# riveSunder/therldaisyworld

Hardware: AMD Instinct MI355X
Metric: cell-updates/sec (grid x batch), fused stencil+growth step (higher is better)
Workload: dtype f32

## Files before the change

therldaisyworld_amd/csrc/dw_api.hip:

```cpp
#include <hip/hip_runtime.h>

#include <cmath>
#include <cstdarg>
#include <cstdio>
#include <cstdlib>
#include <cstring>
#include <memory>
#include <new>
#include <optional>
#include <type_traits>
#include <vector>

#include "../../include/daisyworld_hip.h"
#include "dw_kernels.hpp"
#include "dw_host_util.hpp"
#include "dw_plan.hpp"
#include "dw_series.hpp"
#include "dw_episode_staging.hpp"

using namespace dw;

static thread_local char g_err[512] = "";

static int fail(int code, const char* fmt, ...) {
    va_list ap;
    va_start(ap, fmt);
    vsnprintf(g_err, sizeof(g_err), fmt, ap);
    va_end(ap);
    return code;
}

#define HIPCHK(expr)                                                                           \
    do {                                                                                       \
        hipError_t e_ = (expr);                                                                \
        if (e_ != hipSuccess)                                                                  \
            return fail(e_ == hipErrorOutOfMemory ? DW_ENOMEM : DW_EHIP, "%s failed: %s (%s:%d)", \
                        #expr, hipGetErrorString(e_), __FILE__, __LINE__);                      \
    } while (0)

#define NEED(cond, code, ...)                      \
    do {                                           \
        if (!(cond)) return fail(code, __VA_ARGS__); \
    } while (0)

enum UnqKind { UNQ_F64 = 1, UNQ_F32 = 2 };
enum UnqOwner { OWN_NONE = 0, OWN_CUR = 1, OWN_PREV = 2 };

static thread_local int t_fail_in = 0;
struct DeviceMem {
    static int alloc(void** p, size_t n) {
        if (t_fail_in > 0 && --t_fail_in == 0) return hipErrorOutOfMemory;
        return hipMalloc(p, n);
    }
    static int release(void* p) { return hipFree(p); }
};
struct PinnedMem {
    static int alloc(void** p, size_t n) { return hipHostMalloc(p, n, hipHostMallocDefault); }
    static int release(void* p) { return hipHostFree(p); }
};
template <class T> using DevBuf = Buf<T, DeviceMem>;
template <class T> using PinnedBuf = Buf<T, PinnedMem>;

struct dw_handle {
    dw_params prm;
    hipStream_t stream = nullptr;
    bool own_stream = false;
    size_t cells = 0;
    DevBuf<plane_t> L16[2];
    DevBuf<plane_t> D16[2];
    int cur = 0;
    DevBuf<double> L64;
    DevBuf<double> D64;
    DevBuf<float> U32L;
    DevBuf<float> U32D;
    UnqKind unq_kind = UNQ_F64;
    UnqOwner unq = OWN_NONE;
    bool have_state = false;
    bool stepped = false;
    double L_last = 0.0;
    bool L_per_world = false;
    bool P_per_world = false;
    DevBuf<int> idx;
    DevBuf<double> st;
    DevBuf<int> action;
    DevBuf<int> action_tmp;
    bool have_agents = false;
    DevBuf<StatsDev> stats2[2];
    size_t stats_bytes = 0;
    int sp = 0;
    DevBuf<uint4> fixq;
    unsigned int qcap = 0;
    DevBuf<int> redo_tiles;
    Switches sw{};
    StepPlan plan{};
    DevBuf<int> done_at;
    DevBuf<int> agents_done_at;
    DevBuf<int> n_alive;
    DevBuf<double> scratch;
    DevBuf<unsigned char> ep_buf;
    DevBuf<double> mlp_w;
    int mlp_members = 0;
    PinnedBuf<unsigned char> ep_pinned;
    DevBuf<double> reward_d;
    DevBuf<unsigned char> done_d;
    hipEvent_t ev0 = nullptr, ev1 = nullptr;
    hipEvent_t evf0 = nullptr, evf1 = nullptr;
    int fused_launches = 0;
    DevBuf<StatsDev> side_stats;
    DevBuf<StatsDev> trace_d;
    DevBuf<TempStatsDev> temp_d;
    DevBuf<TempPartial> temp_part;
    DevBuf<unsigned char> pw_tab;
    PinnedBuf<unsigned char> pw_pinned;
    PinnedBuf<unsigned char> pinned;
    struct Snapshot {
        DevBuf<plane_t> L, D;
        DevBuf<plane_t> PL, PD;
        bool stepped = false;
        double L_last = 0.0;
        bool L_per_world = false, P_per_world = false;
        UnqOwner unq = OWN_NONE;
        DevBuf<int> idx;
        DevBuf<double> st;
        DevBuf<unsigned char> stats;
        bool valid = false, agents = false;
    } snap[DW_SNAPSHOT_SLOTS];
    std::vector<std::pair<const void*, size_t>> lds_limit;
    bool created = false;
};

static inline bool cur_quantised(const dw_handle* h) { return h->unq != OWN_CUR; }

static inline bool lacks_shared_L(const dw_handle* h) { return h->stepped && h->L_per_world; }
#define NEED_SHARED_L(h, what)                                                                                          \
    NEED(!lacks_shared_L(h), DW_ESTATE,                                                                                 \
         "%s derives its temperature channels from the last step's luminosity, and the last step "                      \
         "(dw_step_n_trace_per_world) took a per-world luminosity: take a shared-L step or upload a state first", what)
static inline bool lacks_shared_constants(const dw_handle* h) { return lacks_shared_L(h) && h->P_per_world; }
#define NEED_SHARED_CONSTANTS(h, what)                                                                                  \
    NEED(!lacks_shared_constants(h), DW_ESTATE,                                                                         \
         "%s evaluates the last step's input state with one set of constants, and the last step "                       \
         "(dw_step_n_trace_ensemble) took per-world constants: take a shared-L step or upload a state first", what)

template <int V> using int_c = std::integral_constant<int, V>;

template <int V, int... Vs, class F>
static decltype(auto) with_int(int v, F&& f) {
    if constexpr (sizeof...(Vs) == 0) return f(int_c<V>{});
    else return v == V ? f(int_c<V>{}) : with_int<Vs...>(v, f);
}

template <class F>
static decltype(auto) with_bool(bool b, F&& f) { return b ? f(std::true_type{}) : f(std::false_type{}); }

template <class P> using elem_t = std::remove_cv_t<std::remove_pointer_t<P>>;

template <class F>
static decltype(auto) with_unq_planes(const dw_handle* h, F&& f) {
    return h->unq_kind == UNQ_F64 ? f(h->L64.get(), h->D64.get()) : f(h->U32L.get(), h->U32D.get());
}

template <class F>
static decltype(auto) with_planes(const dw_handle* h, bool unq, int buf, F&& f) {
    return unq ? with_unq_planes(h, f) : f(h->L16[buf].get(), h->D16[buf].get());
}

template <class F>
static auto with_derived_from(const dw_handle* h, F&& f) {
    const bool post = h->stepped;
    return with_planes(h, h->unq == (post ? OWN_PREV : OWN_CUR), post ? 1 - h->cur : h->cur, [&](auto* L, auto* D) {
        return with_bool(post, [&](auto POST) { return f(L, D, POST); });
    });
}

struct SyncOnExit {
    hipStream_t stream;
    bool armed = true;
    explicit SyncOnExit(hipStream_t s) : stream(s) {}
    ~SyncOnExit() { if (armed) (void)hipStreamSynchronize(stream); }
    void disarm() { armed = false; }
};

static int alloc_failed(int rc, const char* what, size_t bytes) {
    (void)hipGetLastError();
    const hipError_t e = static_cast<hipError_t>(rc);
    return fail(e == hipErrorOutOfMemory ? DW_ENOMEM : DW_EHIP, "allocating %s (%zu bytes) failed: %s", what, bytes,
                hipGetErrorString(e));
}
template <class B>
static int reserve(B& buf, const char* what, size_t need, size_t first_size = 0) {
    const int rc = buf.reserve(need, first_size);
    return rc ? alloc_failed(rc, what, need) : DW_OK;
}

static int alloc_group(dw_handle* h, const char* what, std::initializer_list<GroupItem<DeviceMem>> group) {
    static int fail_left = -1;
    if (h->created && fail_left < 0)
        if (const char* e = test_hook("DW_TEST_FAIL_GROUP_ALLOC")) fail_left = std::atoi(e);
    const bool armed = h->created && fail_left > 0;
    if (armed) t_fail_in = (int)group.size();
    const int rc = dw::alloc_group(group);
    if (armed && t_fail_in == 0) --fail_left;
    t_fail_in = 0;
    size_t bytes = 0;
    for (const auto& g : group) bytes += g.bytes;
    return rc ? alloc_failed(rc, what, bytes) : DW_OK;
}

static void release_unquantised(dw_handle* h) {
    if (h->unq != OWN_NONE || !h->U32L.get()) return;
    for (const auto& sn : h->snap)
        if (sn.valid && sn.unq == OWN_PREV) return;
    if (h->cells * 2 * sizeof(float) < ((size_t)1 << 30)) return;
    (void)hipStreamSynchronize(h->stream);
    h->U32L.reset();
    h->U32D.reset();
}

static void drop_unquantised_previous(dw_handle* h) {
    if (h->unq == OWN_PREV) { h->unq = OWN_NONE; h->stepped = false; }
    release_unquantised(h);
}

static int ensure_u32(dw_handle* h) {
    const size_t n = sizeof(float) * h->cells;
    return alloc_group(h, "two float32 planes", {{h->U32L, n}, {h->U32D, n}});
}

static int ensure_f64(dw_handle* h) {
    const size_t n = sizeof(double) * h->cells;
    return alloc_group(h, "two float64 planes", {{h->L64, n}, {h->D64, n}});
}
// ... 87 lines not shown
static void fill_episode_io(IO& io, const dw_handle* h, const EpisodeStaging& S) {
    const int cur = h->cur, prev = 1 - h->cur;
    io.L = h->L16[cur].get(); io.D = h->D16[cur].get(); io.prevL = h->L16[prev].get(); io.prevD = h->D16[prev].get();
    io.idx = h->idx.get(); io.st = h->st.get();
    io.P32 = S.at<const PhysF32>(h->ep_buf.get(), EpisodeStaging::P32);
    io.Ls = S.at<const double>(h->ep_buf.get(), EpisodeStaging::LS);
    io.stats = h->stats2[h->sp].get();
    io.fixups = &io.stats[h->prm.batch].sum_l;
}

template <class Kernel>
static int set_lds_limit(dw_handle* h, Kernel kern, size_t bytes) {
    const void* k = reinterpret_cast<const void*>(kern);
    size_t* set = nullptr;
    for (auto& e : h->lds_limit)
        if (e.first == k) set = &e.second;
    if (set && *set >= bytes) return DW_OK;
    HIPCHK(hipFuncSetAttribute(k, hipFuncAttributeMaxDynamicSharedMemorySize, (int)bytes));
    if (set) *set = bytes;
    else h->lds_limit.emplace_back(k, bytes);
    return DW_OK;
}

static int ensure_fixq(dw_handle* h, const StepPlan& plan) {
    if (!plan.need_fixq) return DW_OK;
    const dw_params& p = h->prm;
    size_t per_q = (h->cells / 64 + kNumQueues - 1) / kNumQueues;
    if (per_q < 2048) per_q = 2048;
    per_q = (per_q + 255) / 256 * 256;
    const size_t max_tiles = (size_t)p.batch * ((p.height + 7) / 8) * ((p.width / 4 + 15) / 16);
    if (int rc = alloc_group(h, "the near-tie queues", {{h->fixq, sizeof(uint4) * 3 * per_q * kNumQueues},
                                                         {h->redo_tiles, sizeof(int) * max_tiles}}))
        return rc;
    h->qcap = (unsigned int)per_q;
    return DW_OK;
}

struct StepOut {
    plane_t* L; plane_t* D;
    PhysF32 P;
    PhysF64 P64;
    StatsDev* stats;
    unsigned long long* fixups;
    unsigned long long* zero_me;
    int zero_n;
};
static StepOut step_out(const dw_handle* h) {
    const int out = 1 - h->cur;
    StatsDev* stats = h->stats2[1 - h->sp].get();
    return StepOut{h->L16[out].get(), h->D16[out].get(), PhysF32{}, PhysF64{}, stats, &stats[h->prm.batch].sum_l,
                   reinterpret_cast<unsigned long long*>(h->stats2[h->sp].get()),
                   (int)(h->stats_bytes / sizeof(unsigned long long))};
}

template <int TCQ, int RPT, bool EXACT>
static int launch_tiled(dw_handle* h, const plane_t* iL, const plane_t* iD, const StepOut& o, const FixQ& fq) {
    auto kern = step_tiled<TCQ, RPT, EXACT>;
    if constexpr (TileCfg<TCQ, RPT>::LDS_BYTES > 64 * 1024)
        if (int rc = set_lds_limit(h, kern, TileCfg<TCQ, RPT>::LDS_BYTES)) return rc;
    const Geom& g = h->plan.geom;
    constexpr size_t lds_bytes = TileCfg<TCQ, RPT>::LDS_BYTES;
    hipLaunchKernelGGL(kern, dim3((unsigned)g.chunk * 8u), dim3(256), lds_bytes, h->stream, iL, iD, o.L, o.D, g, o.P, o.stats,
                       o.fixups, o.zero_me, o.zero_n, fq);
    HIPCHK(hipGetLastError());
    if (EXACT) {
        const dim3 qg((fq.qcap + 255) / 256, kNumQueues);
        hipLaunchKernelGGL(fixup_cells, qg, dim3(256), 0, h->stream, o.L, o.D, h->prm.height, h->prm.width, o.P64, o.stats, fq);
        hipLaunchKernelGGL(redo_tiles_f64, dim3(256), dim3(256), 0, h->stream, iL, iD, o.L, o.D, g, TileCfg<TCQ, RPT>::TR, TCQ,
                           o.P64, o.stats, fq);
        HIPCHK(hipGetLastError());
    }
    return DW_OK;
}

static dim3 generic_grid(const dw_params& p, int* cpt) {
    *cpt = generic_cells_per_thread(p.batch, (long long)p.height * p.width);
    return dim3((unsigned)(((long long)p.height * p.width + 256LL * *cpt - 1) / (256LL * *cpt)), (unsigned)p.batch);
}

template <class T, int PREC>
static auto launch_generic(dw_handle* h, const T* iL, const T* iD, const StepOut& o, const FirstStepBound& fb = {}) {
    const dw_params& p = h->prm;
    int cpt;
    const dim3 grid = generic_grid(p, &cpt);
    hipLaunchKernelGGL((step_generic<T, PREC>), grid, dim3(256), 0, h->stream, iL, iD, o.L, o.D, p.height, p.width, o.P, o.P64,
                       o.stats, o.fixups, o.zero_me, o.zero_n, cpt, fb);
}

static int launch_first_step(dw_handle* h, double L, const StepOut& o) {
    const StepPlan& pl = h->plan;
    const FirstStepBound fb = pl.first_prec == 3 ? derive_first_bound(h->prm, L, o.P, h->unq_kind == UNQ_F64, h->sw.first_slack)
                                                 : FirstStepBound{};
    if (pl.first_stream) {
        const dim3 grid((unsigned)((pl.first_geom.nstrips + 3) / 4));
        with_unq_planes(h, [&](auto* iL, auto* iD) {
            with_int<1, 3>(pl.first_prec, [&](auto PR) {
                with_int<0, 1, 2, 3>(pl.halo, [&](auto HL) {
                    hipLaunchKernelGGL((step_first_stream<elem_t<decltype(iL)>, PR, HL>), grid, dim3(256), 0, h->stream, iL, iD,
                                       o.L, o.D, pl.first_geom, o.P, o.P64, o.stats, o.fixups, o.zero_me, o.zero_n, fb);
                });
            });
        });
    } else {
        with_unq_planes(h, [&](auto* iL, auto* iD) {
            with_int<1, 3, 2>(pl.first_prec, [&](auto PR) { launch_generic<elem_t<decltype(iL)>, PR>(h, iL, iD, o, fb); });
        });
    }
    HIPCHK(hipGetLastError());
    return DW_OK;
}

static int launch_step(dw_handle* h, const StepOut& o) {
    const dw_params& p = h->prm;
    const StepPlan& pl = h->plan;
    const plane_t* iL = h->L16[h->cur].get();
    const plane_t* iD = h->D16[h->cur].get();
    const bool ex = p.precision == DW_PRECISION_EXACT;
    if (pl.kind == STEP_GENERIC) {
        const int prec = p.precision == DW_PRECISION_F64 ? 2 : (ex ? 0 : 1);
        with_int<2, 0, 1>(prec, [&](auto PR) { launch_generic<plane_t, PR>(h, iL, iD, o); });
    } else if (pl.kind == STEP_STREAM && ex) {
        const StreamExactArgs A{iL, iD, o.L, o.D, pl.sgeom, o.P, o.stats, o.fixups, o.zero_me, o.zero_n, o.P64};
        with_int<0, 1, 2, 3>(pl.halo, [&](auto HL) {
            with_bool(pl.sym_albedo, [&](auto SYM) {
                hipLaunchKernelGGL((step_stream_exact<HL, SYM>), dim3((unsigned)pl.sgeom.chunk * 8u), dim3(256), 0, h->stream, A);
            });
        });
    } else if (pl.kind == STEP_STREAM) {
        with_int<0, 1, 2, 3>(pl.halo, [&](auto HL) {
            hipLaunchKernelGGL((step_stream_fast<HL>), dim3((unsigned)pl.sgeom.chunk * 8u), dim3(256), 0, h->stream, iL, iD, o.L,
                               o.D, pl.sgeom, o.P, o.P64, o.stats, o.fixups, o.zero_me, o.zero_n);
        });
    } else {
        FixQ fq;
        fq.entries = h->fixq.get();
        fq.counts = reinterpret_cast<unsigned int*>(o.stats + p.batch + 1);
        fq.qcap = h->qcap;
        fq.redo_tiles = h->redo_tiles.get();
        auto tiled = [&](auto TCQ, auto RPT) {
            return with_bool(ex, [&](auto EX) { return launch_tiled<TCQ, RPT, EX>(h, iL, iD, o, fq); });
        };
        if (pl.tcq == 64) return with_int<8, 4, 2>(pl.rpt, [&](auto RPT) { return tiled(int_c<64>{}, RPT); });
        return pl.tcq == 32 ? tiled(int_c<32>{}, int_c<4>{}) : tiled(int_c<16>{}, int_c<2>{});
    }
    HIPCHK(hipGetLastError());
    return DW_OK;
}

static void step_done(dw_handle* h, double L, bool stepped, bool per_world = false, bool per_world_constants = false) {
    h->cur = 1 - h->cur;
    h->sp = 1 - h->sp;
    h->unq = h->unq == OWN_CUR ? OWN_PREV : OWN_NONE;
    h->stepped = stepped;
    h->L_last = L;
    h->L_per_world = per_world;
    h->P_per_world = per_world && per_world_constants;
    release_unquantised(h);
}

static void episode_done(dw_handle* h, double L_last, bool per_world) {
    h->unq = OWN_NONE;
    h->stepped = true;
    h->L_last = per_world ? 0.0 : L_last;
    h->L_per_world = per_world;
    h->P_per_world = per_world;
}

static int launch_forward(dw_handle* h, double L) {
    const dw_params& p = h->prm;
    NEED(h->have_state, DW_ESTATE, "no state uploaded (call dw_upload_state_* or dw_init_random)");
    StepOut o = step_out(h);
    o.P = derive_f32(p, L);
    o.P64 = make_f64(p, L);
#ifdef DW_TUNING
    if (const char* e = std::getenv("DW_ABLATE")) {
        if (std::strcmp(e, "copy") == 0) {
            const int in = h->cur;
            const size_t n4 = h->cells * sizeof(plane_t) / 16;
            hipLaunchKernelGGL(copy_planes, dim3((unsigned)((n4 + 255) / 256)), dim3(256), 0, h->stream,
                               reinterpret_cast<const float4*>(h->L16[in].get()), reinterpret_cast<const float4*>(h->D16[in].get()),
                               reinterpret_cast<float4*>(o.L), reinterpret_cast<float4*>(o.D), n4);
            HIPCHK(hipGetLastError());
            step_done(h, L, true);
            return DW_OK;
        }
        const int v = std::strcmp(e, "nomath") == 0 ? 1 : 0;
        HIPCHK(hipMemcpyToSymbolAsync(HIP_SYMBOL(g_ablate), &v, sizeof(int), 0, hipMemcpyHostToDevice, h->stream));
    }
#endif
    if (int rc = h->unq == OWN_CUR ? launch_first_step(h, L, o) : launch_step(h, o)) return rc;
    step_done(h, L, true);
    return DW_OK;
}

static int launch_forward_pw(dw_handle* h, const PhysF32* row32, const PhysF64* row64, const FirstStepBound* rowfb, bool sym,
                             bool constants) {
    const dw_params& p = h->prm;
    const StepPlan& pl = h->plan;
    const StepOut o = step_out(h);
    const bool ex = p.precision == DW_PRECISION_EXACT;
    auto generic = [&](auto* iL, auto* iD, auto PR) {
        int cpt;
        const dim3 grid = generic_grid(p, &cpt);
        hipLaunchKernelGGL((step_generic_pw<elem_t<decltype(iL)>, PR>), grid, dim3(256), 0, h->stream, iL, iD, o.L, o.D,
                           p.height, p.width, row32, row64, rowfb, o.stats, o.fixups, o.zero_me, o.zero_n, cpt);
    };
    const plane_t* iL = h->L16[h->cur].get();
    const plane_t* iD = h->D16[h->cur].get();
    if (h->unq == OWN_CUR) {
        with_unq_planes(h, [&](auto* uL, auto* uD) {
            with_int<1, 3, 2>(pl.first_prec, [&](auto PR) { generic(uL, uD, PR); });
        });
    } else if (pl.pw_stream && ex) {
        const StreamExactPwArgs A{iL, iD, o.L, o.D, pl.sgeom, row32, row64, o.stats, o.fixups, o.zero_me, o.zero_n};
        with_int<0, 1, 2>(pl.halo, [&](auto HL) {
            with_bool(sym, [&](auto SYM) {
                hipLaunchKernelGGL((step_stream_exact_pw<HL, SYM>), dim3((unsigned)pl.sgeom.chunk * 8u), dim3(256), 0, h->stream, A);
            });
        });
    } else if (pl.pw_stream) {
        with_int<0, 1, 2>(pl.halo, [&](auto HL) {
            hipLaunchKernelGGL((step_stream_fast_pw<HL>), dim3((unsigned)pl.sgeom.chunk * 8u), dim3(256), 0, h->stream, iL, iD, o.L,
                               o.D, pl.sgeom, row32, row64, o.stats, o.fixups, o.zero_me, o.zero_n);
        });
    } else {
        const int prec = p.precision == DW_PRECISION_F64 ? 2 : (ex ? 0 : 1);
        with_int<2, 0, 1>(prec, [&](auto PR) { generic(iL, iD, PR); });
    }
    HIPCHK(hipGetLastError());
    step_done(h, 0.0, true, true, constants);
    return DW_OK;
}

static int launch_forward_fused2_pw(dw_handle* h, const PairPw* row, StatsDev* trace) {
    const StepPlan& pl = h->plan;
    const StepOut o = step_out(h);
    const FusedGeom& g = pl.fgeom;
    const dim3 grid((unsigned)g.chunk * 8u);
    const plane_t *inL = h->L16[h->cur].get(), *inD = h->D16[h->cur].get();
    with_int<kFusedRot, kFusedOvl>(pl.fused_mode, [&](auto MODE) {
        hipLaunchKernelGGL((trace_pair_fast_pw<MODE>), grid, dim3(256), 0, h->stream, inL, inD, o.L, o.D, g, row, o.zero_me,
                           o.zero_n, trace);
    });
    HIPCHK(hipGetLastError());
    step_done(h, 0.0, false, true, true);
    return DW_OK;
}

static int temp_chunks(const dw_handle* h) {
    return (int)(((long long)h->prm.height * h->prm.width + kTempChunk - 1) / kTempChunk);
}
static size_t temp_part_bytes(const dw_handle* h) { return sizeof(TempPartial) * (size_t)h->prm.batch * temp_chunks(h); }

static int launch_temp_moments(dw_handle* h, bool current, double L, const PhysF64* row64, TempStatsDev* out) {
    const dw_params& p = h->prm;
    const int chunks = temp_chunks(h);
    const PhysF64 P = row64 ? PhysF64{} : make_f64(p, L);
    TempPartial* part = h->temp_part.get();
    auto reduce = [&](auto* iL, auto* iD) {
        with_bool(row64 != nullptr, [&](auto TABLE) {
            hipLaunchKernelGGL((temp_moments_pw<elem_t<decltype(iL)>, TABLE>), dim3((unsigned)chunks, (unsigned)p.batch), dim3(256),
                               0, h->stream, iL, iD, p.height, p.width, P, row64, part);
        });
    };
    if (current) with_planes(h, h->unq == OWN_CUR, h->cur, reduce);
    else with_derived_from(h, [&](auto* iL, auto* iD, auto) { reduce(iL, iD); });
    HIPCHK(hipGetLastError());
    hipLaunchKernelGGL(temp_moments_finish_pw, dim3((unsigned)((p.batch + 63) / 64)), dim3(64), 0, h->stream, part, p.batch, chunks,
                       (double)p.height * (double)p.width, out);
    HIPCHK(hipGetLastError());
    return DW_OK;
}

template <class F>
static auto with_fused_layout(const StepPlan& pl, F&& f) {
    if (pl.packed) return f(int_c<kFusedRot>{}, std::true_type{});
    return with_int<kFusedRot, kFusedRing, kFusedOvl>(pl.fused_mode, [&](auto MODE) { return f(MODE, std::false_type{}); });
}

static int launch_forward_fused2(dw_handle* h, double L1, double L2, unsigned int* pstats = nullptr,
                                 float thr_hi = 0.f, StatsDev* trace = nullptr) {
    const dw_params& p = h->prm;
    const StepPlan& pl = h->plan;
    const bool exact = p.precision == DW_PRECISION_EXACT;
    PhysF32 P1, P2;
    if (exact) derive_f32_pair(p, L1, L2, &P1, &P2);
    else { P1 = derive_f32(p, L1); P2 = derive_f32(p, L2); }
    const StepOut o = step_out(h);
    const FusedGeom& g = pl.fgeom;
    const dim3 grid((unsigned)g.chunk * 8u);
    const plane_t *inL = h->L16[h->cur].get(), *inD = h->D16[h->cur].get();
    auto exact_args = [&] {
        return FusedExactArgs{inL, inD, o.L, o.D, g, P1, lum_part(P2), o.zero_me, o.zero_n, pstats, thr_hi, make_f64(p, L1), L1, L2};
    };
    if (trace && exact) {
        const TraceExactArgs A{exact_args(), trace, h->sw.force_rescan ? 1 : 0};
        with_int<kFusedRot, kFusedOvl>(pl.fused_mode, [&](auto MODE) {
            with_bool(pl.sym_albedo, [&](auto SYM) {
                hipLaunchKernelGGL((trace_pair_exact<MODE, SYM>), grid, dim3(256), 0, h->stream, A);
            });
        });
    } else if (trace) {
        with_int<kFusedRot, kFusedOvl>(pl.fused_mode, [&](auto MODE) {
            hipLaunchKernelGGL((trace_pair_fast<MODE>), grid, dim3(256), 0, h->stream, inL, inD, o.L, o.D, g, P1, P2, o.zero_me,
                               o.zero_n, trace);
        });
    } else if (pl.seam_strips && !pstats && !exact) {
        const FusedGeom &gs = pl.seam_geom, &gl = pl.left_geom;
        hipLaunchKernelGGL(step_stream_fused2_seam_pw, dim3((unsigned)gs.chunk * 8u), dim3(256), 0, h->stream, inL, inD, o.L, o.D,
                           gs, P1, P2, o.zero_me, o.zero_n);
        if (gl.nstrips)
            hipLaunchKernelGGL(step_stream_fused2_left_pw, dim3((unsigned)gl.chunk * 8u), dim3(256), 0, h->stream, inL, inD, o.L,
                               o.D, gl, P1, P2, o.zero_me, 0);
    } else if (pl.fmt_planes && !pstats && !exact) {
        hipLaunchKernelGGL((step_stream_fused2_fmt_pw<kFusedOvl>), grid, dim3(256), 0, h->stream, inL, inD, o.L, o.D, g, P1, P2,
                           o.zero_me, o.zero_n);
    } else if (exact) {
        const FusedExactArgs A = exact_args();
        with_bool(pstats != nullptr, [&](auto STATS) {
            with_fused_layout(pl, [&](auto MODE, auto PACK) {
                with_bool(pl.sym_albedo, [&](auto SYM) {
                    hipLaunchKernelGGL((step_stream_fused2_exact<MODE, PACK, STATS, SYM>), grid, dim3(256), 0, h->stream, A);
                });
            });
        });
    } else {
        with_bool(pstats != nullptr, [&](auto STATS) {
            with_fused_layout(pl, [&](auto MODE, auto PACK) {
                hipLaunchKernelGGL((step_stream_fused2<MODE, PACK, STATS>), grid, dim3(256), 0, h->stream, inL, inD, o.L, o.D, g,
                                   P1, P2, o.zero_me, o.zero_n, pstats, thr_hi);
            });
        });
    }
    HIPCHK(hipGetLastError());
    step_done(h, L2, false);
    return DW_OK;
}

static int launch_agents(dw_handle* h, const int* d_action, int act_b, int act_n, bool standalone = false,
                         double* d_reward = nullptr, unsigned char* d_done = nullptr, unsigned char* d_ok = nullptr) {
    const dw_params& p = h->prm;
    if (p.n_agents == 0) return DW_OK;
    NEED(h->have_state, DW_ESTATE, "no state uploaded");
    NEED(h->have_agents, DW_ESTATE, "no agents uploaded (call dw_upload_agents or dw_init_random)");
    NEED(p.collision_mode == 0 || standalone, DW_EINVAL,
         "collision_mode=1: call dw_update_agents, apply the collision pass (it consumes the caller's RNG) to the "
         "downloaded agent states, upload them, then dw_step without actions");
    const int blocks = (p.batch + 63) / 64;
    with_planes(h, h->unq == OWN_CUR, h->cur, [&](auto* L, auto* D) {
        using T = elem_t<decltype(L)>;
        hipLaunchKernelGGL(agents_update<T>, dim3(blocks), dim3(64), 0, h->stream, L, D, h->idx.get(), h->st.get(), d_action,
                           act_b, act_n, p.batch, p.n_agents, p.height, p.width, p.agent_gamma,
                           p.collision_mode == 0 ? 1 : 0, d_reward, d_done, d_ok);
    });
    HIPCHK(hipGetLastError());
    return DW_OK;
}

static int stage_host_actions(dw_handle* h, const int32_t* action, int b, int n) {
    const dw_params& p = h->prm;
    NEED(b >= 0 && n >= 0 && b <= p.batch && n <= p.n_agents, DW_EINVAL,
         "action block %dx%d exceeds (B,N)=(%d,%d)", b, n, p.batch, p.n_agents);
    if ((size_t)b * n)
        HIPCHK(hipMemcpyAsync(h->action_tmp.get(), action, sizeof(int) * (size_t)b * n, hipMemcpyHostToDevice,
                              h->stream));
    return DW_OK;
}

static int clear_stats(dw_handle* h) {
    for (int i = 0; i < 2; ++i) HIPCHK(hipMemsetAsync(h->stats2[i].get(), 0, h->stats_bytes, h->stream));
    return DW_OK;
}

static void state_arrived(dw_handle* h, UnqOwner unq, UnqKind kind = UNQ_F64) {
    if (unq == OWN_CUR) h->unq_kind = kind;
    h->unq = unq;
    h->have_state = true;
    h->stepped = false;
    for (auto& sn : h->snap) sn.valid = false;
}

template <class T>
static auto init_random_into(dw_handle* h, uint64_t seed, T* L, T* D) {
    const dw_params& p = h->prm;
    if (int crc = clear_stats(h)) return crc;
    const int ncell = p.height * p.width;
    const dim3 g((unsigned)((ncell + kInitChunk - 1) / kInitChunk), (unsigned)p.batch);
    hipLaunchKernelGGL((init_random_cells<T>), g, dim3(256), 0, h->stream, L, D, ncell,
                       (long long)p.world_offset, (unsigned long long)seed, (float)p.light_proportion,
                       (float)p.dark_proportion, (float)p.initial_al, (float)p.initial_ad, h->stats2[h->sp].get());
    HIPCHK(hipGetLastError());
    if (p.n_agents) {
        const int bn = p.batch * p.n_agents;
        hipLaunchKernelGGL(init_random_agents, dim3((bn + 255) / 256), dim3(256), 0, h->stream, h->idx.get(), h->st.get(),
                           p.batch, p.n_agents, p.height, p.width, (long long)p.world_offset,
                           (unsigned long long)seed);
        HIPCHK(hipGetLastError());
    }
    h->have_agents = true;
    return (int)DW_OK;
}

extern "C" {

const char* dw_last_error(void) { return g_err; }
int dw_abi_version(void) { return DW_ABI_VERSION; }

int dw_pinned_alloc(size_t bytes, void** out) {
    NEED(out && bytes > 0, DW_EINVAL, "null argument");
    int ndev = 0;
    NEED(hipGetDeviceCount(&ndev) == hipSuccess && ndev > 0, DW_ENODEVICE, "no HIP device");
    HIPCHK(hipHostMalloc(out, bytes, hipHostMallocDefault));
    return DW_OK;
}
int dw_pinned_free(void* p) {
    if (p) HIPCHK(hipHostFree(p));
    return DW_OK;
}

#ifndef DW_BUILD_ID
#define DW_BUILD_ID "unknown"
#endif
static const char kBuildId[] = "DW_BUILD_ID=" DW_BUILD_ID;
const char* dw_build_id(void) { return kBuildId + 12; }

int dw_default_params(dw_params* p, int32_t batch, int32_t height, int32_t width, int32_t n_agents) {
    NEED(p, DW_EINVAL, "null params");
    std::memset(p, 0, sizeof(*p));
    p->abi_version = DW_ABI_VERSION;
    p->batch = batch; p->height = height; p->width = width; p->n_agents = n_agents;
    p->device = 0; p->precision = DW_PRECISION_EXACT; p->obs_mask = 0x0BA; p->collision_mode = 0;
    p->world_offset = 0;
    p->p = 1.0; p->g = 0.003265; p->S = 1000.0; p->sigma = 5.67e-8; p->gamma = 0.25;
    p->q = 0.2 * p->S / p->sigma; p->q2 = p->q / 8.0; p->dt = 1.0;
    p->albedo_bare = 0.5; p->albedo_light = 0.75; p->albedo_dark = 0.25; p->temp_optimal = 295.5;
    p->agent_gamma = 0.05; p->food_chain_penalty = 0.5;
    p->initial_al = 0.2; p->initial_ad = 0.2; p->light_proportion = 0.33; p->dark_proportion = 0.33;
    return DW_OK;
}

static int check_params(const dw_params* p) {
    NEED(p, DW_EINVAL, "null params");
    NEED(p->abi_version == DW_ABI_VERSION, DW_EINVAL, "ABI version %d != %d", p->abi_version, DW_ABI_VERSION);
    NEED(p->batch >= 1 && p->height >= 3 && p->width >= 3, DW_EINVAL,
         "need batch>=1 and grid >= 3x3 (got B=%d H=%d W=%d)", p->batch, p->height, p->width);
    NEED(p->height <= 65535 && p->width <= 65532, DW_EINVAL, "grid dimension too large");
    NEED((long long)p->height * p->width <= 0x7fffffffLL, DW_EINVAL,
         "a world of %dx%d cells exceeds the 2^31-1 cells per world the kernels index", p->height, p->width);
    NEED(p->n_agents >= 0, DW_EINVAL, "n_agents < 0");
    NEED(p->precision >= 0 && p->precision <= 2, DW_EINVAL, "bad precision %d", p->precision);
    NEED(p->precision == DW_PRECISION_F64 || p->g >= 0.0, DW_EINVAL,
         "g < 0 (a growth curve opening upwards) is evaluated by DW_PRECISION_F64 only");
    NEED((double)p->batch * p->height * p->width < 9.0e18, DW_EINVAL, "too many cells");
    return DW_OK;
}

int dw_create(const dw_params* p, dw_handle** out) {
    NEED(out, DW_EINVAL, "null out");
    *out = nullptr;
    int rc = check_params(p);
    if (rc) return rc;
    int ndev = 0;
    if (hipGetDeviceCount(&ndev) != hipSuccess || ndev <= 0)
        return fail(DW_ENODEVICE, "no HIP device available (this library has no CPU fallback)");
    NEED(p->device >= 0 && p->device < ndev, DW_ENODEVICE, "device %d out of range (%d devices)", p->device, ndev);
    HIPCHK(hipSetDevice(p->device));
    hipDeviceProp_t prop;
    HIPCHK(hipGetDeviceProperties(&prop, p->device));
    if (std::strncmp(prop.gcnArchName, "gfx950", 6) != 0)
        return fail(DW_ENODEVICE, "device %d is %s; this library is built for gfx950 only", p->device,
                    prop.gcnArchName);
    std::unique_ptr<dw_handle, int (*)(dw_handle*)> h(new (std::nothrow) dw_handle(), dw_destroy);
    NEED(h, DW_ENOMEM, "host allocation failed");
    h->prm = *p;
    h->cells = (size_t)p->batch * p->height * p->width;
    HIPCHK(hipStreamCreateWithFlags(&h->stream, hipStreamNonBlocking));
    h->own_stream = true;
    const size_t bn = (size_t)p->batch * (p->n_agents > 0 ? p->n_agents : 1);
    const size_t pb = sizeof(plane_t) * h->cells;
    h->stats_bytes = sizeof(StatsDev) * (p->batch + 1) + sizeof(unsigned int) * (kNumQueues + 1) * 16;
    if (int rc = alloc_group(h.get(), "the handle's state",
                             {{h->L16[0], pb}, {h->D16[0], pb}, {h->L16[1], pb}, {h->D16[1], pb},
                              {h->idx, sizeof(int) * bn * 2}, {h->st, sizeof(double) * bn}, {h->action, sizeof(int) * bn},
                              {h->action_tmp, sizeof(int) * bn}, {h->reward_d, sizeof(double) * bn}, {h->done_d, bn},
                              {h->agents_done_at, sizeof(int) * bn}, {h->done_at, sizeof(int) * p->batch},
                              {h->n_alive, sizeof(int)}, {h->stats2[0], h->stats_bytes}, {h->stats2[1], h->stats_bytes},
                              {h->side_stats, sizeof(StatsDev) * (p->batch + 1)}}))
        return rc;
    for (int i = 0; i < 2; ++i) HIPCHK(hipMemsetAsync(h->stats2[i].get(), 0, h->stats_bytes, h->stream));
    h->sw = read_switches();
    h->plan = plan_steps(*p, h->sw);
    if (int rc = ensure_fixq(h.get(), h->plan)) return rc;
    HIPCHK(hipMemsetAsync(h->action.get(), 0, sizeof(int) * bn, h->stream));
    HIPCHK(hipMemsetAsync(h->done_at.get(), 0, sizeof(int) * p->batch, h->stream));
    HIPCHK(hipMemsetAsync(h->agents_done_at.get(), 0, sizeof(int) * bn, h->stream));
    HIPCHK(hipMemsetAsync(h->n_alive.get(), 0, sizeof(int), h->stream));
    HIPCHK(hipEventCreate(&h->ev0));
    HIPCHK(hipEventCreate(&h->ev1));
    HIPCHK(hipEventCreate(&h->evf0));
    HIPCHK(hipEventCreate(&h->evf1));
    h->created = true;
    *out = h.release();
    return DW_OK;
}

int dw_destroy(dw_handle* h) {
    if (!h) return DW_OK;
    (void)hipSetDevice(h->prm.device);
    if (h->stream) (void)hipStreamSynchronize(h->stream);
    if (h->ev0) (void)hipEventDestroy(h->ev0);
    if (h->ev1) (void)hipEventDestroy(h->ev1);
    if (h->evf0) (void)hipEventDestroy(h->evf0);
    if (h->evf1) (void)hipEventDestroy(h->evf1);
    if (h->own_stream && h->stream) (void)hipStreamDestroy(h->stream);
    delete h;
    return DW_OK;
}

int dw_set_params(dw_handle* h, const dw_params* p) {
    NEED(h, DW_EINVAL, "null handle");
    int rc = check_params(p);
    if (rc) return rc;
    const dw_params& o = h->prm;
    NEED(p->batch == o.batch && p->height == o.height && p->width == o.width && p->n_agents == o.n_agents &&
             p->device == o.device,
         DW_EINVAL, "dw_set_params cannot change shape or device; create a new handle");
    HIPCHK(hipSetDevice(p->device));
    const StepPlan plan = plan_steps(*p, h->sw);
    if ((rc = ensure_fixq(h, plan))) return rc;
    h->prm = *p;
    h->plan = plan;
    return DW_OK;
}

int dw_get_params(const dw_handle* h, dw_params* out) {
    NEED(h && out, DW_EINVAL, "null argument");
    *out = h->prm;
    return DW_OK;
}


static int refresh_stats(dw_handle* h) {
    const dw_params& p = h->prm;
    if (int rc = clear_stats(h)) return rc;
    const int n = p.height * p.width;
    const dim3 g((unsigned)((n + kInitChunk - 1) / kInitChunk), (unsigned)p.batch);
    auto reduce = [&](auto* L, auto* D) {
        hipLaunchKernelGGL((stats_only<elem_t<decltype(L)>>), g, dim3(256), 0, h->stream, L, D, n, h->stats2[h->sp].get());
    };
    if (cur_quantised(h)) reduce(h->L16[h->cur].get(), h->D16[h->cur].get());
    else with_unq_planes(h, reduce);
    HIPCHK(hipGetLastError());
    return DW_OK;
}

int dw_upload_state_f64(dw_handle* h, const double* light, const double* dark) {
    NEED(h && light && dark, DW_EINVAL, "null argument");
    HIPCHK(hipSetDevice(h->prm.device));
    if (int arc = ensure_f64(h)) return arc;
    HIPCHK(hipMemcpyAsync(h->L64.get(), light, sizeof(double) * h->cells, hipMemcpyHostToDevice, h->stream));
    HIPCHK(hipMemcpyAsync(h->D64.get(), dark, sizeof(double) * h->cells, hipMemcpyHostToDevice, h->stream));
    state_arrived(h, OWN_CUR, UNQ_F64);
    int rc = refresh_stats(h);
    if (rc) return rc;
    HIPCHK(hipStreamSynchronize(h->stream));
    return DW_OK;
}

int dw_upload_state_f32(dw_handle* h, const float* light, const float* dark, int quantised) {
    NEED(h && light && dark, DW_EINVAL, "null argument");
    HIPCHK(hipSetDevice(h->prm.device));
    const unsigned blocks = (unsigned)((h->cells + 255) / 256);
    if (quantised) {
        int rc = ensure_scratch(h, sizeof(float) * 2 * h->cells);
        if (rc) return rc;
        float* sL = reinterpret_cast<float*>(h->scratch.get());
        float* sD = sL + h->cells;
        HIPCHK(hipMemcpyAsync(sL, light, sizeof(float) * h->cells, hipMemcpyHostToDevice, h->stream));
        HIPCHK(hipMemcpyAsync(sD, dark, sizeof(float) * h->cells, hipMemcpyHostToDevice, h->stream));
        hipLaunchKernelGGL(f32nat_to_plane, dim3(blocks), dim3(256), 0, h->stream, sL, h->L16[h->cur].get(), h->cells);
        hipLaunchKernelGGL(f32nat_to_plane, dim3(blocks), dim3(256), 0, h->stream, sD, h->D16[h->cur].get(), h->cells);
        HIPCHK(hipGetLastError());
        state_arrived(h, OWN_NONE);
    } else {
        int rc = ensure_u32(h);
        if (rc) return rc;
        HIPCHK(hipMemcpyAsync(h->U32L.get(), light, sizeof(float) * h->cells, hipMemcpyHostToDevice, h->stream));
        HIPCHK(hipMemcpyAsync(h->U32D.get(), dark, sizeof(float) * h->cells, hipMemcpyHostToDevice, h->stream));
        hipLaunchKernelGGL(f32nat_to_permille, dim3(blocks), dim3(256), 0, h->stream, h->U32L.get(), h->U32L.get(), h->cells);
        hipLaunchKernelGGL(f32nat_to_permille, dim3(blocks), dim3(256), 0, h->stream, h->U32D.get(), h->U32D.get(), h->cells);
        HIPCHK(hipGetLastError());
        state_arrived(h, OWN_CUR, UNQ_F32);
    }
    int rc = refresh_stats(h);
    if (rc) return rc;
    HIPCHK(hipStreamSynchronize(h->stream));
    return DW_OK;
}

int dw_upload_agents(dw_handle* h, const int32_t* indices, const double* states) {
    NEED(h, DW_EINVAL, "null handle");
    const dw_params& p = h->prm;
    HIPCHK(hipSetDevice(p.device));
    const size_t bn = (size_t)p.batch * p.n_agents;
    if (bn) {
        NEED(indices && states, DW_EINVAL, "null argument");
        for (size_t i = 0; i < bn; ++i) {
            NEED(indices[2 * i] >= 0 && indices[2 * i] < p.height && indices[2 * i + 1] >= 0 &&
                     indices[2 * i + 1] < p.width,
                 DW_EINVAL, "agent %zu position (%d,%d) outside the %dx%d grid", i, indices[2 * i],
                 indices[2 * i + 1], p.height, p.width);
        }
        HIPCHK(hipMemcpyAsync(h->idx.get(), indices, sizeof(int) * bn * 2, hipMemcpyHostToDevice, h->stream));
        HIPCHK(hipMemcpyAsync(h->st.get(), states, sizeof(double) * bn, hipMemcpyHostToDevice, h->stream));
        HIPCHK(hipStreamSynchronize(h->stream));
    }
    h->have_agents = true;
    return DW_OK;
}

int dw_download_agents(dw_handle* h, int32_t* indices, double* states) {
    NEED(h, DW_EINVAL, "null handle");
    const dw_params& p = h->prm;
    HIPCHK(hipSetDevice(p.device));
    const size_t bn = (size_t)p.batch * p.n_agents;
    if (bn) {
        NEED(h->have_agents, DW_ESTATE, "no agents");
        if (indices) HIPCHK(hipMemcpyAsync(indices, h->idx.get(), sizeof(int) * bn * 2, hipMemcpyDeviceToHost, h->stream));
        if (states) HIPCHK(hipMemcpyAsync(states, h->st.get(), sizeof(double) * bn, hipMemcpyDeviceToHost, h->stream));
    }
    HIPCHK(hipStreamSynchronize(h->stream));
    return DW_OK;
}

int dw_init_random(dw_handle* h, uint64_t seed) {
    NEED(h, DW_EINVAL, "null handle");
    HIPCHK(hipSetDevice(h->prm.device));
    if (int rc = ensure_u32(h)) return rc;
    if (int rc = init_random_into(h, seed, h->U32L.get(), h->U32D.get())) return rc;
    state_arrived(h, OWN_CUR, UNQ_F32);
    return DW_OK;
}

int dw_init_random_quantised(dw_handle* h, uint64_t seed) {
    NEED(h, DW_EINVAL, "null handle");
    HIPCHK(hipSetDevice(h->prm.device));
    if (int rc = init_random_into(h, seed, h->L16[h->cur].get(), h->D16[h->cur].get())) return rc;
    state_arrived(h, OWN_NONE);
    release_unquantised(h);
    return DW_OK;
}

int dw_download_planes(dw_handle* h, int which, double* light, double* dark) {
    NEED(h, DW_EINVAL, "null handle");
    NEED(h->have_state, DW_ESTATE, "no state");
    HIPCHK(hipSetDevice(h->prm.device));
    NEED(which == DW_STATE_CURRENT || which == DW_STATE_PREVIOUS, DW_EINVAL, "bad state selector");
    NEED(which == DW_STATE_CURRENT || h->stepped, DW_ESTATE, "no previous state before the first step");
    const int buf = which == DW_STATE_CURRENT ? h->cur : 1 - h->cur;
    const bool unq = (which == DW_STATE_CURRENT && h->unq == OWN_CUR) || (which == DW_STATE_PREVIOUS && h->unq == OWN_PREV);
    const size_t bytes = sizeof(double) * h->cells;
    if (unq && h->unq_kind == UNQ_F64) {
        if (light) HIPCHK(hipMemcpyAsync(light, h->L64.get(), bytes, hipMemcpyDeviceToHost, h->stream));
        if (dark) HIPCHK(hipMemcpyAsync(dark, h->D64.get(), bytes, hipMemcpyDeviceToHost, h->stream));
    } else {
        int rc = ensure_scratch(h, bytes);
        if (rc) return rc;
        const unsigned blocks = (unsigned)((h->cells + 255) / 256);
        for (int pl = 0; pl < 2; ++pl) {
            double* dst = pl == 0 ? light : dark;
            if (!dst) continue;
            if (unq)
                hipLaunchKernelGGL((plane_to_f64<float>), dim3(blocks), dim3(256), 0, h->stream,
                                   pl == 0 ? h->U32L.get() : h->U32D.get(), h->scratch.get(), h->cells);
            else
                hipLaunchKernelGGL((plane_to_f64<plane_t>), dim3(blocks), dim3(256), 0, h->stream,
                                   pl == 0 ? h->L16[buf].get() : h->D16[buf].get(), h->scratch.get(), h->cells);
            HIPCHK(hipGetLastError());
            HIPCHK(hipMemcpyAsync(dst, h->scratch.get(), bytes, hipMemcpyDeviceToHost, h->stream));
        }
    }
    HIPCHK(hipStreamSynchronize(h->stream));
    return DW_OK;
}

static int run_materialise(dw_handle* h, double L, double* d_grid7, double* d_temps, double* d_betas,
                           double* d_growth, double* d_teff) {
    const dw_params& p = h->prm;
    const dim3 g((unsigned)((p.height * p.width + 255) / 256), (unsigned)p.batch);
    const PhysF64 P = make_f64(p, h->stepped && !h->L_per_world ? h->L_last : L);
    const plane_t* cL = h->L16[h->cur].get();
    const plane_t* cD = h->D16[h->cur].get();
    with_derived_from(h, [&](auto* pL, auto* pD, auto POST) {
        hipLaunchKernelGGL((materialise<elem_t<decltype(pL)>, POST>), g, dim3(256), 0, h->stream, pL, pD, cL, cD, p.height,
                           p.width, P, d_grid7, d_temps, d_betas, d_growth, d_teff);
    });
    HIPCHK(hipGetLastError());
    if (h->stepped && d_grid7 && p.n_agents && h->have_agents) {
        hipLaunchKernelGGL(agents_stamp, dim3((p.batch + 63) / 64), dim3(64), 0, h->stream, d_grid7, h->idx.get(),
                           h->st.get(), p.batch, p.n_agents, p.height, p.width);
        HIPCHK(hipGetLastError());
    }
    return DW_OK;
}

int dw_download_grid(dw_handle* h, double L_init, double* grid7) {
    NEED(h && grid7, DW_EINVAL, "null argument");
    NEED(h->have_state, DW_ESTATE, "no state");
    NEED_SHARED_L(h, "dw_download_grid");
    HIPCHK(hipSetDevice(h->prm.device));
    const size_t bytes = sizeof(double) * 7 * h->cells;
    int rc = ensure_scratch(h, bytes);
    if (rc) return rc;
    rc = run_materialise(h, L_init, h->scratch.get(), nullptr, nullptr, nullptr, nullptr);
    if (rc) return rc;
    HIPCHK(hipMemcpyAsync(grid7, h->scratch.get(), bytes, hipMemcpyDeviceToHost, h->stream));
    HIPCHK(hipStreamSynchronize(h->stream));
    return DW_OK;
}

int dw_download_caches(dw_handle* h, double L, double* temps, double* betas, double* growth,
                       double* temp_effective) {
    NEED(h, DW_EINVAL, "null handle");
    NEED(h->have_state, DW_ESTATE, "no state");
    NEED_SHARED_CONSTANTS(h, "dw_download_caches");
    HIPCHK(hipSetDevice(h->prm.device));
    const size_t n = h->cells;
    int rc = ensure_scratch(h, sizeof(double) * 9 * n);
    if (rc) return rc;
    double* d_t = h->scratch.get();
    double* d_b = d_t + 3 * n;
    double* d_g = d_b + 3 * n;
    double* d_e = d_g + 2 * n;
    rc = run_materialise(h, L, nullptr, temps ? d_t : nullptr, betas ? d_b : nullptr, growth ? d_g : nullptr,
                         temp_effective ? d_e : nullptr);
    if (rc) return rc;
    if (temps) HIPCHK(hipMemcpyAsync(temps, d_t, sizeof(double) * 3 * n, hipMemcpyDeviceToHost, h->stream));
    if (betas) HIPCHK(hipMemcpyAsync(betas, d_b, sizeof(double) * 3 * n, hipMemcpyDeviceToHost, h->stream));
    if (growth) HIPCHK(hipMemcpyAsync(growth, d_g, sizeof(double) * 2 * n, hipMemcpyDeviceToHost, h->stream));
    if (temp_effective) HIPCHK(hipMemcpyAsync(temp_effective, d_e, sizeof(double) * n, hipMemcpyDeviceToHost, h->stream));
    HIPCHK(hipStreamSynchronize(h->stream));
    return DW_OK;
}

int dw_reduce_temperature(dw_handle* h, double L, dw_temp_stats* per_world) {
    NEED(h && per_world, DW_EINVAL, "null argument");
    NEED(h->have_state, DW_ESTATE, "no state");
    NEED_SHARED_CONSTANTS(h, "dw_reduce_temperature");
    static_assert(sizeof(dw_temp_stats) == sizeof(TempStatsDev), "temperature record layout");
    HIPCHK(hipSetDevice(h->prm.device));
    const size_t bytes = sizeof(TempStatsDev) * (size_t)h->prm.batch;
    if (int rc = alloc_group(h, "the temperature reduction", {{h->temp_part, temp_part_bytes(h)}, {h->temp_d, bytes}})) return rc;
    if (int rc = launch_temp_moments(h, false, h->stepped && !h->L_per_world ? h->L_last : L, nullptr, h->temp_d.get())) return rc;
    HIPCHK(hipMemcpyAsync(per_world, h->temp_d.get(), bytes, hipMemcpyDeviceToHost, h->stream));
    HIPCHK(hipStreamSynchronize(h->stream));
    return DW_OK;
}


int dw_update_agents(dw_handle* h, const int32_t* action, int32_t action_b, int32_t action_n) {
    NEED(h && action, DW_EINVAL, "null argument");
    HIPCHK(hipSetDevice(h->prm.device));
    int rc = stage_host_actions(h, action, action_b, action_n);
    if (rc) return rc;
    return launch_agents(h, h->action_tmp.get(), action_b, action_n, true);
}

int dw_step(dw_handle* h, const int32_t* action, int32_t action_b, int32_t action_n, double L) {
    NEED(h, DW_EINVAL, "null handle");
    HIPCHK(hipSetDevice(h->prm.device));
    if (action) {
        int rc = stage_host_actions(h, action, action_b, action_n);
        if (rc) return rc;
        rc = launch_agents(h, h->action_tmp.get(), action_b, action_n);
        if (rc) return rc;
    }
    return launch_forward(h, L);
}

int dw_step_device_actions(dw_handle* h, double L) {
    NEED(h, DW_EINVAL, "null handle");
    HIPCHK(hipSetDevice(h->prm.device));
    int rc = launch_agents(h, h->action.get(), h->prm.batch, h->prm.n_agents);
    if (rc) return rc;
    return launch_forward(h, L);
}

int dw_upload_actions(dw_handle* h, const int32_t* action) {
    NEED(h && action, DW_EINVAL, "null argument");
    HIPCHK(hipSetDevice(h->prm.device));
    const size_t bn = (size_t)h->prm.batch * h->prm.n_agents;
    if (bn) {
        HIPCHK(hipMemcpyAsync(h->action.get(), action, sizeof(int) * bn, hipMemcpyHostToDevice, h->stream));
        HIPCHK(hipStreamSynchronize(h->stream));
    }
    return DW_OK;
}

int dw_download_actions(dw_handle* h, int32_t* action) {
    NEED(h && action, DW_EINVAL, "null argument");
    HIPCHK(hipSetDevice(h->prm.device));
    const size_t bn = (size_t)h->prm.batch * h->prm.n_agents;
    if (bn) HIPCHK(hipMemcpyAsync(action, h->action.get(), sizeof(int) * bn, hipMemcpyDeviceToHost, h->stream));
    HIPCHK(hipStreamSynchronize(h->stream));
    return DW_OK;
}

int dw_step_n(dw_handle* h, int32_t nsteps, double* L_io, double dL, double min_L, double max_L,
              int use_device_actions) {
    NEED(h && L_io, DW_EINVAL, "null argument");
    NEED(nsteps >= 0, DW_EINVAL, "nsteps < 0");
    HIPCHK(hipSetDevice(h->prm.device));
    double L = *L_io;
    auto advance = [&]() { L += dL; L = L > max_L ? max_L : L; L = L < min_L ? min_L : L; };
    int s0 = 0;
    h->fused_launches = 0;
    if (!use_device_actions && nsteps >= 1 && h->have_state && !cur_quantised(h)) {
        int rc = launch_forward(h, L);
        if (rc) return rc;
        advance();
        s0 = 1;
    }
    const bool big_packed = h->plan.allow_fuse && h->plan.packed && h->cells >= ((size_t)1 << 23);
    if (!use_device_actions && nsteps - s0 > 1 && h->have_state && h->prm.height * h->prm.width <= 4096 && !big_packed &&
        episode_kernel_applies(h)) {
        std::vector<double> Ls;
        while (s0 < nsteps) {
            const int k = nsteps - s0 < 4096 ? nsteps - s0 : 4096;
            Ls.resize(k);
            for (int i = 0; i < k; ++i) { Ls[i] = L; advance(); }
            int rc = run_episode_impl(h, k, Ls.data(), kPolicySkipAgents, nullptr, nullptr, 5, nullptr, nullptr);
            if (rc) return rc;
            s0 += k;
        }
        *L_io = L;
        return DW_OK;
    }
    if (!use_device_actions && h->plan.allow_fuse && h->have_state && nsteps - s0 >= 3) {
        drop_unquantised_previous(h);
        HIPCHK(hipEventRecord(h->evf0, h->stream));
        int launched = 0;
        while (nsteps - s0 >= 3) {
            const double L1 = L;
            advance();
            const double L2 = L;
            advance();
            int rc = launch_forward_fused2(h, L1, L2);
            if (rc) return rc;
            s0 += 2;
            launched += 1;
        }
        HIPCHK(hipEventRecord(h->evf1, h->stream));
        h->fused_launches = launched;
    }
    for (int s = s0; s < nsteps; ++s) {
        int rc;
        if (use_device_actions) {
            rc = launch_agents(h, h->action.get(), h->prm.batch, h->prm.n_agents);
            if (rc) return rc;
        }
        rc = launch_forward(h, L);
        if (rc) return rc;
        advance();
    }
    *L_io = L;
    return DW_OK;
}

static bool ensemble_pairs(const dw_handle* h) { return h->plan.trace_pairs && h->prm.precision == DW_PRECISION_FAST; }

static int check_per_world(const WorldRows& rows, const dw_world_params* worlds, const double* L_schedule, size_t nsteps, size_t B) {
    for (size_t i = 0; i < nsteps * B; ++i)
        NEED(std::isfinite(L_schedule[i]) && L_schedule[i] >= 0.0, DW_EINVAL,
             "L_schedule[step %zu][world %zu] = %g: a luminosity is finite and not negative", i / B, i % B, L_schedule[i]);
    for (size_t b = 0; worlds && b < B; ++b) {
        if (check_params(&rows.params(b)) != DW_OK) {
            char why[sizeof(g_err)];
            snprintf(why, sizeof(why), "%s", g_err);
            return fail(DW_EINVAL, "worlds[%zu].g = %g: %s", b, worlds[b].g, why);
        }
    }
    return DW_OK;
}

struct PwTable {
    dw_handle* h;
    const PwLayout lay;
    hipEvent_t uploaded = nullptr;
    bool in_flight = false;
    PwTable(dw_handle* h_, const PwLayout& lay_) : h(h_), lay(lay_) {}
    PwTable(const PwTable&) = delete;
    ~PwTable() { if (uploaded) (void)hipEventDestroy(uploaded); }
    unsigned char* img() const { return h->pw_pinned.get(); }
    unsigned char* dev() const { return h->pw_tab.get(); }
    GroupItem<DeviceMem> item() const { return {h->pw_tab, lay.bytes}; }
    int alloc(const char* what, std::initializer_list<GroupItem<DeviceMem>> group) {
        if (int rc = alloc_group(h, what, group)) return rc;
        if (int rc = reserve(h->pw_pinned, "the page-locked image of the per-world constants", lay.bytes)) {
            h->pw_tab.reset();
            return rc;
        }
        HIPCHK(hipEventCreateWithFlags(&uploaded, hipEventDisableTiming));
        return DW_OK;
    }
    int next_chunk(const SeriesSchedule& q, size_t c, const double* Ls, WorldRows& worlds, bool first_bound = false) {
        if (in_flight) HIPCHK(hipEventSynchronize(uploaded));
        fill_chunk(q, c, Ls, worlds, lay, img());
        if (first_bound) worlds.first_bound(Ls, lay.p32(img(), 0), h->unq_kind == UNQ_F64, h->sw.first_slack, lay.fb(img()));
        auto part = [&](size_t off, size_t bytes) { return hipMemcpyAsync(dev() + off, img() + off, bytes, hipMemcpyHostToDevice, h->stream); };
        const size_t singles = q.chunks[c].singles, pairs = q.chunks[c].pairs;
        if (singles) {
            HIPCHK(part(0, sizeof(PhysF32) * singles * lay.B));
            HIPCHK(part(lay.o64, sizeof(PhysF64) * singles * lay.B));
        }
        if (first_bound) HIPCHK(part(lay.ofb, sizeof(FirstStepBound) * lay.B));
        if (pairs) HIPCHK(part(lay.opair, sizeof(PairPw) * pairs * lay.B));
        HIPCHK(hipEventRecord(uploaded, h->stream));
        in_flight = true;
        return DW_OK;
    }
};

struct SeriesRun {
    dw_handle* h;
    const SeriesSchedule& q;
    const double* Ls;
    dw_world_stats* trace;
    dw_temp_stats* temps;
    PwTable* table;
    bool sym, constants;
    size_t B, row_bytes, trow_bytes;
    bool first_pair = true;
    bool keep_rows() const { return trace || q.even; }

    int alloc() {
        const GroupItem<DeviceMem> tr{h->trace_d, keep_rows() ? q.rows * row_bytes : 0}, part{h->temp_part, temp_part_bytes(h)},
            td{h->temp_d, q.rows * trow_bytes};
        if (!table) return temps ? alloc_group(h, "the trace buffer and the temperature reduction", {tr, part, td})
                                 : alloc_group(h, "the trace buffer", {tr});
        if (temps) return table->alloc("the per-world constants, the trace buffer and the temperature reduction", {table->item(), tr, part, td});
        return keep_rows() ? table->alloc("the per-world constants and the trace buffer", {table->item(), tr})
                           : table->alloc("the per-world constants", {table->item()});
    }
    int step(int t) {
        const size_t sr = (size_t)t % q.rows, tr = table ? q.row_of[(size_t)t] : 0;
        StatsDev* row = keep_rows() ? h->trace_d.get() + sr * B : nullptr;
        unsigned char* tab = table ? table->dev() : nullptr;
        if (q.is_pair[(size_t)t]) {
            if (first_pair) drop_unquantised_previous(h);
            first_pair = false;
            return table ? launch_forward_fused2_pw(h, table->lay.pair(tab, tr), row)
                         : launch_forward_fused2(h, Ls[t], Ls[t + 1], nullptr, 0.f, row);
        }
        const PhysF64* r64 = table ? table->lay.p64(tab, tr) : nullptr;
        if (temps)
            if (int rc = launch_temp_moments(h, true, table ? 0.0 : Ls[t], r64, h->temp_d.get() + sr * B)) return rc;
        if (int rc = table ? launch_forward_pw(h, table->lay.p32(tab, tr), r64, table->lay.fb(tab), sym, constants)
                           : launch_forward(h, Ls[t])) return rc;
        if (row) HIPCHK(hipMemcpyAsync(row, h->stats2[h->sp].get(), row_bytes, hipMemcpyDeviceToDevice, h->stream));
        return DW_OK;
    }
    int run(WorldRows* worlds) {
        const int nsteps = (int)q.is_pair.size();
        const bool first_bound = h->unq == OWN_CUR && h->plan.first_prec == 3;
        size_t c = 0;
        for (int t = 0; t < nsteps; t += q.took(t)) {
            const size_t sr = (size_t)t % q.rows, left = (size_t)(nsteps - t), filled = sr + (size_t)q.took(t);
            if (table && t == (c ? q.chunks[c - 1].end : 0)) {
                if (int rc = table->next_chunk(q, c, Ls, *worlds, c == 0 && first_bound)) return rc;
                ++c;
            }
            if (q.even && sr == 0)
                HIPCHK(hipMemsetAsync(h->trace_d.get(), 0, (left < q.rows ? left : q.rows) * row_bytes, h->stream));
            if (int rc = step(t)) return rc;
            if (filled != q.rows && t + q.took(t) != nsteps) continue;
            const size_t r0 = ((size_t)t - sr) * B;
            if (temps) HIPCHK(hipMemcpyAsync(temps + r0, h->temp_d.get(), filled * trow_bytes, hipMemcpyDeviceToHost, h->stream));
            if (trace) HIPCHK(hipMemcpyAsync(trace + r0, h->trace_d.get(), filled * row_bytes, hipMemcpyDeviceToHost, h->stream));
        }
        return DW_OK;
    }
};

enum SeriesForm { SHARED_L, PER_WORLD_L, PER_WORLD_CONSTANTS };
static int run_series(dw_handle* h, int32_t nsteps, const double* L_schedule, dw_world_stats* trace, dw_temp_stats* temps,
                      bool always_even, bool may_pair, SeriesForm form = SHARED_L, const dw_world_params* worlds = nullptr) {
    const bool pw = form != SHARED_L;
    NEED(nsteps >= 0, DW_EINVAL, "nsteps < 0");
    if (nsteps == 0) return DW_OK;
    NEED(h->have_state, DW_ESTATE, "no state uploaded (call dw_upload_state_* or dw_init_random)");
    static_assert(sizeof(dw_world_stats) == sizeof(StatsDev), "stats layout");
    static_assert(sizeof(dw_temp_stats) == sizeof(TempStatsDev), "temperature record layout");
    const dw_params& p = h->prm;
    const size_t B = (size_t)p.batch;
    std::unique_ptr<WorldRows> rows(pw ? new WorldRows(p, worlds, B) : nullptr);
    if (int rc = pw ? check_per_world(*rows, worlds, L_schedule, (size_t)nsteps, B) : DW_OK) return rc;
    const bool sym = worlds ? worlds_symmetric(worlds, B) && !h->sw.no_sym : h->plan.sym_albedo;
    HIPCHK(hipSetDevice(p.device));
    const SeriesSchedule q = plan_series(SeriesSpec{nsteps, B, sizeof(StatsDev), sizeof(TempStatsDev), h->sw.trace_rows, always_even,
                                                    may_pair, cur_quantised(h), temps != nullptr, pw ? L_schedule : nullptr});
    std::unique_ptr<PwTable> table(pw ? new PwTable(h, PwLayout(B, q.trows, q.prows)) : nullptr);
    SeriesRun run{h, q, L_schedule, trace, temps, table.get(), sym, form == PER_WORLD_CONSTANTS, B, sizeof(StatsDev) * B, sizeof(TempStatsDev) * B};
    if (int rc = run.alloc()) return rc;
    SyncOnExit sync(h->stream);
    h->fused_launches = 0;
    if (int rc = run.run(rows.get())) return rc;
    HIPCHK(hipStreamSynchronize(h->stream));
    sync.disarm();
    return DW_OK;
}

int dw_step_n_trace(dw_handle* h, int32_t nsteps, const double* L_schedule, dw_world_stats* trace) {
    NEED(h && L_schedule && trace, DW_EINVAL, "null argument");
    return run_series(h, nsteps, L_schedule, trace, nullptr, true, h->plan.trace_pairs);
}

int dw_step_n_trace_per_world(dw_handle* h, int32_t nsteps, const double* L_schedule, dw_world_stats* trace) {
    NEED(h && L_schedule, DW_EINVAL, "null argument");
    return run_series(h, nsteps, L_schedule, trace, nullptr, false, false, PER_WORLD_L);
}

int dw_world_params_of(const dw_handle* h, dw_world_params* out) {
    NEED(h && out, DW_EINVAL, "null argument");
    *out = world_params_of(h->prm);
    return DW_OK;
}

int dw_step_n_trace_ensemble(dw_handle* h, int32_t nsteps, const dw_world_params* worlds, const double* L_schedule,
                             dw_world_stats* trace, dw_temp_stats* temps) {
    static_assert(sizeof(dw_world_params) == 96, "dw_world_params layout");
    NEED(h && worlds && L_schedule, DW_EINVAL, "null argument");
    return run_series(h, nsteps, L_schedule, trace, temps, false, ensemble_pairs(h), PER_WORLD_CONSTANTS, worlds);
}

int dw_step_n_trace_temperature(dw_handle* h, int32_t nsteps, const double* L_schedule, int per_world, dw_world_stats* trace,
                                dw_temp_stats* temps) {
    NEED(h && L_schedule && temps, DW_EINVAL, "null argument");
    return run_series(h, nsteps, L_schedule, trace, temps, false, false, per_world ? PER_WORLD_L : SHARED_L);
}

int dw_last_step_n_timing(dw_handle* h, float* fused_ms, int32_t* fused_launches, int32_t* plane_elem_bytes) {
    NEED(h && fused_ms && fused_launches && plane_elem_bytes, DW_EINVAL, "null argument");
    HIPCHK(hipSetDevice(h->prm.device));
    *fused_ms = 0.f;
    *fused_launches = h->fused_launches;
    *plane_elem_bytes = (int32_t)sizeof(plane_t);
    if (h->fused_launches > 0) {
        HIPCHK(hipEventSynchronize(h->evf1));
        HIPCHK(hipEventElapsedTime(fused_ms, h->evf0, h->evf1));
    }
    return DW_OK;
}

int dw_forward_f64(dw_handle* h, const double* light, const double* dark, double L, double* grid7,
                   double* temps, double* betas, double* growth, double* temp_effective) {
    NEED(h && light && dark && grid7, DW_EINVAL, "null argument");
    const dw_params& p = h->prm;
    HIPCHK(hipSetDevice(p.device));
    const size_t n = h->cells;
    int rc = ensure_scratch(h, sizeof(double) * 18 * n + sizeof(plane_t) * 2 * n + 16);
    if (rc) return rc;
    double* dL = h->scratch.get();
    double* dD = dL + n;
    double* dG = dD + n;
    double* d_t = dG + 7 * n;
    double* d_b = d_t + 3 * n;
    double* d_g = d_b + 3 * n;
    double* d_e = d_g + 2 * n;
    plane_t* nL = reinterpret_cast<plane_t*>(d_e + n);
    plane_t* nD = nL + n;
    StatsDev* tmp_stats = h->side_stats.get();
    HIPCHK(hipMemsetAsync(tmp_stats, 0, sizeof(StatsDev) * (p.batch + 1), h->stream));
    HIPCHK(hipMemcpyAsync(dL, light, sizeof(double) * n, hipMemcpyHostToDevice, h->stream));
    {
        const hipError_t e2 = hipMemcpyAsync(dD, dark, sizeof(double) * n, hipMemcpyHostToDevice, h->stream);
        if (e2 != hipSuccess) {
            (void)hipStreamSynchronize(h->stream);
            return fail(DW_EHIP, "dw_forward_f64: %s", hipGetErrorString(e2));
        }
    }
    const PhysF32 P = derive_f32(p, L);
    const PhysF64 P64 = make_f64(p, L);
    const dim3 g((unsigned)((p.height * p.width + 255) / 256), (unsigned)p.batch);
    unsigned long long* tmp_fix = &tmp_stats[p.batch].sum_l;
    hipLaunchKernelGGL((step_generic<double, 2>), g, dim3(256), 0, h->stream, dL, dD, nL, nD, p.height, p.width, P,
                       P64, tmp_stats, tmp_fix, (unsigned long long*)nullptr, 0);
    hipLaunchKernelGGL((materialise<double, true>), g, dim3(256), 0, h->stream, dL, dD, nL, nD, p.height, p.width,
                       P64, dG, temps ? d_t : (double*)nullptr, betas ? d_b : (double*)nullptr,
                       growth ? d_g : (double*)nullptr, temp_effective ? d_e : (double*)nullptr);
    hipError_t le = hipGetLastError();
    if (le == hipSuccess && p.n_agents && h->have_agents) {
        hipLaunchKernelGGL(agents_stamp, dim3((p.batch + 63) / 64), dim3(64), 0, h->stream, dG, h->idx.get(), h->st.get(),
                           p.batch, p.n_agents, p.height, p.width);
        le = hipGetLastError();
    }
    if (le == hipSuccess) le = hipMemcpyAsync(grid7, dG, sizeof(double) * 7 * n, hipMemcpyDeviceToHost, h->stream);
    if (le == hipSuccess && temps) le = hipMemcpyAsync(temps, d_t, sizeof(double) * 3 * n, hipMemcpyDeviceToHost, h->stream);
    if (le == hipSuccess && betas) le = hipMemcpyAsync(betas, d_b, sizeof(double) * 3 * n, hipMemcpyDeviceToHost, h->stream);
    if (le == hipSuccess && growth) le = hipMemcpyAsync(growth, d_g, sizeof(double) * 2 * n, hipMemcpyDeviceToHost, h->stream);
    if (le == hipSuccess && temp_effective)
        le = hipMemcpyAsync(temp_effective, d_e, sizeof(double) * n, hipMemcpyDeviceToHost, h->stream);
    const hipError_t se = hipStreamSynchronize(h->stream);
    if (le == hipSuccess) le = se;
    if (le != hipSuccess) return fail(DW_EHIP, "dw_forward_f64: %s", hipGetErrorString(le));
    return DW_OK;
}

int dw_conv3x3_f64(dw_handle* h, const double* plane, const double kernel[9], double* out) {
    NEED(h && plane && kernel && out, DW_EINVAL, "null argument");
    const dw_params& p = h->prm;
    HIPCHK(hipSetDevice(p.device));
    const size_t n = h->cells;
    int rc = ensure_scratch(h, sizeof(double) * 2 * n);
    if (rc) return rc;
    double* d_in = h->scratch.get();
    double* d_out = d_in + n;
    Kernel9 K;
    for (int i = 0; i < 9; ++i) K.k[i] = kernel[i];
    SyncOnExit guard(h->stream);
    HIPCHK(hipMemcpyAsync(d_in, plane, sizeof(double) * n, hipMemcpyHostToDevice, h->stream));
    const dim3 g((unsigned)((p.height * p.width + 255) / 256), (unsigned)p.batch);
    hipLaunchKernelGGL(conv3x3_f64, g, dim3(256), 0, h->stream, d_in, d_out, p.height, p.width, K);
    HIPCHK(hipGetLastError());
    HIPCHK(hipMemcpyAsync(out, d_out, sizeof(double) * n, hipMemcpyDeviceToHost, h->stream));
    HIPCHK(hipStreamSynchronize(h->stream));
    guard.disarm();
    return DW_OK;
}

int dw_stage_f64(dw_handle* h, int stage, const double* in, double* out, double L, const double kernel[9]) {
    NEED(h && in && out, DW_EINVAL, "null argument");
    NEED(stage >= kStageAlbedo && stage <= kStageGrowth, DW_EINVAL, "bad stage %d", stage);
    NEED(kernel || stage > kStageDensity, DW_EINVAL, "the stencil stages need their 3x3 kernel");
    const dw_params& p = h->prm;
    HIPCHK(hipSetDevice(p.device));
    const size_t n = h->cells, nin = (size_t)stage_inputs(stage), nout = (size_t)stage_outputs(stage);
    int rc = ensure_scratch(h, sizeof(double) * (nin + nout) * n);
    if (rc) return rc;
    double* d_in = h->scratch.get();
    double* d_out = d_in + nin * n;
    Kernel9 K{};
    if (kernel) for (int i = 0; i < 9; ++i) K.k[i] = kernel[i];
    const PhysF64 P = make_f64(p, L);
    SyncOnExit guard(h->stream);
    HIPCHK(hipMemcpyAsync(d_in, in, sizeof(double) * nin * n, hipMemcpyHostToDevice, h->stream));
    const dim3 g((unsigned)((p.height * p.width + 255) / 256), (unsigned)p.batch);
    with_int<kStageAlbedo, kStageDensity, kStageTemperature, kStageGrowthRate, kStageGrowth>(stage, [&](auto S) {
        hipLaunchKernelGGL((stage_f64<S>), g, dim3(256), 0, h->stream, d_in, d_out, p.batch, p.height, p.width, P, K);
    });
    HIPCHK(hipGetLastError());
    HIPCHK(hipMemcpyAsync(out, d_out, sizeof(double) * nout * n, hipMemcpyDeviceToHost, h->stream));
    HIPCHK(hipStreamSynchronize(h->stream));
    guard.disarm();
    return DW_OK;
}

int dw_get_obs(dw_handle* h, double L_init, double* obs) {
    NEED(h, DW_EINVAL, "null handle");
    const dw_params& p = h->prm;
    HIPCHK(hipSetDevice(p.device));
    const size_t bn = (size_t)p.batch * p.n_agents;
    if (bn == 0) return DW_OK;
    NEED(obs, DW_EINVAL, "null obs");
    NEED(h->have_state && h->have_agents, DW_ESTATE, "no state / agents");
    int rc = observe_into_scratch(h, L_init, 0);
    if (rc) return rc;
    HIPCHK(hipMemcpyAsync(obs, h->scratch.get(), sizeof(double) * bn * 63, hipMemcpyDeviceToHost, h->stream));
    HIPCHK(hipStreamSynchronize(h->stream));
    return DW_OK;
}

int dw_env_step(dw_handle* h, const int32_t* action, int32_t action_b, int32_t action_n, double L, double* obs,
                double* reward, uint8_t* done) {
    NEED(h, DW_EINVAL, "null handle");
    const dw_params& p = h->prm;
    HIPCHK(hipSetDevice(p.device));
    const size_t bn = (size_t)p.batch * p.n_agents;
    auto up = [](size_t v) { return (v + 255) / 256 * 256; };
    const bool big_obs = sizeof(double) * bn * 63 > ((size_t)512 << 10);
    const size_t o_act = 0, o_obs = up(sizeof(int) * bn), o_rew = o_obs + sizeof(double) * bn * 63;
    const size_t total = up(o_rew + sizeof(double) * bn + bn) + 256;
    if (int rc = reserve(h->pinned, "the page-locked step staging", total)) return rc;
    if (action) {
        NEED(action_b >= 0 && action_n >= 0 && action_b <= p.batch && action_n <= p.n_agents, DW_EINVAL,
             "action block %dx%d exceeds (B,N)=(%d,%d)", action_b, action_n, p.batch, p.n_agents);
        const size_t na = (size_t)action_b * action_n;
        if (na) {
            std::memcpy(h->pinned.get() + o_act, action, sizeof(int) * na);
            HIPCHK(hipMemcpyAsync(h->action_tmp.get(), h->pinned.get() + o_act, sizeof(int) * na, hipMemcpyHostToDevice, h->stream));
        }
        int rc = launch_agents(h, h->action_tmp.get(), action_b, action_n);
        if (rc) return rc;
    }
    int rc = launch_forward(h, L);
    if (rc) return rc;
    if (bn) {
        NEED(h->have_agents, DW_ESTATE, "no agents");
        const size_t d_rew = sizeof(double) * bn * 63, d_done = d_rew + sizeof(double) * bn, d_total = d_done + bn;
        rc = observe_into_scratch(h, L, d_total - d_rew + 64, true);
        if (rc) return rc;
        unsigned char* blk = reinterpret_cast<unsigned char*>(h->scratch.get());
        if (big_obs) {
            if (obs) HIPCHK(hipMemcpyAsync(obs, blk, d_rew, hipMemcpyDeviceToHost, h->stream));
            HIPCHK(hipMemcpyAsync(h->pinned.get() + o_rew, blk + d_rew, d_total - d_rew, hipMemcpyDeviceToHost, h->stream));
        } else {
            HIPCHK(hipMemcpyAsync(h->pinned.get() + o_obs, blk, d_total, hipMemcpyDeviceToHost, h->stream));
        }
        HIPCHK(hipStreamSynchronize(h->stream));
        const unsigned char* src = big_obs ? h->pinned.get() + o_rew - d_rew : h->pinned.get() + o_obs;
        if (obs && !big_obs) std::memcpy(obs, src, d_rew);
        if (reward) std::memcpy(reward, src + d_rew, sizeof(double) * bn);
        if (done) std::memcpy(done, src + d_done, bn);
    }
    return DW_OK;
}

int dw_get_reward_done(dw_handle* h, double* reward, uint8_t* done) {
    NEED(h, DW_EINVAL, "null handle");
    const dw_params& p = h->prm;
    HIPCHK(hipSetDevice(p.device));
    const int bn = p.batch * p.n_agents;
    if (bn == 0) return DW_OK;
    NEED(h->have_agents, DW_ESTATE, "no agents");
    hipLaunchKernelGGL(reward_done, dim3((bn + 255) / 256), dim3(256), 0, h->stream, h->st.get(), h->reward_d.get(), h->done_d.get(), bn);
    HIPCHK(hipGetLastError());
    if (reward) HIPCHK(hipMemcpyAsync(reward, h->reward_d.get(), sizeof(double) * bn, hipMemcpyDeviceToHost, h->stream));
    if (done) HIPCHK(hipMemcpyAsync(done, h->done_d.get(), (size_t)bn, hipMemcpyDeviceToHost, h->stream));
    HIPCHK(hipStreamSynchronize(h->stream));
    return DW_OK;
}

int dw_reduce(dw_handle* h, dw_world_stats* per_world) {
    NEED(h && per_world, DW_EINVAL, "null argument");
    NEED(h->have_state, DW_ESTATE, "no state");
    static_assert(sizeof(dw_world_stats) == sizeof(StatsDev), "stats layout");
    HIPCHK(hipSetDevice(h->prm.device));
    HIPCHK(hipMemcpyAsync(per_world, h->stats2[h->sp].get(), sizeof(StatsDev) * h->prm.batch, hipMemcpyDeviceToHost,
                          h->stream));
    HIPCHK(hipStreamSynchronize(h->stream));
    return DW_OK;
}

static int launch_policy_greedy(dw_handle* h, int argmin, const int* agent_mode, int codes) {
    const dw_params& p = h->prm;
    const int bn = p.batch * p.n_agents;
    const dim3 g((unsigned)((bn + 255) / 256));
    if (h->unq == OWN_CUR && h->unq_kind == UNQ_F32)
        hipLaunchKernelGGL(policy_greedy<float>, g, dim3(256), 0, h->stream, h->U32L.get(), h->U32D.get(), h->idx.get(), p.batch, p.n_agents,
                           p.height, p.width, p.obs_mask, argmin, agent_mode, h->action.get(), codes);
    else
        hipLaunchKernelGGL(policy_greedy<plane_t>, g, dim3(256), 0, h->stream, h->L16[h->cur].get(), h->D16[h->cur].get(), h->idx.get(),
                           p.batch, p.n_agents, p.height, p.width, p.obs_mask, argmin, agent_mode, h->action.get(), codes);
    HIPCHK(hipGetLastError());
    return DW_OK;
}

int dw_policy_greedy(dw_handle* h, int mode) {
    NEED(h, DW_EINVAL, "null handle");
    const dw_params& p = h->prm;
    HIPCHK(hipSetDevice(p.device));
    const int bn = p.batch * p.n_agents;
    if (bn == 0) return DW_OK;
    NEED(h->have_state && h->have_agents, DW_ESTATE, "no state / agents");
    NEED(mode == DW_POLICY_ARGMAX || mode == DW_POLICY_ARGMIN, DW_EINVAL, "bad policy mode");
    NEED(cur_quantised(h) || h->unq_kind != UNQ_F64, DW_ESTATE,
         "device policy on an exact float64 initial state is not supported; compute the action on the host");
    return launch_policy_greedy(h, mode == DW_POLICY_ARGMIN ? 1 : 0, nullptr, 0);
}

int dw_policy_per_agent(dw_handle* h, const int32_t* agent_mode) {
    NEED(h && agent_mode, DW_EINVAL, "null argument");
    const dw_params& p = h->prm;
    HIPCHK(hipSetDevice(p.device));
    const int bn = p.batch * p.n_agents;
    if (bn == 0) return DW_OK;
    NEED(h->have_state && h->have_agents, DW_ESTATE, "no state / agents");
    NEED(cur_quantised(h) || h->unq_kind != UNQ_F64, DW_ESTATE,
         "device policy on an exact float64 initial state is not supported; compute the action on the host");
    for (int n = 0; n < p.n_agents; ++n)
        NEED(agent_mode[n] == DW_POLICY_ARGMAX || agent_mode[n] == DW_POLICY_ARGMIN || agent_mode[n] == DW_POLICY_TABLE,
             DW_EINVAL, "agent %d: bad policy mode %d", n, agent_mode[n]);
    std::vector<int> m(p.n_agents);
    for (int n = 0; n < p.n_agents; ++n) m[n] = agent_mode[n] == DW_POLICY_TABLE ? 2 : agent_mode[n];
    HIPCHK(hipMemcpyAsync(h->action_tmp.get(), m.data(), sizeof(int) * p.n_agents, hipMemcpyHostToDevice, h->stream));
    const int prc = launch_policy_greedy(h, 0, h->action_tmp.get(), 0);
    HIPCHK(hipStreamSynchronize(h->stream));
    return prc;
}

static int observe_into_scratch(dw_handle* h, double L_init, size_t extra_bytes, bool reward_tail) {
    const dw_params& p = h->prm;
    const size_t bn = (size_t)p.batch * p.n_agents;
    NEED_SHARED_L(h, "an observation");
    int rc = ensure_scratch(h, sizeof(double) * bn * 63 + extra_bytes);
    if (rc) return rc;
    double* d_rew = reward_tail ? h->scratch.get() + bn * 63 : nullptr;
    unsigned char* d_done = reward_tail ? reinterpret_cast<unsigned char*>(h->scratch.get() + bn * 64) : nullptr;
    const int threads = (int)(bn * 9);
    const dim3 g((threads + 127) / 128);
    const PhysF64 P = make_f64(p, h->stepped ? h->L_last : L_init);
    const plane_t* cL = h->L16[h->cur].get();
    const plane_t* cD = h->D16[h->cur].get();
    with_derived_from(h, [&](auto* pL, auto* pD, auto POST) {
        hipLaunchKernelGGL((observe<elem_t<decltype(pL)>, POST>), g, dim3(128), 0, h->stream, pL, pD, cL, cD, h->idx.get(),
                           h->st.get(), p.batch, p.n_agents, p.height, p.width, P, p.obs_mask, h->scratch.get(), d_rew, d_done);
    });
    HIPCHK(hipGetLastError());
    return DW_OK;
}

static int policy_mlp_impl(dw_handle* h, const double* params, int32_t n_members, const int32_t* world_member,
                           int32_t agent_begin, int32_t agent_end, double L_init) {
    const dw_params& p = h->prm;
    NEED(agent_begin >= 0 && agent_begin <= agent_end && agent_end <= p.n_agents, DW_EINVAL, "bad agent range");
    NEED(h->have_state && h->have_agents, DW_ESTATE, "no state / agents");
    const size_t bn = (size_t)p.batch * p.n_agents;
    if (bn == 0 || agent_begin == agent_end) return DW_OK;
    if (world_member)
        for (int b = 0; b < p.batch; ++b)
            NEED(world_member[b] >= 0 && world_member[b] < n_members, DW_EINVAL, "world %d: member %d out of range", b,
                 world_member[b]);
    const size_t wbytes = sizeof(double) * 1808 * (size_t)n_members;
    const size_t mbytes = world_member ? sizeof(int) * (size_t)p.batch : 0;
    int rc = observe_into_scratch(h, L_init, wbytes + mbytes + 16);
    if (rc) return rc;
    double* d_w = h->scratch.get() + bn * 63;
    int* d_m = world_member ? reinterpret_cast<int*>(d_w + 1808 * (size_t)n_members) : nullptr;
    SyncOnExit guard(h->stream);
    HIPCHK(hipMemcpyAsync(d_w, params, wbytes, hipMemcpyHostToDevice, h->stream));
    if (world_member) HIPCHK(hipMemcpyAsync(d_m, world_member, mbytes, hipMemcpyHostToDevice, h->stream));
    const int n = p.batch * (agent_end - agent_begin);
    hipLaunchKernelGGL(policy_mlp, dim3((n + 3) / 4), dim3(64), 0, h->stream, h->scratch.get(), d_w, d_m, p.batch,
                       p.n_agents, agent_begin, agent_end, h->action.get());
    HIPCHK(hipGetLastError());
    HIPCHK(hipStreamSynchronize(h->stream));
    guard.disarm();
    return DW_OK;
}

int dw_policy_mlp(dw_handle* h, const double* params, int32_t n_params, int32_t agent_begin, int32_t agent_end,
                  double L_init) {
    NEED(h && params, DW_EINVAL, "null argument");
    HIPCHK(hipSetDevice(h->prm.device));
    NEED(n_params == 63 * 16 + 16 * 32 + 32 * 9, DW_EINVAL, "the MLP policy has 1808 parameters (63-16-32-9), got %d", n_params);
    return policy_mlp_impl(h, params, 1, nullptr, agent_begin, agent_end, L_init);
}

int dw_policy_mlp_population(dw_handle* h, const double* params, int32_t n_members, const int32_t* world_member,
                             int32_t agent_begin, int32_t agent_end, double L_init) {
    NEED(h && params && world_member, DW_EINVAL, "null argument");
    HIPCHK(hipSetDevice(h->prm.device));
    NEED(n_members >= 1, DW_EINVAL, "n_members < 1");
    return policy_mlp_impl(h, params, n_members, world_member, agent_begin, agent_end, L_init);
}

int dw_run_episode_mlp(dw_handle* h, int32_t nsteps, const double* L_schedule, const double* params, int32_t n_members,
                       const int32_t* member_a, const int32_t* member_b, int32_t split, double L_init, double* reward,
                       uint8_t* done) {
    NEED(h && L_schedule, DW_EINVAL, "null argument");
    const dw_params& p = h->prm;
    HIPCHK(hipSetDevice(p.device));
    NEED(nsteps >= 1 && nsteps <= 4096, DW_EINVAL, "nsteps must be in 1..4096");
    NEED(n_members >= 1, DW_EINVAL, "n_members < 1");
    NEED(params || (h->mlp_w.get() && h->mlp_members == n_members), DW_ESTATE,
         "params == NULL but no parameter sets of %d members are on the device", n_members);
    NEED(p.collision_mode == 0, DW_EINVAL, "collision_mode=1 is not implemented on the device");
    NEED(split >= 0 && split <= p.n_agents, DW_EINVAL, "split outside 0..n_agents");
    NEED(h->have_state && h->have_agents, DW_ESTATE, "no state / agents");
    const int B = p.batch, N = p.n_agents;
    const size_t K = (size_t)nsteps, bn = (size_t)B * N;
    NEED(bn > 0, DW_EINVAL, "no agents");
    for (int b = 0; b < B; ++b) {
        NEED(!member_a || (member_a[b] >= 0 && member_a[b] < n_members), DW_EINVAL, "world %d: member out of range", b);
        NEED(!member_b || (member_b[b] >= 0 && member_b[b] < n_members), DW_EINVAL, "world %d: member out of range", b);
    }
    NEED(n_members == 1 || (member_a && member_b), DW_EINVAL, "several parameter sets need both member maps");
    const size_t wbytes = sizeof(double) * 1808 * (size_t)n_members;
    EpisodeRegions regions;
    regions.rows = K; regions.mlp = true;
    const EpisodeStaging S(K, (size_t)B, (size_t)N, regions);
    using R = EpisodeStaging;
    const size_t o_ma = S.off[R::MEMBER_A], o_mb = S.off[R::MEMBER_B], o_p32 = S.off[R::P32], o_ls = S.off[R::LS];
    if (int erc = ensure_ep_buf(h, S.total)) return erc;
    if (params) {
        if (h->mlp_members != n_members) {
            h->mlp_w.reset();
            h->mlp_members = 0;
            if (int rc = reserve(h->mlp_w, "the parameter sets", wbytes)) return rc;
            h->mlp_members = n_members;
        }
    }
    const double* d_w = h->mlp_w.get();
    const int* d_ma = member_a ? reinterpret_cast<const int*>(h->ep_buf.get() + o_ma) : nullptr;
    const int* d_mb = member_b ? reinterpret_cast<const int*>(h->ep_buf.get() + o_mb) : nullptr;
    double* d_r = S.at<double>(h->ep_buf.get(), R::REWARD);
    unsigned char* d_d = S.at<unsigned char>(h->ep_buf.get(), R::DONE);
    SyncOnExit guard(h->stream);
    if (params) HIPCHK(hipMemcpyAsync(h->mlp_w.get(), params, wbytes, hipMemcpyHostToDevice, h->stream));
    if (member_a) HIPCHK(hipMemcpyAsync(h->ep_buf.get() + o_ma, member_a, sizeof(int) * B, hipMemcpyHostToDevice, h->stream));
    if (member_b) HIPCHK(hipMemcpyAsync(h->ep_buf.get() + o_mb, member_b, sizeof(int) * B, hipMemcpyHostToDevice, h->stream));
    const int Cc = p.height * p.width;
    const int wpb = worlds_per_block(Cc);
    size_t lds = 0;
    const EpisodeForm form = episode_mlp_form(h, &lds);
    const bool wave_kernel = form == EPISODE_WAVE, small = form != EPISODE_STEPWISE;
    std::vector<PhysF32> p32;
    SyncOnExit guard2(h->stream);
    size_t t = 0;
    while (t < K) {
        if (small && cur_quantised(h) && h->stepped && h->unq == OWN_NONE) {
            NEED_SHARED_L(h, "the episode's first observation");
            const size_t Kr = K - t;
            p32.resize(Kr);
            for (size_t i = 0; i < Kr; ++i) p32[i] = derive_f32(p, L_schedule[t + i]);
            HIPCHK(hipMemcpyAsync(h->ep_buf.get() + o_p32, p32.data(), sizeof(PhysF32) * Kr, hipMemcpyHostToDevice, h->stream));
            HIPCHK(hipMemcpyAsync(h->ep_buf.get() + o_ls, L_schedule + t, sizeof(double) * Kr, hipMemcpyHostToDevice, h->stream));
            StatsDev* stats = h->stats2[h->sp].get();
            if (!wave_kernel) HIPCHK(hipMemsetAsync(stats, 0, sizeof(StatsDev) * (B + 1), h->stream));
            EpisodeMlpIO io;
            fill_episode_io(io, h, S);
            io.weights = d_w; io.member_a = d_ma; io.member_b = d_mb;
            io.reward = d_r + t * bn; io.done = d_d + t * bn;
            io.action = h->action.get();
            const bool ex = p.precision == DW_PRECISION_EXACT;
            if (wave_kernel) {
                auto kern = ex ? episode_mlp_wave<true> : episode_mlp_wave<false>;
                if (int rc = set_lds_limit(h, kern, lds)) return rc;
                const EpisodeMlpWaveArgs A{io, B, N, p.height, p.width, (int)Kr, p.obs_mask, (int)split, p.agent_gamma,
                                           h->L_last, make_f64(p, L_schedule[t])};
                hipLaunchKernelGGL(kern, dim3((unsigned)((B + 3) / 4)), dim3(256), lds, h->stream, A);
            } else {
                auto kern = ex ? episode_mlp<true> : episode_mlp<false>;
                if (int rc = set_lds_limit(h, kern, lds)) return rc;
                hipLaunchKernelGGL(kern, dim3((unsigned)((B + wpb - 1) / wpb)), dim3(256), lds, h->stream, io, B, N, p.height,
                                   p.width, wpb, (int)Kr, p.obs_mask, p.agent_gamma, make_f64(p, L_schedule[t]), h->L_last,
                                   (int)split);
            }
            HIPCHK(hipGetLastError());
            h->stepped = true;
            h->L_last = L_schedule[K - 1];
            h->L_per_world = false;
            t = K;
            break;
        }
        int rc = observe_into_scratch(h, L_init, 0);
        if (rc) return rc;
        hipLaunchKernelGGL(policy_mlp, dim3((unsigned)((bn + 3) / 4)), dim3(64), 0, h->stream, h->scratch.get(), d_w, d_ma, B, N,
                           0, N, h->action.get(), d_mb, split);
        HIPCHK(hipGetLastError());
        rc = launch_agents(h, h->action.get(), B, N, false, d_r + t * bn, d_d + t * bn);
        if (rc) return rc;
        rc = launch_forward(h, L_schedule[t]);
        if (rc) return rc;
        ++t;
    }
    if (reward) HIPCHK(hipMemcpyAsync(reward, d_r, sizeof(double) * K * bn, hipMemcpyDeviceToHost, h->stream));
    if (done) HIPCHK(hipMemcpyAsync(done, d_d, K * bn, hipMemcpyDeviceToHost, h->stream));
    HIPCHK(hipStreamSynchronize(h->stream));
    guard2.disarm();
    guard.disarm();
    return DW_OK;
}

int dw_lifespan_reset(dw_handle* h) {
    NEED(h, DW_EINVAL, "null handle");
    const dw_params& p = h->prm;
    HIPCHK(hipSetDevice(p.device));
    const size_t bn = (size_t)p.batch * (p.n_agents > 0 ? p.n_agents : 1);
    HIPCHK(hipMemsetAsync(h->done_at.get(), 0, sizeof(int) * p.batch, h->stream));
    HIPCHK(hipMemsetAsync(h->agents_done_at.get(), 0, sizeof(int) * bn, h->stream));
    HIPCHK(hipMemsetAsync(h->n_alive.get(), 0, sizeof(int), h->stream));
    return DW_OK;
}

int dw_lifespan_accumulate(dw_handle* h, uint32_t threshold_k) {
    NEED(h, DW_EINVAL, "null handle");
    const dw_params& p = h->prm;
    HIPCHK(hipSetDevice(p.device));
    HIPCHK(hipMemsetAsync(h->n_alive.get(), 0, sizeof(int), h->stream));
    const int n = p.batch * (p.n_agents > 0 ? p.n_agents : 1);
    hipLaunchKernelGGL(lifespan_accumulate, dim3((n + 255) / 256), dim3(256), 0, h->stream, h->stats2[h->sp].get(), h->st.get(), p.batch,
                       p.n_agents, threshold_k, h->done_at.get(), h->agents_done_at.get(), h->n_alive.get());
    HIPCHK(hipGetLastError());
    return DW_OK;
}

int dw_lifespan_download(dw_handle* h, int32_t* done_at, int32_t* agents_done_at, int32_t* n_worlds_alive) {
    NEED(h, DW_EINVAL, "null handle");
    const dw_params& p = h->prm;
    HIPCHK(hipSetDevice(p.device));
    if (done_at) HIPCHK(hipMemcpyAsync(done_at, h->done_at.get(), sizeof(int) * p.batch, hipMemcpyDeviceToHost, h->stream));
    if (agents_done_at && p.n_agents)
        HIPCHK(hipMemcpyAsync(agents_done_at, h->agents_done_at.get(), sizeof(int) * (size_t)p.batch * p.n_agents,
                              hipMemcpyDeviceToHost, h->stream));
    if (n_worlds_alive) HIPCHK(hipMemcpyAsync(n_worlds_alive, h->n_alive.get(), sizeof(int), hipMemcpyDeviceToHost, h->stream));
    HIPCHK(hipStreamSynchronize(h->stream));
    return DW_OK;
}

int dw_run_episode(dw_handle* h, int32_t nsteps, const double* L_schedule, int policy_mode,
                   const uint8_t* use_table, const int8_t* table, uint32_t threshold_k, uint8_t* world_alive,
                   uint8_t* agent_ok) {
    NEED(h && L_schedule, DW_EINVAL, "null argument");
    NEED(policy_mode >= 0 && policy_mode <= 3, DW_EINVAL, "bad policy mode");
    return run_episode_impl(h, nsteps, L_schedule, policy_mode, use_table, table, threshold_k, world_alive, agent_ok);
}

static EpisodeForm episode_form(const dw_handle* h) {
    const dw_params& p = h->prm;
    const int C = p.height * p.width, N = p.n_agents;
    if (C > 4096 || p.precision == DW_PRECISION_F64 || p.collision_mode != 0 || h->sw.no_episode_kernel)
        return EPISODE_STEPWISE;
    return C <= kEwMaxCells && N <= 64 && !h->sw.no_episode_wave ? EPISODE_WAVE : EPISODE_WORKGROUP;
}

static EpisodeForm episode_mlp_form(const dw_handle* h, size_t* lds_bytes) {
    const dw_params& p = h->prm;
    const int Cc = p.height * p.width, N = p.n_agents;
    const int wpb = worlds_per_block(Cc);
    const bool wave_kernel = Cc <= kEwMaxCells && 16 * N <= 64 && !h->sw.no_episode_wave;
    const size_t lds = wave_kernel ? episode_wave_shared_bytes() + episode_mlp_wave_world_bytes(Cc, N) * 4
                                   : episode_mlp_world_bytes(Cc, N) * wpb;
    if (lds_bytes) *lds_bytes = lds;
    const bool small = Cc <= 4096 && lds <= 160 * 1024 && p.precision != DW_PRECISION_F64 && p.collision_mode == 0 &&
                       !h->sw.no_episode_kernel;
    return !small ? EPISODE_STEPWISE : (wave_kernel ? EPISODE_WAVE : EPISODE_WORKGROUP);
}

static bool episode_kernel_applies(const dw_handle* h) { return episode_form(h) != EPISODE_STEPWISE && cur_quantised(h); }

static int launch_policy(dw_handle* h, int policy_mode, bool from_table, const unsigned char* codes, unsigned char* d_ok = nullptr) {
    const size_t bn = (size_t)h->prm.batch * h->prm.n_agents;
    if (policy_mode == DW_POLICY_TABLE || from_table) {
        hipLaunchKernelGGL(actions_from_table, dim3((unsigned)((bn + 255) / 256)), dim3(256), 0, h->stream,
                           reinterpret_cast<const signed char*>(codes), (int)bn, h->action.get());
        if (int rc = launch_policy_greedy(h, 0, nullptr, 1)) return rc;
    } else if (policy_mode == DW_POLICY_ZEROS) {
        HIPCHK(hipMemsetAsync(h->action.get(), 0, sizeof(int) * bn, h->stream));
    } else if (int rc = launch_policy_greedy(h, policy_mode == DW_POLICY_ARGMIN ? 1 : 0, nullptr, 0)) {
        return rc;
    }
    HIPCHK(hipGetLastError());
    return launch_agents(h, h->action.get(), h->prm.batch, h->prm.n_agents, false, nullptr, nullptr, d_ok);
}

static EpisodeIO episode_io(const dw_handle* h, int policy_mode, const EpisodeStaging& S, size_t t0, bool wave, bool have_use_table,
                            bool have_table) {
    using R = EpisodeStaging;
    unsigned char* dev = h->ep_buf.get();
    EpisodeIO io{};
    fill_episode_io(io, h, S);
    io.use_table = wave && !have_use_table ? nullptr : dev + S.off[R::USE_TABLE] + t0;
    io.table = wave && !have_table ? nullptr : reinterpret_cast<const signed char*>(dev + S.off[R::TABLE] + t0 * S.bn);
    io.world_alive = dev + S.off[R::WORLD_ALIVE] + t0 * S.B;
    io.agent_ok = dev + S.off[R::AGENT_OK] + t0 * S.bn;
    io.action = (h->prm.n_agents > 0 && policy_mode != kPolicySkipAgents) ? h->action.get() : nullptr;
    return io;
}

static int run_episode_stepwise(dw_handle* h, int32_t nsteps, const double* L_schedule, int policy_mode,
                                const uint8_t* use_table, const int8_t* table, uint32_t threshold_k, uint8_t* world_alive,
                                uint8_t* agent_ok, dw_world_stats* trace, WorldRows* worlds = nullptr, bool sym = false) {
    using R = EpisodeStaging;
    const dw_params& p = h->prm;
    const int N = p.n_agents, B = p.batch;
    const size_t K = (size_t)nsteps, Bz = (size_t)B, bn = Bz * N;
    const bool plain = !trace && !worlds;
    EpisodeRegions regions;
    regions.trace = trace != nullptr; regions.pairs = plain; regions.slack = 256;
    EpisodeBuffers E(h, EpisodeStaging(K, Bz, (size_t)N, regions));
    SeriesSchedule q;
    std::optional<PwTable> tab;
    if (worlds) {
        q = plan_series(SeriesSpec{nsteps, Bz, sizeof(StatsDev), 0, 0, false, false, true, false, L_schedule});
        tab.emplace(h, PwLayout(Bz, q.trows));
    }
    if (int rc = E.alloc(false)) return rc;
    if (tab)
        if (int rc = tab->alloc("the per-world constants", {tab->item()})) return rc;
    SyncOnExit guard(h->stream);
    if (int rc = E.upload(nullptr, 0, true, nullptr, table)) return rc;
    unsigned char* const d_tab = E.dev(R::TABLE);
    unsigned char* const d_wa = E.dev(R::WORLD_ALIVE);
    unsigned char* const d_ok = E.dev(R::AGENT_OK);
    unsigned char* const d_code = E.dev(R::CODE);
    StatsDev* const rows = E.dev<StatsDev>(R::TRACE);
    const int nflag = B > (int)bn ? B : (int)bn;
    const bool table_steps = use_table && !(worlds && policy_mode == DW_POLICY_ZEROS);
    auto from_table = [&](size_t t) { return policy_mode == DW_POLICY_TABLE || (table_steps && use_table[t]); };
    const bool may_pair = plain && h->plan.allow_fuse && bn && N <= kLookaheadMaxAgents && policy_mode != kPolicySkipAgents &&
                          !h->sw.no_agent_fuse;
    unsigned int* pstats = (plain && world_alive) ? E.dev<unsigned int>(R::PAIR_STATS) : nullptr;
    if (pstats && may_pair) HIPCHK(hipMemsetAsync(pstats, 0, sizeof(unsigned int) * 2 * B, h->stream));
    const int uniform_code = policy_mode == DW_POLICY_ZEROS ? 0 : (policy_mode == DW_POLICY_ARGMIN ? 0xFE : 0xFF);
    if (may_pair && policy_mode != DW_POLICY_TABLE) HIPCHK(hipMemsetAsync(d_code, uniform_code, bn, h->stream));
    const bool no_preapply = h->sw.no_agent_preapply;
    bool pre_applied = false;
    size_t c = 0;
    for (size_t t = 0; t < K; ++t) {
        if (tab && (int)t == (c ? q.chunks[c - 1].end : 0)) {
            if (int rc = tab->next_chunk(q, c, L_schedule, *worlds)) return rc;
            ++c;
        }
        const bool pair = may_pair && cur_quantised(h) && K - t >= 3;
        if (pre_applied) {
            pre_applied = false;
        } else if (bn && policy_mode != kPolicySkipAgents) {
            if (int rc = launch_policy(h, policy_mode, from_table(t), d_tab + t * bn, pair ? d_ok + t * bn : nullptr)) return rc;
        }
        if (pair) {
            const double L1 = L_schedule[t], L2 = L_schedule[t + 1];
            int rc = launch_forward_fused2(h, L1, L2, pstats, (float)threshold_k);
            if (rc) return rc;
            LookaheadArgs A;
            A.inL = h->L16[1 - h->cur].get(); A.inD = h->D16[1 - h->cur].get();
            A.outL = h->L16[h->cur].get(); A.outD = h->D16[h->cur].get();
            A.idx = h->idx.get(); A.st = h->st.get();
            A.code = reinterpret_cast<const signed char*>(from_table(t + 1) ? d_tab + (t + 1) * bn : d_code);
            A.agent_ok = d_ok + (t + 1) * bn;
            A.code_next = nullptr;
            A.agent_ok_next = nullptr;
            A.action_out = h->action.get();
            if (t + 2 < K && !no_preapply) {
                A.code_next = reinterpret_cast<const signed char*>(from_table(t + 2) ? d_tab + (t + 2) * bn : d_code);
                A.agent_ok_next = d_ok + (t + 2) * bn;
                pre_applied = true;
            }
            A.alive_t = pstats ? d_wa + t * Bz : nullptr;
            A.alive_t1 = pstats ? d_wa + (t + 1) * Bz : nullptr;
            A.pstats = pstats; A.thr = threshold_k;
            A.B = B; A.N = N; A.H = p.height; A.W = p.width; A.mask = p.obs_mask;
            A.agent_gamma = p.agent_gamma;
            A.P1 = derive_f32(p, L1); A.P2 = derive_f32(p, L2);
            A.P64 = make_f64(p, L1); A.La = L1; A.Lb = L2;
            if (p.precision == DW_PRECISION_EXACT)
                hipLaunchKernelGGL((agents_lookahead_patch<true>), dim3((unsigned)B), dim3(64), 0, h->stream, A);
            else
                hipLaunchKernelGGL((agents_lookahead_patch<false>), dim3((unsigned)B), dim3(64), 0, h->stream, A);
            HIPCHK(hipGetLastError());
            ++t;
            continue;
        }
        if (tab) {
            const size_t tr = q.row_of[t];
            if (int rc = launch_forward_pw(h, tab->lay.p32(tab->dev(), tr), tab->lay.p64(tab->dev(), tr), tab->lay.fb(tab->dev()), sym, true)) return rc;
        } else if (int rc = launch_forward(h, L_schedule[t])) {
            return rc;
        }
        hipLaunchKernelGGL(episode_flags, dim3((unsigned)((nflag + 255) / 256)), dim3(256), 0, h->stream,
                           h->stats2[h->sp].get(), h->st.get(), B, N, threshold_k, d_wa + t * Bz, d_ok + t * bn);
        if (trace)
            hipLaunchKernelGGL(episode_stats_row_pw, dim3((unsigned)((B + 255) / 256)), dim3(256), 0, h->stream,
                               h->stats2[h->sp].get(), B, rows + t * Bz);
        HIPCHK(hipGetLastError());
    }
    if (int rc = E.finish(world_alive, agent_ok, trace)) return rc;
    guard.disarm();
    return DW_OK;
}

static int check_episode_call(const dw_handle* h, int32_t nsteps, int policy_mode, const uint8_t* use_table, const int8_t* table) {
    const dw_params& p = h->prm;
    NEED(nsteps >= 1 && nsteps <= 4096, DW_EINVAL, "nsteps must be in 1..4096");
    NEED(p.precision != DW_PRECISION_F64, DW_EINVAL, "dw_run_episode supports exact and fast precision");
    NEED(p.collision_mode == 0, DW_EINVAL, "collision_mode=1 is not implemented on the device");
    NEED(h->have_state, DW_ESTATE, "no state uploaded");
    NEED(p.n_agents == 0 || h->have_agents, DW_ESTATE, "no agents uploaded");
    NEED(cur_quantised(h), DW_ESTATE, "the current state is not quantised yet; take the first step with dw_step");
    NEED(policy_mode != DW_POLICY_TABLE || table, DW_EINVAL, "DW_POLICY_TABLE needs a table");
    if (use_table && !table)
        for (int t = 0; t < nsteps; ++t) NEED(!use_table[t], DW_EINVAL, "use_table set but no table given");
    return DW_OK;
}

static int run_episode_impl(dw_handle* h, int32_t nsteps, const double* L_schedule, int policy_mode,
                            const uint8_t* use_table, const int8_t* table, uint32_t threshold_k,
                            uint8_t* world_alive, uint8_t* agent_ok, dw_world_stats* trace) {
    const dw_params& p = h->prm;
    HIPCHK(hipSetDevice(p.device));
    if (int rc = check_episode_call(h, nsteps, policy_mode, use_table, table)) return rc;
    const int C = p.height * p.width, N = p.n_agents, B = p.batch;
    const EpisodeForm form = episode_form(h);
    if (form == EPISODE_STEPWISE || (trace && form != EPISODE_WAVE))
        return run_episode_stepwise(h, nsteps, L_schedule, policy_mode, use_table, table, threshold_k, world_alive, agent_ok, trace);
    const bool wave_kernel = form == EPISODE_WAVE;
    const int wpb = worlds_per_block(C);
    const size_t world_bytes = wave_kernel ? episode_wave_world_bytes(C, N) : episode_world_bytes(C, N);
    const size_t lds = trace ? episode_wave_stats_lds_bytes(C, N)
                             : world_bytes * wpb + (wave_kernel ? episode_wave_shared_bytes() : 0);
    NEED(lds <= 160 * 1024, DW_EINVAL, "too many agents for the LDS-resident episode kernel");
    const size_t K = (size_t)nsteps;
    EpisodeRegions regions;
    regions.rows = K; regions.use_table = true; regions.trace = trace != nullptr;
    EpisodeBuffers E(h, EpisodeStaging(K, (size_t)B, (size_t)N, regions));
    if (int rc = E.alloc(E.S.fits_image())) return rc;
    PhysF32* p32 = E.p32();
    for (size_t t = 0; t < K; ++t) p32[t] = derive_f32(p, L_schedule[t]);
    SyncOnExit guard(h->stream);
    if (int rc = E.upload(L_schedule, K, true, use_table, table)) return rc;
    StatsDev* stats = h->stats2[h->sp].get();
    if (!wave_kernel) HIPCHK(hipMemsetAsync(stats, 0, sizeof(StatsDev) * (B + 1), h->stream));
    const EpisodeIO io = episode_io(h, policy_mode, E.S, 0, wave_kernel, use_table != nullptr, table && E.S.bn);
    const PhysF64 P64 = make_f64(p, L_schedule[0]);
    const dim3 grid((unsigned)((B + wpb - 1) / wpb));
    const bool ex = p.precision == DW_PRECISION_EXACT;
    if (trace) {
        auto kern = ex ? episode_wave_stats_pw<true> : episode_wave_stats_pw<false>;
        const EpisodeWaveStatsArgs A{io, E.dev<StatsDev>(EpisodeStaging::TRACE), B, N, p.height, p.width, nsteps,
                                     policy_mode, p.obs_mask, threshold_k, p.agent_gamma, P64};
        hipLaunchKernelGGL(kern, grid, dim3(256), lds, h->stream, A);
    } else if (wave_kernel) {
        auto kern = ex ? episode_wave<true> : episode_wave<false>;
        if (int rc = set_lds_limit(h, kern, lds)) return rc;
        const EpisodeWaveArgs A{io, B, N, p.height, p.width, nsteps, policy_mode, p.obs_mask, threshold_k, p.agent_gamma, P64};
        hipLaunchKernelGGL(kern, grid, dim3(256), lds, h->stream, A);
    } else {
        auto kern = ex ? episode_small<true> : episode_small<false>;
        if (int rc = set_lds_limit(h, kern, lds)) return rc;
        hipLaunchKernelGGL(kern, grid, dim3(256), lds, h->stream, io, B, N, p.height, p.width, wpb, nsteps, policy_mode,
                           p.obs_mask, p.agent_gamma, threshold_k, P64);
    }
    HIPCHK(hipGetLastError());
    episode_done(h, L_schedule[K - 1], false);
    release_unquantised(h);
    if (int rc = E.finish(world_alive, agent_ok, trace)) return rc;
    guard.disarm();
    return DW_OK;
}

int dw_run_episode_trace(dw_handle* h, int32_t nsteps, const double* L_schedule, int policy_mode,
                         const uint8_t* use_table, const int8_t* table, uint32_t threshold_k, uint8_t* world_alive,
                         uint8_t* agent_ok, dw_world_stats* trace) {
    NEED(h && L_schedule, DW_EINVAL, "null argument");
    NEED(trace, DW_EINVAL, "dw_run_episode_trace needs a trace array");
    NEED(policy_mode >= 0 && policy_mode <= 3, DW_EINVAL, "bad policy mode");
    return run_episode_impl(h, nsteps, L_schedule, policy_mode, use_table, table, threshold_k, world_alive, agent_ok, trace);
}

int dw_run_episode_ensemble(dw_handle* h, int32_t nsteps, const dw_world_params* worlds, const double* L_schedule, int policy_mode,
                            const uint8_t* use_table, const int8_t* table, uint32_t threshold_k, uint8_t* world_alive,
                            uint8_t* agent_ok) {
    NEED(h && worlds && L_schedule, DW_EINVAL, "null argument");
    NEED(policy_mode >= 0 && policy_mode <= 3, DW_EINVAL, "bad policy mode");
    const dw_params& p = h->prm;
    HIPCHK(hipSetDevice(p.device));
    if (int rc = check_episode_call(h, nsteps, policy_mode, use_table, table)) return rc;
    const int C = p.height * p.width, N = p.n_agents, B = p.batch;
    const size_t K = (size_t)nsteps, Bz = (size_t)B;
    const bool wave = episode_form(h) == EPISODE_WAVE;
    WorldRows rows_of(p, worlds, Bz, !wave);
    if (int rc = check_per_world(rows_of, worlds, L_schedule, K, Bz)) return rc;
    if (!wave)
        return run_episode_stepwise(h, nsteps, L_schedule, policy_mode, use_table, table, threshold_k, world_alive, agent_ok, nullptr,
                                    &rows_of, worlds_symmetric(worlds, Bz) && !h->sw.no_sym);
    const size_t lds = episode_wave_pw_shared_bytes() + episode_wave_pw_world_bytes(C, N) * 4;
    NEED(lds <= 160 * 1024, DW_EINVAL, "too many agents for the LDS-resident episode kernel");
    const size_t row_bytes = (sizeof(PhysF32) + sizeof(double)) * Bz;
    size_t rows = ((size_t)32 << 20) / row_bytes / kEwSeg * kEwSeg;
    rows = rows < (size_t)kEwSeg ? (size_t)kEwSeg : rows;
    rows = rows > K ? K : rows;
    EpisodeRegions regions;
    regions.rows = rows; regions.per_world = true; regions.use_table = true;
    EpisodeBuffers E(h, EpisodeStaging(K, Bz, (size_t)N, regions));
    if (int rc = E.alloc(true)) return rc;
    SyncOnExit guard(h->stream);
    PhysF64* p64 = E.S.at<PhysF64>(E.img, EpisodeStaging::P64);
    for (size_t b = 0; b < Bz; ++b) p64[b] = make_f64(rows_of.params(b), 0.0);
    const bool ex = p.precision == DW_PRECISION_EXACT;
    auto kern = ex ? episode_wave_pw<true> : episode_wave_pw<false>;
    if (int rc = set_lds_limit(h, kern, lds)) return rc;
    PhysF32* r32 = E.p32();
    for (size_t t0 = 0; t0 < K; t0 += rows) {
        const size_t kk = K - t0 < rows ? K - t0 : rows;
        if (t0) HIPCHK(hipStreamSynchronize(h->stream));
        for (size_t t = 0; t < kk; ++t) rows_of.single(L_schedule + (t0 + t) * Bz, r32 + t * Bz, nullptr);
        if (int rc = E.upload(L_schedule + t0 * Bz, kk * Bz, t0 == 0, use_table, table)) return rc;
        const EpisodeWavePwArgs A{episode_io(h, policy_mode, E.S, t0, true, use_table != nullptr, table && E.S.bn),
                                  E.dev<const PhysF64>(EpisodeStaging::P64), B, N, p.height, p.width, (int)kk, policy_mode,
                                  p.obs_mask, threshold_k, p.agent_gamma};
        hipLaunchKernelGGL(kern, dim3((unsigned)((B + 3) / 4)), dim3(256), lds, h->stream, A);
        HIPCHK(hipGetLastError());
        episode_done(h, 0.0, true);
    }
    release_unquantised(h);
    if (int rc = E.finish(world_alive, agent_ok, nullptr)) return rc;
    guard.disarm();
    return DW_OK;
}

struct CopyJobs {
    const void* src[8];
    void* dst[8];
    unsigned long long bytes[8];
    int n;
};
__global__ __launch_bounds__(256) void copy_regions(CopyJobs J) {
    const size_t stride = (size_t)gridDim.x * blockDim.x, t0 = (size_t)blockIdx.x * blockDim.x + threadIdx.x;
    for (int j = 0; j < J.n; ++j) {
        const size_t nb = J.bytes[j];
        const uint4* s16 = static_cast<const uint4*>(J.src[j]);
        uint4* d16 = static_cast<uint4*>(J.dst[j]);
        for (size_t i = t0; i < nb / 16; i += stride) d16[i] = s16[i];
        const unsigned char* s1 = static_cast<const unsigned char*>(J.src[j]);
        unsigned char* d1 = static_cast<unsigned char*>(J.dst[j]);
        for (size_t i = (nb & ~(size_t)15) + t0; i < nb; i += stride) d1[i] = s1[i];
    }
}
static int launch_copy_regions(dw_handle* h, const CopyJobs& J) {
    size_t most = 0;
    for (int j = 0; j < J.n; ++j) {
        NEED(J.src[j] && J.dst[j], DW_EINVAL, "snapshot region not allocated");
        NEED(((reinterpret_cast<uintptr_t>(J.src[j]) | reinterpret_cast<uintptr_t>(J.dst[j])) & 15) == 0, DW_EINVAL,
             "snapshot region not 16-byte aligned");
        most = J.bytes[j] > most ? J.bytes[j] : most;
    }
    if (J.n == 0 || most == 0) return DW_OK;
    size_t blocks = (most / 16 + 255) / 256;
    blocks = blocks < 1 ? 1 : (blocks > 8192 ? 8192 : blocks);
    hipLaunchKernelGGL(copy_regions, dim3((unsigned)blocks), dim3(256), 0, h->stream, J);
    HIPCHK(hipGetLastError());
    return DW_OK;
}

int dw_snapshot_save_slot(dw_handle* h, int32_t slot) {
    NEED(h, DW_EINVAL, "null handle");
    NEED(slot >= 0 && slot < DW_SNAPSHOT_SLOTS, DW_EINVAL, "snapshot slot out of range");
    const dw_params& p = h->prm;
    HIPCHK(hipSetDevice(p.device));
    NEED(h->have_state, DW_ESTATE, "no state uploaded");
    NEED(cur_quantised(h), DW_ESTATE, "the current state is an un-quantised upload; take a step first");
    dw_handle::Snapshot& sn = h->snap[slot];
    sn.valid = false;
    const size_t bn = (size_t)p.batch * p.n_agents;
    const size_t pb = sizeof(plane_t) * h->cells;
    const int rc = bn ? alloc_group(h, "a snapshot", {{sn.L, pb}, {sn.D, pb}, {sn.stats, h->stats_bytes},
                                                      {sn.idx, sizeof(int) * 2 * bn}, {sn.st, sizeof(double) * bn}})
                      : alloc_group(h, "a snapshot", {{sn.L, pb}, {sn.D, pb}, {sn.stats, h->stats_bytes}});
    if (rc) return rc;
    const bool keep_prev = h->stepped && h->unq != OWN_PREV;
    if (keep_prev)
        if (int prc = alloc_group(h, "a snapshot's previous state", {{sn.PL, pb}, {sn.PD, pb}})) return prc;
    CopyJobs J;
    J.n = 0;
    auto job = [&J](void* dst, const void* src, size_t bytes) { J.dst[J.n] = dst; J.src[J.n] = src; J.bytes[J.n] = bytes; ++J.n; };
    job(sn.L.get(), h->L16[h->cur].get(), pb);
    job(sn.D.get(), h->D16[h->cur].get(), pb);
    job(sn.stats.get(), h->stats2[h->sp].get(), h->stats_bytes);
    if (keep_prev) {
        job(sn.PL.get(), h->L16[1 - h->cur].get(), pb);
        job(sn.PD.get(), h->D16[1 - h->cur].get(), pb);
    }
    sn.stepped = h->stepped;
    sn.L_last = h->L_last;
    sn.L_per_world = h->L_per_world;
    sn.P_per_world = h->P_per_world;
    sn.unq = h->unq;
    sn.agents = bn && h->have_agents;
    if (sn.agents) {
        job(sn.idx.get(), h->idx.get(), sizeof(int) * 2 * bn);
        job(sn.st.get(), h->st.get(), sizeof(double) * bn);
    }
    if (int crc = launch_copy_regions(h, J)) return crc;
    sn.valid = true;
    return DW_OK;
}

int dw_snapshot_restore_slot(dw_handle* h, int32_t slot) {
    NEED(h, DW_EINVAL, "null handle");
    NEED(slot >= 0 && slot < DW_SNAPSHOT_SLOTS, DW_EINVAL, "snapshot slot out of range");
    const dw_params& p = h->prm;
    HIPCHK(hipSetDevice(p.device));
    const dw_handle::Snapshot& sn = h->snap[slot];
    NEED(sn.valid, DW_ESTATE, "no snapshot saved in this slot (or a later upload / dw_init_random invalidated it)");
    const size_t bn = (size_t)p.batch * p.n_agents;
    const size_t pb = sizeof(plane_t) * h->cells;
    CopyJobs J;
    J.n = 0;
    auto job = [&J](void* dst, const void* src, size_t bytes) { J.dst[J.n] = dst; J.src[J.n] = src; J.bytes[J.n] = bytes; ++J.n; };
    job(h->L16[h->cur].get(), sn.L.get(), pb);
    job(h->D16[h->cur].get(), sn.D.get(), pb);
    job(h->stats2[h->sp].get(), sn.stats.get(), h->stats_bytes);
    if (sn.agents) {
        job(h->idx.get(), sn.idx.get(), sizeof(int) * 2 * bn);
        job(h->st.get(), sn.st.get(), sizeof(double) * bn);
    }
    if (sn.stepped && sn.unq != OWN_PREV) {
        job(h->L16[1 - h->cur].get(), sn.PL.get(), pb);
        job(h->D16[1 - h->cur].get(), sn.PD.get(), pb);
    }
    if (int rc = launch_copy_regions(h, J)) return rc;
    HIPCHK(hipMemsetAsync(h->stats2[1 - h->sp].get(), 0, h->stats_bytes, h->stream));
    h->unq = sn.unq;
    h->stepped = sn.stepped;
    h->L_last = sn.L_last;
    h->L_per_world = sn.L_per_world;
    h->P_per_world = sn.P_per_world;
    return DW_OK;
}

int dw_snapshot_save(dw_handle* h) { return dw_snapshot_save_slot(h, 0); }
int dw_snapshot_restore(dw_handle* h) { return dw_snapshot_restore_slot(h, 0); }


int dw_set_stream(dw_handle* h, void* hip_stream) {
    NEED(h, DW_EINVAL, "null handle");
    HIPCHK(hipSetDevice(h->prm.device));
    HIPCHK(hipStreamSynchronize(h->stream));
    if (h->own_stream) HIPCHK(hipStreamDestroy(h->stream));
    h->stream = reinterpret_cast<hipStream_t>(hip_stream);
    h->own_stream = false;
    return DW_OK;
}

int dw_sync(dw_handle* h) {
    NEED(h, DW_EINVAL, "null handle");
    HIPCHK(hipSetDevice(h->prm.device));
    HIPCHK(hipStreamSynchronize(h->stream));
    return DW_OK;
}

int dw_timer_start(dw_handle* h) {
    NEED(h, DW_EINVAL, "null handle");
    HIPCHK(hipSetDevice(h->prm.device));
    HIPCHK(hipEventRecord(h->ev0, h->stream));
    return DW_OK;
}

int dw_timer_stop(dw_handle* h, float* elapsed_ms) {
    NEED(h && elapsed_ms, DW_EINVAL, "null argument");
    HIPCHK(hipSetDevice(h->prm.device));
    HIPCHK(hipEventRecord(h->ev1, h->stream));
    HIPCHK(hipEventSynchronize(h->ev1));
    HIPCHK(hipEventElapsedTime(elapsed_ms, h->ev0, h->ev1));
    return DW_OK;
}

int dw_device_planes(dw_handle* h, int which, void** light, void** dark) {
    NEED(h && light && dark, DW_EINVAL, "null argument");
    NEED(which == DW_STATE_CURRENT || which == DW_STATE_PREVIOUS, DW_EINVAL, "bad state selector");
    const int buf = which == DW_STATE_CURRENT ? h->cur : 1 - h->cur;
    NEED(which != DW_STATE_CURRENT || cur_quantised(h), DW_ESTATE,
         "the current state is an un-quantised upload: it has no binary16 planes before the first step");
    *light = h->L16[buf].get();
    *dark = h->D16[buf].get();
    return DW_OK;
}

int dw_kernel_info(dw_handle* h, char* buf, size_t buflen) {
    NEED(h && buf && buflen, DW_EINVAL, "null argument");
    const dw_params& p = h->prm;
    const StepPlan& pl = h->plan;
    const char* prec = p.precision == DW_PRECISION_EXACT ? "exact" : (p.precision == DW_PRECISION_FAST ? "fast" : "f64");
    static const char* const halo_name[] = {"rotate", "dpp-old", "general", "packed"};
    if (pl.kind == STEP_STREAM) {
        const StripGeom& g = pl.sgeom;
        snprintf(buf, buflen,
                 "step_stream_%s<halo=%s> wave-strip=%dx256 cells, register window + DPP neighbours, %d-row blocks in "
                 "flight%s, %d strips, grid=%d x 256 threads (4 strips each), XCD-chunked",
                 prec, halo_name[pl.halo], g.SR,
                 p.precision == DW_PRECISION_EXACT ? DW_STREAM_RB_EXACT : DW_STREAM_RB_FAST,
                 p.precision == DW_PRECISION_EXACT ? ", in-wave float64 fix-up from an LDS queue" : "", g.nstrips,
                 g.chunk * 8);
        if (pl.allow_fuse) {
            const size_t n = std::strlen(buf);
            snprintf(buf + n, buflen - n, "; dw_step_n fuses step pairs (step_stream_fused2%s%s",
                     p.precision == DW_PRECISION_EXACT ? "_exact" : "",
                     pl.seam_strips ? "_seam_pw, format buffer accesses" : (pl.fmt_planes ? "_fmt_pw, format buffer accesses" : ""));
            if (pl.seam_strips) {
                const size_t m = std::strlen(buf);
                snprintf(buf + m, buflen - m, ", seam strips: %d x %d columns + %d columns of %d row bands per wave", pl.seam_geom.ncs,
                         kSeamCols, pl.left_geom.cols_per_strip, pl.left_geom.wpr);
            }
            const size_t m = std::strlen(buf);
            snprintf(buf + m, buflen - m, ")");
        }
    } else if (pl.kind == STEP_TILED) {
        const int TR = (256 / pl.tcq) * pl.rpt;
        snprintf(buf, buflen,
                 "step_tiled<TCQ=%d,RPT=%d,%s> tile=%dx%d cells, %zu B LDS/workgroup, %d tiles, grid=%d x 256 threads, "
                 "XCD-chunked",
                 pl.tcq, pl.rpt, prec, TR, pl.tcq * 4, pl.tile_lds, pl.geom.ntiles, pl.geom.chunk * 8);
    } else {
        snprintf(buf, buflen, "step_generic<%s> one thread per cell, grid=(%d,%d) x 256 threads", prec,
                 (p.height * p.width + 255) / 256, p.batch);
    }
    {
        const size_t n = std::strlen(buf);
        snprintf(buf + n, buflen - n, pl.trace_pairs ? "; trace: step pairs" : "; trace: single steps");
    }
    {
        const size_t n = std::strlen(buf);
        snprintf(buf + n, buflen - n, pl.pw_stream ? "; per-world L: wave strips" : "; per-world L: generic");
    }
    {
        static const char* const form_name[] = {"launches per step", "workgroup (LDS)", "one wave per world"};
        const size_t n = std::strlen(buf);
        snprintf(buf + n, buflen - n, "; episode: %s; mlp episode: %s", form_name[episode_form(h)], form_name[episode_mlp_form(h)]);
    }
    {
        const size_t n = std::strlen(buf);
        snprintf(buf + n, buflen - n, "; ensemble episode: %s", episode_form(h) == EPISODE_WAVE ? "one wave per world" : "launches per step");
    }
    {
        const size_t n = std::strlen(buf);
        snprintf(buf + n, buflen - n, "; episode trace: %s", episode_form(h) == EPISODE_WAVE ? "one wave per world" : "launches per step");
    }
    if (pl.first_stream) {
        const size_t n = std::strlen(buf);
        snprintf(buf + n, buflen - n, "; first step: wave-strip=%dx256", pl.first_geom.SR);
    }
    if (h->sw.text[0]) {
        const size_t n = std::strlen(buf);
        snprintf(buf + n, buflen - n, "; switches[%s]", h->sw.text);
    }
    {
        const size_t n = std::strlen(buf);
        snprintf(buf + n, buflen - n, "; per-world constants: %s",
                 ensemble_pairs(h) ? "step pairs" : (pl.pw_stream ? "wave strips" : "generic"));
    }
    return DW_OK;
}

int dw_audit_tie_bound(dw_handle* h, double L, double out[4]) {
    NEED(h && out, DW_EINVAL, "null argument");
    const dw_params& p = h->prm;
    HIPCHK(hipSetDevice(p.device));
    NEED(h->have_state && cur_quantised(h), DW_ESTATE, "the audit needs a quantised current state");
    const StepPlan& pl = h->plan;
    int rc = ensure_scratch(h, 4 * sizeof(unsigned long long));
    if (rc) return rc;
    unsigned long long* d = reinterpret_cast<unsigned long long*>(h->scratch.get());
    HIPCHK(hipMemsetAsync(d, 0, 4 * sizeof(unsigned long long), h->stream));
    const dim3 g((unsigned)((p.height * p.width + 255) / 256), (unsigned)p.batch);
    hipLaunchKernelGGL(tie_audit, g, dim3(256), 0, h->stream, h->L16[h->cur].get(), h->D16[h->cur].get(), p.height, p.width,
                       derive_f32(p, L), make_f64(p, L), d, pl.sym_albedo && pl.kind == STEP_STREAM ? 1 : 0);
    HIPCHK(hipGetLastError());
    unsigned long long r[4];
    HIPCHK(hipMemcpyAsync(r, d, sizeof(r), hipMemcpyDeviceToHost, h->stream));
    HIPCHK(hipStreamSynchronize(h->stream));
    std::memcpy(&out[0], &r[0], sizeof(double));
    std::memcpy(&out[1], &r[1], sizeof(double));
    out[2] = (double)r[2];
    out[3] = (double)r[3];
    return DW_OK;
}

int dw_last_fixup_count(dw_handle* h, uint64_t* count) {
    NEED(h && count, DW_EINVAL, "null argument");
    HIPCHK(hipSetDevice(h->prm.device));
    std::vector<StatsDev> st((size_t)h->prm.batch + 1);
    HIPCHK(hipMemcpyAsync(st.data(), h->stats2[h->sp].get(), sizeof(StatsDev) * st.size(), hipMemcpyDeviceToHost, h->stream));
    HIPCHK(hipStreamSynchronize(h->stream));
    unsigned long long v = st[h->prm.batch].sum_l;
    for (int b = 0; b < h->prm.batch; ++b) v += st[b].reserved;
    *count = v;
    return DW_OK;
}

}
```

therldaisyworld_amd/csrc/dw_common.hpp:

```cpp
#pragma once
#include <type_traits>

#include "dw_physics.hpp"
#include "dw_types.hpp"

namespace dw {

__device__ __forceinline__ float wave_sum(float v) {
#pragma unroll
    for (int o = 32; o > 0; o >>= 1) v += __shfl_xor(v, o, 64);
    return v;
}
__device__ __forceinline__ float wave_max(float v) {
#pragma unroll
    for (int o = 32; o > 0; o >>= 1) v = fmaxf(v, __shfl_xor(v, o, 64));
    return v;
}

__device__ __forceinline__ double to_natural(double x) { return x; }
__device__ __forceinline__ double to_natural(float k) { return (double)k / 1000.0; }
__device__ __forceinline__ double to_natural(plane_t k) { return dw_permille_to_natural((double)(float)k); }
__device__ __forceinline__ float to_permille(double x) { return (float)(x * 1000.0); }
__device__ __forceinline__ float to_permille(float k) { return k; }
__device__ __forceinline__ float to_permille(plane_t k) { return (float)k; }

typedef _Float16 dw_f16x4 __attribute__((ext_vector_type(4)));
typedef unsigned int dw_u32x2 __attribute__((ext_vector_type(2)));
__device__ __forceinline__ dw_f16x4 stream_load4_raw(const plane_t* p) { return *reinterpret_cast<const dw_f16x4*>(p); }
__device__ __forceinline__ float4 widen4(const dw_f16x4& v) { return make_float4((float)v.x, (float)v.y, (float)v.z, (float)v.w); }
__device__ __forceinline__ float4 stream_load4(const plane_t* p) { return widen4(stream_load4_raw(p)); }
__device__ __forceinline__ void stream_store4(plane_t* p, const float4& v) {
    dw_u32x2 t;
    t.x = __builtin_bit_cast(unsigned int, __builtin_amdgcn_cvt_pkrtz(v.x, v.y));
    t.y = __builtin_bit_cast(unsigned int, __builtin_amdgcn_cvt_pkrtz(v.z, v.w));
    __builtin_nontemporal_store(t, reinterpret_cast<dw_u32x2*>(p));
}

typedef float dw_fmt_f32x4 __attribute__((ext_vector_type(4)));
typedef int dw_i32x4 __attribute__((ext_vector_type(4)));
__device__ dw_fmt_f32x4 dw_buf_load_fmt4(dw_i32x4 rsrc, int voff, int soff, int aux) __asm("llvm.amdgcn.raw.buffer.load.format.v4f32");
__device__ dw_f32x2 dw_buf_load_fmt2(dw_i32x4 rsrc, int voff, int soff, int aux) __asm("llvm.amdgcn.raw.buffer.load.format.v2f32");
__device__ void dw_buf_store_fmt4(dw_fmt_f32x4 v, dw_i32x4 rsrc, int voff, int soff, int aux) __asm("llvm.amdgcn.raw.buffer.store.format.v4f32");
constexpr int kBufAuxNonTemporal = 2;
constexpr int kFmtRsrcQuads = 0x00067FAC, kFmtRsrcPairs = 0x0002FFAC;
__device__ __forceinline__ dw_i32x4 fmt_plane_rsrc(const plane_t* plane, int world, unsigned int world_bytes,
                                                   int word3 = kFmtRsrcQuads) {
    const unsigned long long base = (unsigned long long)plane + (unsigned long long)world * world_bytes;
    dw_i32x4 r;
    r.x = __builtin_amdgcn_readfirstlane((int)(unsigned int)base);
    r.y = __builtin_amdgcn_readfirstlane((int)(unsigned int)(base >> 32)) & 0xffff;
    r.z = __builtin_amdgcn_readfirstlane((int)world_bytes);
    r.w = word3;
    return r;
}
__device__ __forceinline__ float4 fmt_load4(const dw_i32x4& rsrc, int voff, int soff) {
    const dw_fmt_f32x4 v = dw_buf_load_fmt4(rsrc, voff, soff, 0);
    return make_float4(v.x, v.y, v.z, v.w);
}
__device__ __forceinline__ float4 fmt_load2x2(const dw_i32x4& rsrc, int voff_a, int voff_b, int soff) {
    const dw_f32x2 a = dw_buf_load_fmt2(rsrc, voff_a, soff, 0), c = dw_buf_load_fmt2(rsrc, voff_b, soff, 0);
    return make_float4(a.x, a.y, c.x, c.y);
}
__device__ __forceinline__ void fmt_store4(const dw_i32x4& rsrc, int voff, int soff, const float4& v) {
    dw_buf_store_fmt4(dw_fmt_f32x4{v.x, v.y, v.z, v.w}, rsrc, voff, soff, kBufAuxNonTemporal);
}
__device__ __forceinline__ float4 widen4(const float4& v) {
    typedef float f2 __attribute__((ext_vector_type(2)));
    unsigned long long lo, hi;
    asm("v_pk_mov_b32 %0, %1, %1 op_sel:[0,1]" : "=v"(lo) : "v"(f2{v.x, v.y}));
    asm("v_pk_mov_b32 %0, %1, %1 op_sel:[0,1]" : "=v"(hi) : "v"(f2{v.z, v.w}));
    return make_float4(__uint_as_float((unsigned int)lo), __uint_as_float((unsigned int)(lo >> 32)),
                       __uint_as_float((unsigned int)hi), __uint_as_float((unsigned int)(hi >> 32)));
}

__device__ __forceinline__ int wrap_near(int v, int n) { return v < 0 ? v + n : (v >= n ? v - n : v); }
__device__ __forceinline__ int wrap_near2(int v, int n) { return wrap_near(wrap_near(v, n), n); }

template <typename T>
__device__ __forceinline__ void gather9(const T* __restrict__ plane, int H, int W, int r, int c,
                                        double out[9]) {
    const int ru = r == 0 ? H - 1 : r - 1, rd = r == H - 1 ? 0 : r + 1;
    const int cl = c == 0 ? W - 1 : c - 1, cr = c == W - 1 ? 0 : c + 1;
    const int rows[3] = {ru, r, rd}, cols[3] = {cl, c, cr};
#pragma unroll
    for (int a = 0; a < 3; ++a)
#pragma unroll
        for (int b = 0; b < 3; ++b) out[a * 3 + b] = to_natural(plane[(size_t)rows[a] * W + cols[b]]);
}

struct Row4 {
    float x[4];
    float h2[4];
};

__device__ __forceinline__ Row4 load_row(const float* __restrict__ lds_row_group) {
    const float4 a = *reinterpret_cast<const float4*>(lds_row_group);
    const float4 m = *reinterpret_cast<const float4*>(lds_row_group + 4);
    const float4 c = *reinterpret_cast<const float4*>(lds_row_group + 8);
    Row4 r;
    r.x[0] = m.x; r.x[1] = m.y; r.x[2] = m.z; r.x[3] = m.w;
    r.h2[0] = a.w + m.y;
    r.h2[1] = m.x + m.z;
    r.h2[2] = m.y + m.w;
    r.h2[3] = m.z + c.x;
    return r;
}

template <bool EXACT, bool SYM = false, typename F = bool>
__device__ __forceinline__ void cells4(const PhysF32& P, const Row4& upL, const Row4& miL, const Row4& dnL,
                                       const Row4& upD, const Row4& miD, const Row4& dnD, float* ol, float* od,
                                       F* tie) {
#pragma clang fp contract(off)
    using T = dw_f32x2;
    constexpr int N = Lanes<T>::N;
#pragma unroll
    for (int i = 0; i < 4; i += N) {
        auto pr = [&](const float* a) -> T { return Lanes<T>::load(a, i); };
        const T li = pr(miL.x), di = pr(miD.x);
        const T El = pr(miL.h2) + (pr(upL.x) + pr(dnL.x));
        const T Cl = pr(upL.h2) + pr(dnL.h2);
        const T Ed = pr(miD.h2) + (pr(upD.x) + pr(dnD.x));
        const T Cd = pr(upD.h2) + pr(dnD.h2);
        const GrowthT<T> g = growth_t<EXACT || kFastSplit, T, EXACT && SYM>(P, li, di, El, Cl, Ed, Cd);
        T vl, vd;
        if (EXACT) {
            F tl[N], td[N];
            if constexpr (DW_TIE_FROM_BETA || sizeof(F) == 8) {
                vl = finish_exact_beta_t<T, F>(P, li, g.gql, g.dKl, g.bl, tl);
                vd = finish_exact_beta_t<T, F>(P, di, g.gqd, g.dKd, g.bd, td);
            } else {
                vl = finish_exact_t<T>(P, li, g.gql, g.dKl, g.oml, tl);
                vd = finish_exact_t<T>(P, di, g.gqd, g.dKd, g.omd, td);
            }
#pragma unroll
            for (int e = 0; e < N; ++e) tie[i + e] = tl[e] | td[e];
        } else {
            vl = finish_fast_t<T>(li, g.dKl, g.fl);
            vd = finish_fast_t<T>(di, g.dKd, g.fd);
        }
#pragma unroll
        for (int e = 0; e < N; ++e) {
            ol[i + e] = Lanes<T>::get(vl, e);
            od[i + e] = Lanes<T>::get(vd, e);
        }
    }
}

}
```

therldaisyworld_amd/csrc/dw_plan.hpp:

```cpp
#pragma once
#include <climits>
#include <cmath>
#include <cstddef>
#include <cstdio>
#include <cstdlib>
#include <cstring>

#include "../../include/daisyworld_hip.h"
#include "dw_types.hpp"

namespace dw {

struct Switches {
    bool no_sym = false, no_pack = false, no_fuse = false, no_ring = false, no_fmt_planes = false, no_seam_strips = false,
         no_episode_kernel = false,
         no_episode_wave = false, no_agent_fuse = false, no_agent_preapply = false, first_f64 = false,
         first_generic = false, force_rescan = false, test_hooks = false;
    int pack_min_strips = -1, strip_rows = 0, tile_rpt = 0, queue_cap = -1, mismatch_cap = -1, trace_rows = 0;
    double first_slack = -1.0;
    char kernel[16] = {0};
    char text[256] = {0};
};
inline const char* test_hook(const char* name) {
    return std::getenv("DW_TEST_HOOKS") ? std::getenv(name) : nullptr;
}
inline Switches read_switches() {
    Switches w;
    auto note = [&](const char* name, const char* val) {
        const size_t n = std::strlen(w.text);
        snprintf(w.text + n, sizeof(w.text) - n, "%s%s%s%s", n ? " " : "", name, val ? "=" : "", val ? val : "");
    };
    auto flag = [&](const char* name, bool& dst) { if (std::getenv(name)) { dst = true; note(name, nullptr); } };
    auto num = [&](const char* name, int& dst, bool test) {
        if (const char* e = test ? test_hook(name) : std::getenv(name)) { dst = std::atoi(e); note(name, e); }
    };
    w.test_hooks = std::getenv("DW_TEST_HOOKS") != nullptr;
    flag("DW_NO_SYM", w.no_sym); flag("DW_NO_PACK", w.no_pack); flag("DW_NO_FUSE", w.no_fuse); flag("DW_NO_RING", w.no_ring);
    flag("DW_NO_FMT_PLANES", w.no_fmt_planes); flag("DW_NO_SEAM_STRIPS", w.no_seam_strips);
    flag("DW_NO_EPISODE_KERNEL", w.no_episode_kernel); flag("DW_NO_EPISODE_WAVE", w.no_episode_wave);
    flag("DW_NO_AGENT_FUSE", w.no_agent_fuse); flag("DW_NO_AGENT_PREAPPLY", w.no_agent_preapply);
    flag("DW_FIRST_STEP_F64", w.first_f64); flag("DW_FIRST_GENERIC", w.first_generic);
    num("DW_PACK_MIN_STRIPS", w.pack_min_strips, false); num("DW_STRIP_ROWS", w.strip_rows, false);
    num("DW_TILE_RPT", w.tile_rpt, false);
    num("DW_TEST_QUEUE_CAP", w.queue_cap, true); num("DW_TEST_MISMATCH_CAP", w.mismatch_cap, true);
    num("DW_TEST_TRACE_ROWS", w.trace_rows, true);
    if (test_hook("DW_TEST_FORCE_RESCAN")) { w.force_rescan = true; note("DW_TEST_FORCE_RESCAN", nullptr); }
    if (const char* e = test_hook("DW_TEST_FIRST_SLACK")) { w.first_slack = std::atof(e); note("DW_TEST_FIRST_SLACK", e); }
    if (const char* e = std::getenv("DW_KERNEL")) { snprintf(w.kernel, sizeof(w.kernel), "%s", e); note("DW_KERNEL", e); }
    return w;
}

inline dw_params with_world_params(dw_params p, const dw_world_params& w) {
    p.p = w.p; p.g = w.g; p.S = w.S; p.sigma = w.sigma; p.gamma = w.gamma; p.q = w.q; p.q2 = w.q2; p.dt = w.dt;
    p.albedo_bare = w.albedo_bare; p.albedo_light = w.albedo_light; p.albedo_dark = w.albedo_dark;
    p.temp_optimal = w.temp_optimal;
    return p;
}
inline dw_world_params world_params_of(const dw_params& p) {
    return dw_world_params{p.p, p.g, p.S, p.sigma, p.gamma, p.q, p.q2, p.dt, p.albedo_bare, p.albedo_light, p.albedo_dark,
                           p.temp_optimal};
}
inline bool albedo_symmetric(double bare, double light, double dark) { return (dark - bare) == -(light - bare); }
inline bool worlds_symmetric(const dw_world_params* worlds, size_t B) {
    for (size_t b = 0; b < B; ++b)
        if (!albedo_symmetric(worlds[b].albedo_bare, worlds[b].albedo_light, worlds[b].albedo_dark)) return false;
    return true;
}

inline PhysF64 make_f64(const dw_params& p, double L) {
    PhysF64 P;
    P.p = p.p; P.g = p.g; P.S = p.S; P.sigma = p.sigma; P.gamma = p.gamma; P.q = p.q; P.q2 = p.q2;
    P.dt = p.dt; P.ab = p.albedo_bare; P.al = p.albedo_light; P.ad = p.albedo_dark;
    P.To = p.temp_optimal; P.L = L;
    const double e1 = std::exp(-1.0), e2 = std::exp(-2.0);
    const double s = 1.0 + 4.0 * e1 + 4.0 * e2;
    P.w0 = 1.0 / s; P.w1 = e1 / s; P.w2 = e2 / s;
    return P;
}

inline double cbeta_host(const dw_params& p) {
    const double cbeta = p.g * p.temp_optimal * p.temp_optimal;
    return cbeta > 1e-30 ? 1.0 / std::sqrt(cbeta) : 0x1p60;
}

inline void split_hi_lo(double v, double scale, float* hi, float* lo) {
    const double h = std::nearbyint(v * scale) / scale;
    *hi = (float)h;
    *lo = (float)(v - h);
}

inline float round_up(double v) {
    const float f = (float)v;
    return (double)f < v ? std::nextafterf(f, INFINITY) : f;
}

struct EConst { double c0l, c0d; };
inline EConst e_const(const dw_params& p, double L) {
    const double To4 = std::pow(p.temp_optimal, 4), K = p.S * L / p.sigma;
    const double e0 = K * (1.0 - p.albedo_bare * p.p) / To4 - 1.0;
    return EConst{e0 + p.q2 * (p.albedo_bare * p.p - p.albedo_light) / To4,
                  e0 + p.q2 * (p.albedo_bare * p.p - p.albedo_dark) / To4};
}

struct TieChain {
    double emin, emax, vlo;
    bool admissible;
    double ew;
    double kbmax;
    double pu, safety;
};
inline TieChain tie_chain(const dw_params& p, const EConst& c, double a1, double a2, double a3, double a4, double de) {
    const double u = std::ldexp(1.0, -24), kmax = 1000.0;
    TieChain t;
    const double pos = (std::fmax(a1, 0.0) + std::fmax(a2, 0.0)) * 8 * kmax + (std::fmax(a3, 0.0) + std::fmax(a4, 0.0)) * kmax;
    const double neg = (std::fmin(a1, 0.0) + std::fmin(a2, 0.0)) * 8 * kmax + (std::fmin(a3, 0.0) + std::fmin(a4, 0.0)) * kmax;
    t.emax = std::fmax(c.c0l, c.c0d) + pos;
    t.emin = std::fmin(c.c0l, c.c0d) + neg;
    const double vmin = 1.0 + t.emin, vmax = 1.0 + t.emax;
    t.admissible = vmin > 0.02;
    t.vlo = std::fmax(vmin, 0.02);
    const double smax = std::sqrt(std::fmax(vmax, t.vlo));
    const double ymax = std::sqrt(smax);
    const double sg = smax / (smax + 1.0), et = ymax / (ymax + 1.0);
    const double re = std::fmax(std::fabs(t.emin) / t.vlo, std::fabs(t.emax) / std::fmax(vmax, t.vlo));
    const double ev = u * (1.0 + re) + de / t.vlo;
    const double eD = 3.0 * u + (0.5 * ev + 2.0 * u) * sg + (0.25 * ev + 3.0 * u) * et;
    t.ew = 4.0 * u + eD;
    t.kbmax = std::fmax(std::fabs(p.p), std::fabs(p.p - 2.0));
    t.pu = (double)(float)p.p == p.p ? 0.0 : std::fabs(p.p);
    t.safety = 1.0 + 0x1p-7;
    return t;
}

inline PhysF32 derive_f32(const dw_params& p, double L, int hb_cap = 40) {
    const double To4 = std::pow(p.temp_optimal, 4);
    const double K = p.S * L / p.sigma;
    const double dal = p.albedo_light - p.albedo_bare, dad = p.albedo_dark - p.albedo_bare;
    const double a1 = (p.q - K) * dal / (8000.0 * To4);
    const double a2 = (p.q - K) * dad / (8000.0 * To4);
    const double a3 = (-p.q + p.q2) * dal / (1000.0 * To4);
    const double a4 = (-p.q + p.q2) * dad / (1000.0 * To4);
    const EConst c0 = e_const(p, L);
    const double c0l = c0.c0l, c0d = c0.c0d;
    const double kmax = 1000.0;
    const double maxsum = std::fabs(a1) * 8 * kmax + std::fabs(a2) * 8 * kmax + std::fabs(a3) * kmax +
                          std::fabs(a4) * kmax + std::fmax(std::fabs(c0l), std::fabs(c0d));
    int hb = 23 - (int)std::ceil(std::log2(std::fmax(maxsum, 1e-30)));
    if (hb > hb_cap) hb = hb_cap;
    if (hb < 0) hb = 0;
    const double scale = std::ldexp(1.0, hb);
    PhysF32 P;
    P.hi_bits = hb;
    split_hi_lo(a1, scale, &P.a1h, &P.a1l);
    split_hi_lo(a2, scale, &P.a2h, &P.a2l);
    split_hi_lo(a3, scale, &P.a3h, &P.a3l);
    split_hi_lo(a4, scale, &P.a4h, &P.a4l);
    split_hi_lo(c0l, scale, &P.c0lh, &P.c0ll);
    float c0dl;
    split_hi_lo(c0d, scale, &P.c0dh, &c0dl);
    P.dc0l = c0dl - P.c0ll;
    P.a1 = (float)((double)P.a1h + P.a1l); P.a2 = (float)((double)P.a2h + P.a2l);
    P.a3 = (float)((double)P.a3h + P.a3l); P.a4 = (float)((double)P.a4h + P.a4l);
    P.c0ls = (float)((double)P.c0lh + P.c0ll); P.c0ds = (float)((double)P.c0dh + c0dl);
    const double kbe = cbeta_host(p);
    P.kbeta = (float)kbe;
    const PhysF64 P64 = make_f64(p, L);
    P.dw0 = (float)(p.dt * P64.w0); P.dw1 = (float)(p.dt * P64.w1); P.dw2 = (float)(p.dt * P64.w2);
    P.p = (float)p.p; P.ck = p.dt != 0.0 ? (float)(0.001 / p.dt) : 0.f;
    P.ngamma = (float)(-p.gamma);
    const double u = std::ldexp(1.0, -24);
    const double lo_mag = std::ldexp(1.0, -(hb + 1)) * 18.0 * kmax + std::ldexp(1.0, -(hb + 1));
    const double de_abs = 6.0 * u * lo_mag + 1e-9;
    const TieChain t = tie_chain(p, c0, a1, a2, a3, a4, de_abs);
    auto e_over_D2 = [&](double e) {
        const double v = std::fmax(1.0 + e, t.vlo), sv = std::sqrt(v), yv = std::sqrt(sv);
        const double D = kbe * (yv + 1.0) * (sv + 1.0);
        return std::fabs(e) / (D * D);
    };
    const double Ae = 2.0 * de_abs * std::fmax(e_over_D2(t.emin), e_over_D2(t.emax));
    double A0 = t.safety * (kmax * std::fabs(p.dt) * t.kbmax * Ae + 2e-6);
    if (!t.admissible) A0 = 1.0;
    const double eA = t.safety * 13.0 * u;
    const double eK0d = t.safety * (6.0 * std::fabs(p.p) + t.pu + t.kbmax + 8.0 * std::fabs(p.gamma)) * u;
    const double eK1d = t.safety * ((6.0 * std::fabs(p.p) + t.pu) * u + t.kbmax * (u + 2.0 * t.ew));
    P.tie_lo = (float)(0.5 - A0);
    if ((double)P.tie_lo > 0.5 - A0) P.tie_lo = std::nextafterf(P.tie_lo, -INFINITY);
    P.eA = round_up(eA);
    const float eK0 = round_up(eK0d), eK1 = round_up(eK1d);
    P.eK0s = p.dt < 0.0 ? eK0 : -eK0;
    P.eK1s = p.dt < 0.0 ? eK1 : -eK1;
    P.neK1s = -P.eK1s;
// ... 195 lines not shown
```

therldaisyworld_amd/csrc/dw_step_fused.hpp:

```cpp
#pragma once
#include <type_traits>
#include "dw_step_stream.hpp"
#include "dw_types.hpp"

namespace dw {


template <typename TI>
__device__ inline unsigned int exact1_word(const TI* __restrict__ pL, const TI* __restrict__ pD, int H, int W,
                                           int r, int c, const PhysF64& Pa) {
    const int rr = wrap_near2(r, H), cc = wrap_near2(c, W);
    const int ru = rr == 0 ? H - 1 : rr - 1, rd = rr == H - 1 ? 0 : rr + 1;
    const int cl = cc == 0 ? W - 1 : cc - 1, cr = cc == W - 1 ? 0 : cc + 1;
    const int rows[3] = {ru, rr, rd}, cols[3] = {cl, cc, cr};
    unsigned int w1[9];
#pragma unroll
    for (int x = 0; x < 3; ++x)
#pragma unroll
        for (int y = 0; y < 3; ++y) {
            const size_t o = (size_t)rows[x] * W + cols[y];
            w1[x * 3 + y] = (unsigned)(float)pL[o] | ((unsigned)(float)pD[o] << 16);
        }
    const NewCoverF64 s1 = cell_f64_lean(Pa, w1);
    return (unsigned)dw_round3_k(s1.nl) | ((unsigned)dw_round3_k(s1.nd) << 16);
}

template <typename TI>
__device__ inline void exact2_cell(const TI* __restrict__ pL, const TI* __restrict__ pD, int H, int W, int r,
                                   int c, const PhysF64& Pa, const PhysF64& Pb, float& kl, float& kd) {
    unsigned int w2[9];
#pragma unroll
    for (int a = 0; a < 3; ++a)
#pragma unroll
        for (int e = 0; e < 3; ++e) {
            int rr = r + a - 1, cc = c + e - 1;
            rr = rr < 0 ? rr + H : (rr >= H ? rr - H : rr);
            cc = cc < 0 ? cc + W : (cc >= W ? cc - W : cc);
            const int ru = rr == 0 ? H - 1 : rr - 1, rd = rr == H - 1 ? 0 : rr + 1;
            const int cl = cc == 0 ? W - 1 : cc - 1, cr = cc == W - 1 ? 0 : cc + 1;
            const int rows[3] = {ru, rr, rd}, cols[3] = {cl, cc, cr};
            unsigned int w1[9];
#pragma unroll
            for (int x = 0; x < 3; ++x)
#pragma unroll
                for (int y = 0; y < 3; ++y) {
                    const size_t o = (size_t)rows[x] * W + cols[y];
                    w1[x * 3 + y] = (unsigned)(float)pL[o] | ((unsigned)(float)pD[o] << 16);
                }
            const NewCoverF64 s1 = cell_f64_lean(Pa, w1);
            w2[a * 3 + e] = (unsigned)dw_round3_k(s1.nl) | ((unsigned)dw_round3_k(s1.nd) << 16);
        }
    const NewCoverF64 s2 = cell_f64_lean(Pb, w2);
    kl = (float)dw_round3_k(s2.nl);
    kd = (float)dw_round3_k(s2.nd);
}

template <int MODE, bool EXACT, bool PACK = false, bool STATS = false, bool SYM = false, typename TI = plane_t,
          typename TO = plane_t, bool TRACE = false, bool FMT = false, int SEAM = kSeamNone>
__device__ __forceinline__ void fused2_body(const TI* __restrict__ inL, const TI* __restrict__ inD,
                                            TO* __restrict__ outL, TO* __restrict__ outD, const FusedGeom& G,
                                            const PhysF32& P1_, const PhysF32& P2_, const PhysF64& P64,
                                            const double& La, const double& Lb,
                                            unsigned long long* __restrict__ zero_me, int zero_n,
                                            unsigned int* __restrict__ pstats = nullptr, float thr_hi = 0.f,
                                            StatsDev* __restrict__ trace = nullptr, int trace_rescan = 0) {
    constexpr bool ROT = MODE == kFusedRot, RING = MODE == kFusedRing;
    static_assert(!RING || !PACK, "the ring exchange is written for un-packed worlds");
    static_assert(!TRACE || (!PACK && !STATS && !RING), "the trace form exists for un-packed overlapped / rotating strips");
    static_assert(SEAM == kSeamNone || FMT, "the seam strips exist for the format-access kernel");
    static_assert(!FMT || (MODE == kFusedOvl && !EXACT && !PACK && !STATS && !TRACE), "the format-access form exists for the plain float32 kernel on overlapped strips");
    __shared__ float s_edge[RING ? 2 * 4 * 8 : 1];
    __shared__ uint4 s_queue[EXACT ? 4 * kWaveQueueCap * 3 : 1];
    __shared__ unsigned int s_mm[EXACT ? 4 * kMismatchCap : 1];
    const int bid = blockIdx.x;
    const int wg = (bid & 7) * G.chunk + (bid >> 3);
    if (wg >= G.nwg) return;
    const int tid = threadIdx.x, wv = tid >> 6, lane = tid & 63;
    if (wg == 0)
        for (int i = tid; i < zero_n; i += 256) zero_me[i] = 0ull;
    const int s = RING ? wg : __builtin_amdgcn_readfirstlane(wg * 4 + wv);
    if (!RING && s >= G.nstrips) return;
    uint4* q = s_queue + (EXACT ? wv * kWaveQueueCap * 3 : 0);
    unsigned int* mm = s_mm + (EXACT ? wv * kMismatchCap : 0);
    const int spw = SEAM == kSeamLeft ? (G.nrs + G.wpr - 1) / G.wpr : G.nrs * G.ncs;
    const int b = s / spw;
    const int sw = s - b * spw;
    const int rs = SEAM == kSeamLeft ? sw * G.wpr : sw / G.ncs, cs = SEAM == kSeamLeft ? G.ncs : sw - rs * G.ncs;
    const int r0 = rs * G.SR;
    const int nr = min(G.SR, G.H - r0);
    const int band_g = SEAM == kSeamLeft ? min(lane / G.lpw, G.wpr - 1) : 0;
    const int band_j = SEAM == kSeamLeft ? min(lane - band_g * G.lpw, G.lpw - 1) : 0;
    const int band_rs = SEAM == kSeamLeft ? min(rs + band_g, G.nrs - 1) : 0;
    const int band_dr = SEAM == kSeamLeft ? (band_rs - rs) * G.SR : 0;
    const int band_nr = SEAM == kSeamLeft ? min(G.SR, G.H - band_rs * G.SR) : 0;
    const int pw = PACK ? lane / G.lpw : 0, pj = PACK ? lane - pw * G.lpw : 0;
    const int lsrc = PACK ? (pj == 0 ? lane + G.lpw - 1 : lane - 1) : 0;
    const int rsrc = PACK ? (pj == G.lpw - 1 ? lane - (G.lpw - 1) : lane + 1) : 0;
    auto world_off = [&](int lc) -> size_t {
        return (size_t)(PACK ? min(b * G.wpr + min((lc >> 2) / G.lpw, G.wpr - 1), G.B - 1) : b) * G.H * G.W;
    };
    const size_t woff = world_off(4 * lane);
    const int c00 = ROT ? 0 : (RING ? 256 * __builtin_amdgcn_readfirstlane(wv)
                                    : (SEAM == kSeamStrip ? cs * kSeamCols : (SEAM == kSeamLeft ? cs * kSeamCols - 4 : cs * 248 - 4)));
    int col = PACK ? 4 * pj : c00 + 4 * (SEAM == kSeamLeft ? band_j : lane);
    col = col < 0 ? col + G.W : col;
    col = col >= G.W ? col - G.W : col;
    int col_b = col + 2;
    if (SEAM == kSeamStrip && lane == 63) col_b = c00 == 0 ? G.W - 2 : c00 - 2;
    const bool writes = SEAM == kSeamStrip ? lane < 63
                      : SEAM == kSeamLeft ? (lane < G.wpr * G.lpw && rs + band_g < G.nrs && band_j >= 1 && band_j <= G.lpw - 2)
                      : PACK ? (pw < G.wpr && b * G.wpr + pw < G.B)
                             : ((ROT || RING) ? true : (lane >= 1 && lane <= 62 && cs * 248 + 4 * (lane - 1) < G.W));
    bool need1[4] = {true, true, true, true};
    if (PACK) { need1[0] = need1[1] = need1[2] = need1[3] = writes; }
    if (EXACT && !ROT && !RING) {
        const bool wl = __builtin_amdgcn_update_dpp(0, writes ? 1 : 0, kDppWaveShr1, 0xf, 0xf, false) != 0;
        const bool wr = __builtin_amdgcn_update_dpp(0, writes ? 1 : 0, kDppWaveShl1, 0xf, 0xf, false) != 0;
        need1[0] = writes || wl;
        need1[1] = writes;
        need1[2] = writes;
        need1[3] = writes || wr;
    }
    constexpr bool LANE_BOOLS = PACK || (STATS && MODE == kFusedOvl);
    using TieT = std::conditional_t<LANE_BOOLS, bool, unsigned long long>;
    TieT need1m[4], writes_m;
    if constexpr (LANE_BOOLS) {
        for (int i = 0; i < 4; ++i) need1m[i] = need1[i];
        writes_m = writes;
    } else {
        for (int i = 0; i < 4; ++i) need1m[i] = lane_mask(need1[i]);
        writes_m = lane_mask(writes);
    }
    const TI* pL = inL + woff;
    const TI* pD = inD + woff;

    dw_i32x4 fmt_inL, fmt_inD, fmt_outL, fmt_outD;
    int fmt_col = 0, fmt_row = 0, fmt_col_b = 0;
    if constexpr (FMT) {
        const unsigned int world_bytes = (unsigned int)(G.H * G.W) * 2u;
        fmt_inL = fmt_plane_rsrc(inL, b, world_bytes, SEAM == kSeamStrip ? kFmtRsrcPairs : kFmtRsrcQuads);
        fmt_inD = fmt_plane_rsrc(inD, b, world_bytes, SEAM == kSeamStrip ? kFmtRsrcPairs : kFmtRsrcQuads);
        fmt_outL = fmt_plane_rsrc(outL, b, world_bytes);
        fmt_outD = fmt_plane_rsrc(outD, b, world_bytes);
        fmt_col = col * 2;
        fmt_col_b = col_b * 2;
        fmt_row = G.W * 2;
    }
    struct RawIn { std::conditional_t<FMT, float4, dw_f16x4> l, d; };
    auto load_raw = [&](int rr) -> RawIn {
        RawIn w;
        if constexpr (SEAM == kSeamLeft) {
            int lr = min(rr + band_dr, r0 + band_dr + band_nr + 1);
            lr = lr < 0 ? lr + G.H : lr;
            lr = lr >= G.H ? lr - G.H : lr;
            w.l = fmt_load4(fmt_inL, fmt_col + lr * fmt_row, 0);
            w.d = fmt_load4(fmt_inD, fmt_col + lr * fmt_row, 0);
            return w;
        }
        rr = min(rr, r0 + nr + 1);
        rr = rr < 0 ? rr + G.H : rr;
        rr = rr >= G.H ? rr - G.H : rr;
        if constexpr (SEAM == kSeamStrip) {
            w.l = fmt_load2x2(fmt_inL, fmt_col, fmt_col_b, rr * fmt_row);
            w.d = fmt_load2x2(fmt_inD, fmt_col, fmt_col_b, rr * fmt_row);
        } else if constexpr (FMT) {
            w.l = fmt_load4(fmt_inL, fmt_col, rr * fmt_row);
            w.d = fmt_load4(fmt_inD, fmt_col, rr * fmt_row);
        } else {
            w.l = stream_load4_raw(pL + (size_t)rr * G.W + col);
            w.d = stream_load4_raw(pD + (size_t)rr * G.W + col);
        }
        return w;
    };
    auto pin_edge_sums = [&](Row4& L, Row4& D) {
        asm volatile("" : "+v"(L.h2[0]), "+v"(L.h2[3]), "+v"(D.h2[0]), "+v"(D.h2[3]));
    };
    auto nbrs = [&](const float4& v, float& a, float& c) {
        if (PACK) { a = __shfl(v.w, lsrc, 64); c = __shfl(v.x, rsrc, 64); }
        else if (ROT || SEAM == kSeamStrip) { a = dpp_mov_nb<kDppWaveRor1>(v.w); c = dpp_mov_nb<kDppWaveRol1>(v.x); }
        else { a = dpp_mov_nb<kDppWaveShr1>(v.w); c = dpp_mov_nb<kDppWaveShl1>(v.x); }
    };
    auto to_rows4 = [&](const float4& l, const float4& d, Row4& L, Row4& D) {
        float a, c;
        nbrs(l, a, c);
        L = make_row(l, a, c);
        nbrs(d, a, c);
        D = make_row(d, a, c);
    };
    int ring_par = 0;
    auto rows_ring = [&](const float4* v, Row4* const* out, auto NC) {
        constexpr int n = decltype(NC)::value;
        float* mine = s_edge + (ring_par * 4 + wv) * 8;
        if (lane == 63) {
#pragma unroll
            for (int i = 0; i < n; ++i) mine[i] = v[i].w;
        }
        if (lane == 0) {
#pragma unroll
            for (int i = 0; i < n; ++i) mine[4 + i] = v[i].x;
        }
        __syncthreads();
        const float* lw = s_edge + (ring_par * 4 + ((wv + 3) & 3)) * 8;
        const float* rw = s_edge + (ring_par * 4 + ((wv + 1) & 3)) * 8 + 4;
#pragma unroll
        for (int i = 0; i < n; ++i) {
            const float a = dpp_mov<kDppWaveShr1>(lw[i], v[i].w);
            const float c = dpp_mov<kDppWaveShl1>(rw[i], v[i].x);
            *out[i] = make_row(v[i], a, c);
        }
        ring_par ^= 1;
    };
    unsigned int nq = 0;
#ifndef DW_PIN_CONSTS
#define DW_PIN_CONSTS -1
#endif
    PhysF32 P1 = P1_, P2 = P2_;
    constexpr int PIN = DW_PIN_CONSTS < 0 ? (MODE == kFusedOvl ? 14 : (MODE == kFusedRing ? 8 : 0)) : DW_PIN_CONSTS;
    if constexpr (EXACT && PIN != 0 && !STATS && !PACK) {
        if constexpr ((PIN & 1) != 0) asm volatile("" : "+v"(P1.c0l), "+v"(P2.c0l));
        if constexpr ((PIN & 2) != 0) { asm volatile("" : "+v"(P1.pck)); P2.pck = P1.pck; }
        if constexpr ((PIN & 4) != 0) { asm volatile("" : "+v"(P1.eKb)); P2.eKb = P1.eKb; }
        if constexpr ((PIN & 8) != 0) { asm volatile("" : "+v"(P1.gt)); P2.gt = P1.gt; }
// ... 72 lines not shown
            const unsigned long long eq = __builtin_amdgcn_fcmpf(sm, thr_hi + 1.0f, 1 ) & writes_mask;
            if (__builtin_expect(eq != 0ull, 0)) {
                float m = 0.f;
#pragma unroll
                for (int i = 0; i < 4; ++i) m = fmaxf(m, tie_lane(tie[i]) ? 0.f : fmaxf(ol[i], od[i]));
                st_x1 = fmaxf(st_x1, in_mask(eq) ? m : 0.f);
            }
        }
    };
    const TieT use2[4] = {writes_m, writes_m, writes_m, writes_m};

    unsigned int nmm = 0;
    bool redo = false;
    const int flush_at = G.qcap >> 1;
    auto world_of = [&](int lc) -> int {
        return PACK ? min(b * G.wpr + min((lc >> 2) / G.lpw, G.wpr - 1), G.B - 1) : b;
    };
    auto grid_rc = [&](int lrow, int lc, int& gr, int& gc) {
        gr = r0 - 2 + lrow;
        gr = gr < 0 ? gr + G.H : (gr >= G.H ? gr - G.H : gr);
        gc = c00 + lc;
        gc = gc < 0 ? gc + G.W : (gc >= G.W ? gc - G.W : gc);
    };
    auto locate = [&](int lrow, int lc, size_t& wo, int& gr, int& gc) -> bool {
        grid_rc(lrow, lc, gr, gc);
        wo = world_off(lc);
        if (!PACK) return true;
        const int pwc = (lc >> 2) / G.lpw;
        gc = lc - pwc * G.W;
        return pwc < G.wpr && b * G.wpr + pwc < G.B;
    };
    auto is_output = [&](int lrow, int lc) -> bool {
        if (lrow < 2 || lrow > nr + 1) return false;
        if (PACK) return (lc >> 2) / G.lpw < G.wpr && b * G.wpr + (lc >> 2) / G.lpw < G.B;
        if (ROT || RING) return true;
        const int ln = lc >> 2;
        return lc >= 4 && lc < 252 && cs * 248 + 4 * (ln - 1) < G.W;
    };
    auto sweep_queue = [&]() {
        if (nq > (unsigned)G.qcap) redo = true;
        if (!redo && nq) {
            wait_row_stores_before_patching();
            const PhysF64* p64 = &P64;
            const double* pLa = &La;
            const double* pLb = &Lb;
            asm volatile("" : "+s"(p64), "+s"(pLa), "+s"(pLb));
            PhysF64 Pe = *p64;
            const double la = *pLa, lb = *pLb;
            for (unsigned int base = 0; base < nq; base += 64) {
                const unsigned int e = base + lane;
                bool mism = false;
                unsigned int where = 0;
                if (e < nq) {
                    const uint4 e0 = q[e * 3], e1 = q[e * 3 + 1], e2 = q[e * 3 + 2];
                    const unsigned int w[9] = {unpack_ld(e0.z), unpack_ld(e0.w), unpack_ld(e1.x),
                                               unpack_ld(e1.y), unpack_ld(e1.z), unpack_ld(e1.w),
                                               unpack_ld(e2.x), unpack_ld(e2.y), unpack_ld(e2.z)};
                    Pe.L = e0.x == 1u ? la : lb;
                    const NewCoverF64 o = cell_f64_lean(Pe, w);
                    const unsigned int kl = (unsigned)dw_round3_k(o.nl), kd = (unsigned)dw_round3_k(o.nd);
                    where = e0.y;
                    if (TRACE && (e0.x != 1u || is_output((int)(where >> 16), (int)(where & 0xffffu)))) {
                        const unsigned int f32v = unpack_ld(e2.w);
                        const float pl = (float)(f32v & 0xffffu), pd = (float)(f32v >> 16);
                        if (e0.x == 1u) {
                            tr_fix_l1 += (float)kl - pl;
                            tr_fix_d1 += (float)kd - pd;
                            tr_x1 = fmaxf(tr_x1, (float)(kl > kd ? kl : kd));
                        } else {
                            tr_fix_l2 += (float)kl - pl;
                            tr_fix_d2 += (float)kd - pd;
                            trace_patch2(pl, (float)kl);
                            trace_patch2(pd, (float)kd);
                        }
                    }
                    if (e0.x == 1u) {
                        mism = (kl | (kd << 16)) != unpack_ld(e2.w);
                        if (STATS && is_output((int)(where >> 16), (int)(where & 0xffffu))) {
                            const unsigned int mx = kl > kd ? kl : kd;
                            if (PACK) atomicMax(&pstats[2 * world_of((int)(where & 0xffffu))], mx);
                            else st_x1 = fmaxf(st_x1, (float)mx);
                        }
                    } else {
                        int gr, gc;
                        size_t wo;
                        locate((int)(where >> 16), (int)(where & 0xffffu), wo, gr, gc);
                        const size_t off = wo + (size_t)gr * G.W + gc;
                        outL[off] = (TO)(float)kl;
                        outD[off] = (TO)(float)kd;
                    }
                }
                const unsigned long long mask = lane_mask(mism);
                if (mism) {
                    const unsigned int slot = nmm + __builtin_amdgcn_mbcnt_hi((unsigned)(mask >> 32),
                                                                             __builtin_amdgcn_mbcnt_lo((unsigned)mask, 0u));
                    if (slot < (unsigned)G.mcap) mm[slot] = where;
                }
                nmm += (unsigned)__popcll(mask);
            }
            __builtin_amdgcn_fence(__ATOMIC_RELEASE, "wavefront");
            __builtin_amdgcn_wave_barrier();
        }
        nq = 0;
    };

    Row4 IL[3], ID[3], SL[3], SD[3];
    {
        const RawIn p0 = load_raw(r0 - 2), p1 = load_raw(r0 - 1), p2 = load_raw(r0);
        if constexpr (RING) {
            const float4 va[4] = {widen4(p0.l), widen4(p0.d), widen4(p1.l), widen4(p1.d)};
            const float4 vb[2] = {widen4(p2.l), widen4(p2.d)};
            Row4* const oa[4] = {&IL[0], &ID[0], &IL[1], &ID[1]};
            Row4* const ob[2] = {&IL[2], &ID[2]};
            rows_ring(va, oa, std::integral_constant<int, 4>{});
            rows_ring(vb, ob, std::integral_constant<int, 2>{});
        } else {
            to_rows4(widen4(p0.l), widen4(p0.d), IL[0], ID[0]);
            to_rows4(widen4(p1.l), widen4(p1.d), IL[1], ID[1]);
            to_rows4(widen4(p2.l), widen4(p2.d), IL[2], ID[2]);
        }
    }
    using U0 = std::integral_constant<int, 0>;
    using U1 = std::integral_constant<int, 1>;
    using U2 = std::integral_constant<int, 2>;
    auto iter = [&](auto U, auto D1, auto D2, int j, auto ST, auto MINE) {
        constexpr int u = decltype(U)::value;
        constexpr bool do1 = decltype(D1)::value, do2 = decltype(D2)::value;
        constexpr bool st_on = STATS && decltype(ST)::value;
        RawIn nx;
        if (do1) nx = load_raw(r0 + j);
        __builtin_amdgcn_sched_barrier(0);
        float l1[4], d1[4], l2[4], d2[4];
        TieT tie1[4], tie2[4];
        float sm1 = 0.f, sm2 = 0.f;
        if (do2)
            row_cells(P2, SL[u], SL[(u + 1) % 3], SL[(u + 2) % 3], SD[u], SD[(u + 1) % 3], SD[(u + 2) % 3], l2, d2, tie2,
                      use2, st_on ? &sm2 : nullptr);
        if (do1)
            row_cells(P1, IL[(u + 2) % 3], IL[u], IL[(u + 1) % 3], ID[(u + 2) % 3], ID[u], ID[(u + 1) % 3], l1, d1, tie1,
                      need1m, st_on ? &sm1 : nullptr);
        if (do2) {
            row_queue(SL[u], SL[(u + 1) % 3], SL[(u + 2) % 3], SD[u], SD[(u + 1) % 3], SD[(u + 2) % 3], l2, d2, tie2, 2,
                      j - 2);
            if (st_on) stats_step2(sm2);
            if constexpr (TRACE) trace_step2(l2, d2);
            if constexpr (SEAM == kSeamLeft) {
                if (writes && j - 4 < band_nr) {
                    const int voff = fmt_col + (r0 + band_dr + j - 4) * fmt_row;
                    fmt_store4(fmt_outL, voff, 0, make_float4(l2[0], l2[1], l2[2], l2[3]));
                    fmt_store4(fmt_outD, voff, 0, make_float4(d2[0], d2[1], d2[2], d2[3]));
                }
            } else if constexpr (FMT) {
                if (writes) {
                    fmt_store4(fmt_outL, fmt_col, (r0 + j - 4) * fmt_row, make_float4(l2[0], l2[1], l2[2], l2[3]));
                    fmt_store4(fmt_outD, fmt_col, (r0 + j - 4) * fmt_row, make_float4(d2[0], d2[1], d2[2], d2[3]));
                }
            } else if (writes) {
                const size_t off = woff + (size_t)(r0 + j - 4) * G.W + col;
                stream_store4(outL + off, make_float4(l2[0], l2[1], l2[2], l2[3]));
                stream_store4(outD + off, make_float4(d2[0], d2[1], d2[2], d2[3]));
            }
        }
        if (do1) {
            row_queue(IL[(u + 2) % 3], IL[u], IL[(u + 1) % 3], ID[(u + 2) % 3], ID[u], ID[(u + 1) % 3], l1, d1, tie1, 1, j);
            if (st_on) stats_step1(sm1, l1, d1, tie1, j >= 2 && j <= nr + 1);
            if constexpr (TRACE) {
                if (decltype(MINE)::value || (j >= 2 && j <= nr + 1)) trace_step1(l1, d1, tie1);
            }
            if constexpr (RING) {
                const float4 v[4] = {make_float4(l1[0], l1[1], l1[2], l1[3]), make_float4(d1[0], d1[1], d1[2], d1[3]),
                                     widen4(nx.l), widen4(nx.d)};
                Row4* const o[4] = {&SL[u], &SD[u], &IL[(u + 2) % 3], &ID[(u + 2) % 3]};
                rows_ring(v, o, std::integral_constant<int, 4>{});
            } else {
                to_rows4(make_float4(l1[0], l1[1], l1[2], l1[3]), make_float4(d1[0], d1[1], d1[2], d1[3]), SL[u], SD[u]);
                __builtin_amdgcn_sched_barrier(0);
                to_rows4(widen4(nx.l), widen4(nx.d), IL[(u + 2) % 3], ID[(u + 2) % 3]);
                if (!PACK) pin_edge_sums(IL[(u + 2) % 3], ID[(u + 2) % 3]);
            }
        }
    };
    using Yes = std::true_type;
    using No = std::false_type;
    iter(U1{}, Yes{}, No{}, 1, Yes{}, No{});
    iter(U2{}, Yes{}, No{}, 2, Yes{}, No{});
    iter(U0{}, Yes{}, No{}, 3, Yes{}, No{});
    const int jend = nr + 2;
    const int jloop = TRACE ? jend - 1 : jend;
    int j = 4;
    for (; j + 2 <= jloop; j += 3) {
        iter(U1{}, Yes{}, Yes{}, j, Yes{}, Yes{});
        iter(U2{}, Yes{}, Yes{}, j + 1, Yes{}, Yes{});
        iter(U0{}, Yes{}, Yes{}, j + 2, Yes{}, Yes{});
        if (EXACT && !STATS && __builtin_expect(nq >= (unsigned)flush_at, 0)) sweep_queue();
        if (CHEAP && st_sure1 && st_c2w >= (unsigned int)G.sure_need) { j += 3; break; }
    }
    if constexpr (CHEAP) {
        for (; j + 2 <= jend; j += 3) {
            iter(U1{}, Yes{}, Yes{}, j, No{}, No{});
            iter(U2{}, Yes{}, Yes{}, j + 1, No{}, No{});
            iter(U0{}, Yes{}, Yes{}, j + 2, No{}, No{});
        }
    }
    if (j <= jend) { iter(U1{}, Yes{}, Yes{}, j, Yes{}, No{}); ++j; }
    if (j <= jend) { iter(U2{}, Yes{}, Yes{}, j, Yes{}, No{}); ++j; }
    if constexpr (TRACE) {
        if (j <= jend) { iter(U0{}, Yes{}, Yes{}, j, Yes{}, No{}); ++j; }
    }
    if (j % 3 == 1) iter(U1{}, No{}, Yes{}, j, Yes{}, No{});
    else if (j % 3 == 2) iter(U2{}, No{}, Yes{}, j, Yes{}, No{});
    else iter(U0{}, No{}, Yes{}, j, Yes{}, No{});

    if (EXACT) {
        PhysF64 Pa = P64, Pb = P64;
        Pa.L = La;
        Pb.L = Lb;
        if (RING) {
            wait_row_stores_before_patching();
            __syncthreads();
        }
        sweep_queue();
        if (nmm > (unsigned)G.mcap) redo = true;
        if (RING) {
            wait_row_stores_before_patching();
            __syncthreads();
        }
        if (!redo) {
            unsigned int* s1 = reinterpret_cast<unsigned int*>(q);
            for (unsigned int m0 = 0; m0 < nmm; m0 += 2) {
                if constexpr (TRACE) wait_row_stores_before_patching();
                __builtin_amdgcn_wave_barrier();
                {
                    const unsigned int mi = lane / 25u, t = lane - mi * 25u;
                    if (lane < 50 && m0 + mi < nmm) {
                        const unsigned int where = mm[m0 + mi];
                        const int lrow = (int)(where >> 16) + (int)(t / 5u) - 2;
                        const int lcm = (int)(where & 0xffffu), dx5 = (int)(t % 5u) - 2;
                        if (PACK) {
                            const size_t wo = world_off(lcm);
                            s1[lane] = exact1_word(inL + wo, inD + wo, G.H, G.W, r0 - 2 + lrow,
                                                   lcm - ((lcm >> 2) / G.lpw) * G.W + dx5, Pa);
                        } else {
                            s1[lane] = exact1_word(pL, pD, G.H, G.W, r0 - 2 + lrow, c00 + lcm + dx5, Pa);
                        }
                    }
                }
                __builtin_amdgcn_fence(__ATOMIC_RELEASE, "wavefront");
                __builtin_amdgcn_wave_barrier();
                __builtin_amdgcn_fence(__ATOMIC_ACQUIRE, "wavefront");
                {
                    const unsigned int mi = lane / 9u, t = lane - mi * 9u;
                    if (lane < 18 && m0 + mi < nmm) {
                        const unsigned int where = mm[m0 + mi];
                        const int dy = (int)(t / 3u) - 1, dx = (int)(t % 3u) - 1;
                        const int lrow = (int)(where >> 16) + dy;
                        int lc = (int)(where & 0xffffu) + dx;
                        if (PACK) {
                            const int lcm = (int)(where & 0xffffu), base = ((lcm >> 2) / G.lpw) * G.W;
                            lc = base + (lcm - base + dx + G.W) % G.W;
                        } else if (ROT) {
                            lc = (lc + 256) & 255;
                        }
                        if (is_output(lrow, lc)) {
                            unsigned int w2[9];
#pragma unroll
                            for (int a = 0; a < 3; ++a)
#pragma unroll
                                for (int e = 0; e < 3; ++e) w2[a * 3 + e] = s1[mi * 25u + (unsigned)((1 + dy + a) * 5 + (1 + dx + e))];
                            const NewCoverF64 o = cell_f64_lean(Pb, w2);
                            int gr, gc;
                            size_t wo;
                            locate(lrow, lc, wo, gr, gc);
                            const size_t off = wo + (size_t)gr * G.W + gc;
                            if constexpr (TRACE) {
                                const float ol_ = (float)__builtin_bit_cast(TO, __hip_atomic_load(reinterpret_cast<const unsigned short*>(outL + off),
                                                                                                  __ATOMIC_RELAXED, __HIP_MEMORY_SCOPE_AGENT));
                                const float od_ = (float)__builtin_bit_cast(TO, __hip_atomic_load(reinterpret_cast<const unsigned short*>(outD + off),
                                                                                                  __ATOMIC_RELAXED, __HIP_MEMORY_SCOPE_AGENT));
                                const float nl_ = (float)dw_round3_k(o.nl), nd_ = (float)dw_round3_k(o.nd);
                                bool dup = false;
                                if (mi == 1u) {
                                    const unsigned int w0 = mm[m0];
                                    const int dr = lrow - (int)(w0 >> 16);
                                    int dc = lc - (int)(w0 & 0xffffu);
                                    dc = dc < 0 ? -dc : dc;
                                    if (ROT) dc = min(dc, 256 - dc);
                                    dup = dr >= -1 && dr <= 1 && dc <= 1;
                                }
                                if (!dup) {
                                    tr_fix_l2 += nl_ - ol_;
                                    tr_fix_d2 += nd_ - od_;
                                }
                                trace_patch2(ol_, nl_);
                                trace_patch2(od_, nd_);
                            }
                            outL[off] = (TO)(float)dw_round3_k(o.nl);
                            outD[off] = (TO)(float)dw_round3_k(o.nd);
                        }
                    }
                }
            }
        } else {
            const int ncol = ROT ? 256 : (RING ? 258 : 248);
            if constexpr (TRACE) {
                tr_l1 = tr_d1 = tr_l2 = tr_d2 = dw_f32x2(0.f);
                tr_m1 = tr_m2 = 0;
                tr_fix_l1 = tr_fix_d1 = tr_fix_l2 = tr_fix_d2 = 0.f;
                tr_x1 = tr_new2 = tr_low2 = 0.f;
            }
            for (int i = lane; i < nr * ncol; i += 64) {
                const int lrow = 2 + i / ncol, lc = (ROT ? 0 : (RING ? -1 : 4)) + i % ncol;
                if (!is_output(lrow, lc)) continue;
                int gr, gc;
                size_t wo;
                locate(lrow, lc, wo, gr, gc);
                float kl, kd;
                exact2_cell(inL + wo, inD + wo, G.H, G.W, gr, gc, Pa, Pb, kl, kd);
                const size_t off = wo + (size_t)gr * G.W + gc;
                outL[off] = (TO)kl;
                outD[off] = (TO)kd;
                if constexpr (TRACE) {
                    const unsigned int w1 = exact1_word(inL + wo, inD + wo, G.H, G.W, gr, gc, Pa);
                    const float l1 = (float)(w1 & 0xffffu), d1 = (float)(w1 >> 16);
                    tr_fix_l1 += l1;
                    tr_fix_d1 += d1;
                    tr_x1 = fmaxf(tr_x1, fmaxf(l1, d1));
                    tr_fix_l2 += kl;
                    tr_fix_d2 += kd;
                    tr_new2 = fmaxf(tr_new2, fmaxf(kl, kd));
                }
                if (STATS) {
                    const unsigned int w1 = exact1_word(inL + wo, inD + wo, G.H, G.W, gr, gc, Pa);
                    atomicMax(&pstats[2 * world_of(lc)], (w1 & 0xffffu) > (w1 >> 16) ? (w1 & 0xffffu) : (w1 >> 16));
                }
            }
            st_m1 = 0.f;
            st_x1 = 0.f;
            st_c2 = 0;
            st_c2w = 0;
        }
        st_nmm = nmm;
    }
    if constexpr (TRACE) {
        const bool own = writes && !redo;
        float l1 = own ? tr_l1.x + tr_l1.y : 0.f, d1 = own ? tr_d1.x + tr_d1.y : 0.f;
        float l2 = own ? tr_l2.x + tr_l2.y : 0.f, d2 = own ? tr_d2.x + tr_d2.y : 0.f;
        float m1 = own ? __int_as_float(tr_m1) : 0.f, m2 = own ? __int_as_float(tr_m2) : 0.f;
        if (EXACT) {
            l1 += tr_fix_l1; d1 += tr_fix_d1; l2 += tr_fix_l2; d2 += tr_fix_d2;
            m1 = fmaxf(m1, tr_x1);
        }
        m1 = wave_max(m1);
        m2 = wave_max(m2);
        if (EXACT) {
            m2 = fmaxf(m2, wave_max(tr_new2));
            const float lw = wave_max(tr_low2);
            if (__builtin_expect(!redo && (lw >= m2 || trace_rescan), 0)) {
                wait_row_stores_before_patching();
                float m = 0.f;
                for (int k0 = 0; k0 < nr; k0 += 8) {
                    unsigned long long wl[8], wd[8];
#pragma unroll
                    for (int jj = 0; jj < 8; ++jj) {
                        const int kk = min(k0 + jj, nr - 1);
                        const size_t off = woff + (size_t)(r0 + kk) * G.W + col;
                        wl[jj] = __hip_atomic_load(reinterpret_cast<const unsigned long long*>(outL + off), __ATOMIC_RELAXED,
                                                   __HIP_MEMORY_SCOPE_AGENT);
                        wd[jj] = __hip_atomic_load(reinterpret_cast<const unsigned long long*>(outD + off), __ATOMIC_RELAXED,
                                                   __HIP_MEMORY_SCOPE_AGENT);
                    }
#pragma unroll
                    for (int jj = 0; jj < 8; ++jj) {
                        const float4 fl = widen4(__builtin_bit_cast(dw_f16x4, wl[jj])), fd = widen4(__builtin_bit_cast(dw_f16x4, wd[jj]));
                        m = fmaxf(m, fmaxf(fmaxf(fmaxf(fl.x, fl.y), fmaxf(fl.z, fl.w)), fmaxf(fmaxf(fd.x, fd.y), fmaxf(fd.z, fd.w))));
                    }
                }
                m2 = wave_max(writes ? m : 0.f);
            }
        }
        l1 = wave_sum(l1); d1 = wave_sum(d1); l2 = wave_sum(l2); d2 = wave_sum(d2);
        if (lane == 0) {
            StatsDev* const t1 = trace + b;
            StatsDev* const t2 = t1 + G.B;
            atomicMax(&t1->max_k, (unsigned int)m1);
            atomicAdd(&t1->sum_l, (unsigned long long)l1);
            atomicAdd(&t1->sum_d, (unsigned long long)d1);
            atomicMax(&t2->max_k, (unsigned int)m2);
            atomicAdd(&t2->sum_l, (unsigned long long)l2);
            atomicAdd(&t2->sum_d, (unsigned long long)d2);
        }
    }
    if (STATS) {
        if (PACK) {
            float m = st_m1;
            unsigned int c = st_c2;
            if ((G.lpw & (G.lpw - 1)) == 0) {
                for (int o = G.lpw >> 1; o > 0; o >>= 1) {
                    m = fmaxf(m, __shfl_xor(m, o, 64));
                    c += (unsigned int)__shfl_xor((int)c, o, 64);
                }
            } else {
                for (int o = 1; o < G.lpw; ++o) {
                    const int src = min(lane + o, 63);
                    m = fmaxf(m, __shfl(st_m1, src, 64));
                    c += (unsigned int)__shfl((int)st_c2, src, 64);
                }
            }
            c = c > 9u * st_nmm ? c - 9u * st_nmm : 0u;
            if (pj == 0 && writes) {
                atomicMax(&pstats[2 * (b * G.wpr + pw)], (unsigned int)m);
                if (c) atomicAdd(&pstats[2 * (b * G.wpr + pw) + 1], c);
            }
        } else {
            const float mf = wave_max(st_m1), mx = wave_max(st_x1);
            const float m = (EXACT && !(mf > thr_hi + 1.0f)) ? mx : mf;
            unsigned int c = st_c2w;
            c = c > 9u * st_nmm ? c - 9u * st_nmm : 0u;
            if (lane == 0) {
                atomicMax(&pstats[2 * b], (unsigned int)m);
                if (c) atomicAdd(&pstats[2 * b + 1], c);
            }
        }
    }
}

#ifndef DW_FUSED_FAST_WAVES
#define DW_FUSED_FAST_WAVES 4
#endif
template <int MODE, bool PACK, bool STATS>
constexpr int fused_fast_waves() { return ((MODE == kFusedRing && STATS) || PACK) ? 3 : DW_FUSED_FAST_WAVES; }
template <int MODE, bool PACK = false, bool STATS = false>
__global__ __launch_bounds__(256)
__attribute__((amdgpu_waves_per_eu(fused_fast_waves<MODE, PACK, STATS>(), fused_fast_waves<MODE, PACK, STATS>())))
void step_stream_fused2(const plane_t* __restrict__ inL, const plane_t* __restrict__ inD,
                                                          plane_t* __restrict__ outL, plane_t* __restrict__ outD,
                                                          FusedGeom G, PhysF32 P1, PhysF32 P2,
                                                          unsigned long long* __restrict__ zero_me, int zero_n,
                                                          unsigned int* __restrict__ pstats, float thr_hi) {
    const PhysF64 dummy{};
    const double zero = 0.0;
    fused2_body<MODE, false, PACK, STATS>(inL, inD, outL, outD, G, P1, P2, dummy, zero, zero, zero_me, zero_n, pstats, thr_hi);
}

template <int MODE>
__global__ __launch_bounds__(256) __attribute__((amdgpu_waves_per_eu(DW_FUSED_FAST_WAVES, DW_FUSED_FAST_WAVES)))
void step_stream_fused2_fmt_pw(const plane_t* __restrict__ inL, const plane_t* __restrict__ inD,
                               plane_t* __restrict__ outL, plane_t* __restrict__ outD, FusedGeom G, PhysF32 P1, PhysF32 P2,
                               unsigned long long* __restrict__ zero_me, int zero_n) {
    const PhysF64 dummy{};
    const double zero = 0.0;
    fused2_body<MODE, false, false, false, false, plane_t, plane_t, false, true>(inL, inD, outL, outD, G, P1, P2, dummy, zero,
                                                                                  zero, zero_me, zero_n);
}

__global__ __launch_bounds__(256) __attribute__((amdgpu_waves_per_eu(DW_FUSED_FAST_WAVES, DW_FUSED_FAST_WAVES)))
void step_stream_fused2_seam_pw(const plane_t* __restrict__ inL, const plane_t* __restrict__ inD,
                                plane_t* __restrict__ outL, plane_t* __restrict__ outD, FusedGeom G, PhysF32 P1, PhysF32 P2,
                                unsigned long long* __restrict__ zero_me, int zero_n) {
    const PhysF64 dummy{};
    const double zero = 0.0;
    fused2_body<kFusedOvl, false, false, false, false, plane_t, plane_t, false, true, kSeamStrip>(inL, inD, outL, outD, G, P1, P2, dummy,
                                                                                                 zero, zero, zero_me, zero_n);
}
__global__ __launch_bounds__(256) __attribute__((amdgpu_waves_per_eu(DW_FUSED_FAST_WAVES, DW_FUSED_FAST_WAVES)))
void step_stream_fused2_left_pw(const plane_t* __restrict__ inL, const plane_t* __restrict__ inD,
                                plane_t* __restrict__ outL, plane_t* __restrict__ outD, FusedGeom G, PhysF32 P1, PhysF32 P2,
                                unsigned long long* __restrict__ zero_me, int zero_n) {
    const PhysF64 dummy{};
    const double zero = 0.0;
    fused2_body<kFusedOvl, false, false, false, false, plane_t, plane_t, false, true, kSeamLeft>(inL, inD, outL, outD, G, P1, P2, dummy,
                                                                                                zero, zero, zero_me, zero_n);
}

#ifndef DW_EXACT_PACK_WAVES
#define DW_EXACT_PACK_WAVES 3
#endif
template <int MODE, bool PACK, bool STATS>
constexpr int fused_exact_waves() {
    return (PACK && STATS) || (STATS && MODE == kFusedRing) ? 2 : (PACK ? DW_EXACT_PACK_WAVES : 3);
}
struct FusedExactArgs {
    const plane_t* inL; const plane_t* inD; plane_t* outL; plane_t* outD;
    FusedGeom G;
    PhysF32 P1; PhysLumF32 lum2;
    unsigned long long* zero_me; int zero_n;
    unsigned int* pstats; float thr_hi;
    PhysF64 P64; double La; double Lb;
};

template <int MODE, bool PACK = false, bool STATS = false, bool SYM = false>
__global__ __launch_bounds__(256)
__attribute__((amdgpu_waves_per_eu(fused_exact_waves<MODE, PACK, STATS>(), fused_exact_waves<MODE, PACK, STATS>())))
void step_stream_fused2_exact(FusedExactArgs A) {
    const FusedExactArgs& cold = kernarg_struct<FusedExactArgs>();
    const PhysF32 P2 = with_lum(A.P1, A.lum2);
    fused2_body<MODE, true, PACK, STATS, SYM>(A.inL, A.inD, A.outL, A.outD, A.G, A.P1, P2, cold.P64, cold.La, cold.Lb, A.zero_me,
                                             A.zero_n, A.pstats, A.thr_hi);
}

#ifndef DW_TRACE_FAST_WAVES
#define DW_TRACE_FAST_WAVES 3
#endif
#ifndef DW_TRACE_EXACT_WAVES
#define DW_TRACE_EXACT_WAVES 2
#endif
template <int MODE>
__global__ __launch_bounds__(256) __attribute__((amdgpu_waves_per_eu(DW_TRACE_FAST_WAVES, DW_TRACE_FAST_WAVES)))
void trace_pair_fast(const plane_t* __restrict__ inL, const plane_t* __restrict__ inD, plane_t* __restrict__ outL,
                     plane_t* __restrict__ outD, FusedGeom G, PhysF32 P1, PhysF32 P2,
                     unsigned long long* __restrict__ zero_me, int zero_n, StatsDev* __restrict__ trace) {
    const PhysF64 dummy{};
    const double zero = 0.0;
    fused2_body<MODE, false, false, false, false, plane_t, plane_t, true>(inL, inD, outL, outD, G, P1, P2, dummy, zero, zero,
                                                                           zero_me, zero_n, nullptr, 0.f, trace, 0);
}

struct TraceExactArgs {
    FusedExactArgs F;
    StatsDev* trace;
    int rescan;
};

template <int MODE, bool SYM = false>
__global__ __launch_bounds__(256) __attribute__((amdgpu_waves_per_eu(DW_TRACE_EXACT_WAVES, DW_TRACE_EXACT_WAVES)))
void trace_pair_exact(TraceExactArgs A) {
    const FusedExactArgs& cold = kernarg_struct<TraceExactArgs>().F;
    const PhysF32 P2 = with_lum(A.F.P1, A.F.lum2);
    fused2_body<MODE, true, false, false, SYM, plane_t, plane_t, true>(A.F.inL, A.F.inD, A.F.outL, A.F.outD, A.F.G, A.F.P1, P2,
                                                                       cold.P64, cold.La, cold.Lb, A.F.zero_me, A.F.zero_n,
                                                                       nullptr, 0.f, A.trace, A.rescan);
}

}
```

Baseline: 826.0 billion.

## Fuse the final step pair of even runs and defer unfused tail replay

```diff
diff --git a/therldaisyworld_amd/csrc/dw_api.hip b/therldaisyworld_amd/csrc/dw_api.hip
--- a/therldaisyworld_amd/csrc/dw_api.hip
+++ b/therldaisyworld_amd/csrc/dw_api.hip
@@ -78,6 +78,8 @@
     bool have_state = false;
     bool stepped = false;
     double L_last = 0.0;
+    bool tail_deferred = false;
+    double tail_L[2] = {0.0, 0.0};
     bool L_per_world = false;
     bool P_per_world = false;
     DevBuf<int> idx;
@@ -471,6 +473,7 @@
     h->sp = 1 - h->sp;
     h->unq = h->unq == OWN_CUR ? OWN_PREV : OWN_NONE;
     h->stepped = stepped;
+    h->tail_deferred = false;
     h->L_last = L;
     h->L_per_world = per_world;
     h->P_per_world = per_world && per_world_constants;
@@ -511,6 +514,16 @@
     step_done(h, L, true);
     return DW_OK;
 }
+
+static int settle(dw_handle* h) {
+    if (!h->tail_deferred) return DW_OK;
+    HIPCHK(hipSetDevice(h->prm.device));
+    h->tail_deferred = false;
+    h->cur = 1 - h->cur;
+    if (int rc = launch_forward(h, h->tail_L[0])) return rc;
+    return launch_forward(h, h->tail_L[1]);
+}
+#define SETTLE(h) do { if (int settle_rc_ = settle(h)) return settle_rc_; } while (0)
 
 static int launch_forward_pw(dw_handle* h, const PhysF32* row32, const PhysF64* row64, const FirstStepBound* rowfb, bool sym,
                              bool constants) {
@@ -598,7 +611,7 @@
 }
 
 static int launch_forward_fused2(dw_handle* h, double L1, double L2, unsigned int* pstats = nullptr,
-                                 float thr_hi = 0.f, StatsDev* trace = nullptr) {
+                                 float thr_hi = 0.f, StatsDev* trace = nullptr, bool last = false) {
     const dw_params& p = h->prm;
     const StepPlan& pl = h->plan;
     const bool exact = p.precision == DW_PRECISION_EXACT;
@@ -624,6 +637,16 @@
             hipLaunchKernelGGL((trace_pair_fast<MODE>), grid, dim3(256), 0, h->stream, inL, inD, o.L, o.D, g, P1, P2, o.zero_me,
                                o.zero_n, trace);
         });
+    } else if (last && pl.seam_strips) {
+        const FusedGeom &gs = pl.seam_geom, &gl = pl.left_geom;
+        hipLaunchKernelGGL(step_stream_fused2_seam_last_pw, dim3((unsigned)gs.chunk * 8u), dim3(256), 0, h->stream, inL, inD, o.L,
+                           o.D, gs, P1, P2, o.zero_me, o.zero_n, o.stats);
+        if (gl.nstrips)
+            hipLaunchKernelGGL(step_stream_fused2_left_last_pw, dim3((unsigned)gl.chunk * 8u), dim3(256), 0, h->stream, inL, inD,
+                               o.L, o.D, gl, P1, P2, o.zero_me, 0, o.stats);
+    } else if (last) {
+        hipLaunchKernelGGL((step_stream_fused2_fmt_last_pw<kFusedOvl>), grid, dim3(256), 0, h->stream, inL, inD, o.L, o.D, g, P1,
+                           P2, o.zero_me, o.zero_n, o.stats);
     } else if (pl.seam_strips && !pstats && !exact) {
         const FusedGeom &gs = pl.seam_geom, &gl = pl.left_geom;
         hipLaunchKernelGGL(step_stream_fused2_seam_pw, dim3((unsigned)gs.chunk * 8u), dim3(256), 0, h->stream, inL, inD, o.L, o.D,
@@ -653,6 +676,11 @@
     }
     HIPCHK(hipGetLastError());
     step_done(h, L2, false);
+    if (last) {
+        h->tail_deferred = true;
+        h->tail_L[0] = L1;
+        h->tail_L[1] = L2;
+    }
     return DW_OK;
 }
 
@@ -696,6 +724,7 @@
     h->unq = unq;
     h->have_state = true;
     h->stepped = false;
+    h->tail_deferred = false;
     for (auto& sn : h->snap) sn.valid = false;
 }
 
@@ -838,6 +867,7 @@
 
 int dw_set_params(dw_handle* h, const dw_params* p) {
     NEED(h, DW_EINVAL, "null handle");
+    SETTLE(h);
     int rc = check_params(p);
     if (rc) return rc;
     const dw_params& o = h->prm;
@@ -919,6 +949,7 @@
 
 int dw_upload_agents(dw_handle* h, const int32_t* indices, const double* states) {
     NEED(h, DW_EINVAL, "null handle");
+    SETTLE(h);
     const dw_params& p = h->prm;
     HIPCHK(hipSetDevice(p.device));
     const size_t bn = (size_t)p.batch * p.n_agents;
@@ -940,6 +971,7 @@
 
 int dw_download_agents(dw_handle* h, int32_t* indices, double* states) {
     NEED(h, DW_EINVAL, "null handle");
+    SETTLE(h);
     const dw_params& p = h->prm;
     HIPCHK(hipSetDevice(p.device));
     const size_t bn = (size_t)p.batch * p.n_agents;
@@ -975,6 +1007,7 @@
     NEED(h->have_state, DW_ESTATE, "no state");
     HIPCHK(hipSetDevice(h->prm.device));
     NEED(which == DW_STATE_CURRENT || which == DW_STATE_PREVIOUS, DW_EINVAL, "bad state selector");
+    if (which == DW_STATE_PREVIOUS) SETTLE(h);
     NEED(which == DW_STATE_CURRENT || h->stepped, DW_ESTATE, "no previous state before the first step");
     const int buf = which == DW_STATE_CURRENT ? h->cur : 1 - h->cur;
     const bool unq = (which == DW_STATE_CURRENT && h->unq == OWN_CUR) || (which == DW_STATE_PREVIOUS && h->unq == OWN_PREV);
@@ -1026,6 +1059,7 @@
 int dw_download_grid(dw_handle* h, double L_init, double* grid7) {
     NEED(h && grid7, DW_EINVAL, "null argument");
     NEED(h->have_state, DW_ESTATE, "no state");
+    SETTLE(h);
     NEED_SHARED_L(h, "dw_download_grid");
     HIPCHK(hipSetDevice(h->prm.device));
     const size_t bytes = sizeof(double) * 7 * h->cells;
@@ -1042,6 +1076,7 @@
                        double* temp_effective) {
     NEED(h, DW_EINVAL, "null handle");
     NEED(h->have_state, DW_ESTATE, "no state");
+    SETTLE(h);
     NEED_SHARED_CONSTANTS(h, "dw_download_caches");
     HIPCHK(hipSetDevice(h->prm.device));
     const size_t n = h->cells;
@@ -1065,6 +1100,7 @@
 int dw_reduce_temperature(dw_handle* h, double L, dw_temp_stats* per_world) {
     NEED(h && per_world, DW_EINVAL, "null argument");
     NEED(h->have_state, DW_ESTATE, "no state");
+    SETTLE(h);
     NEED_SHARED_CONSTANTS(h, "dw_reduce_temperature");
     static_assert(sizeof(dw_temp_stats) == sizeof(TempStatsDev), "temperature record layout");
     HIPCHK(hipSetDevice(h->prm.device));
@@ -1079,6 +1115,7 @@
 
 int dw_update_agents(dw_handle* h, const int32_t* action, int32_t action_b, int32_t action_n) {
     NEED(h && action, DW_EINVAL, "null argument");
+    SETTLE(h);
     HIPCHK(hipSetDevice(h->prm.device));
     int rc = stage_host_actions(h, action, action_b, action_n);
     if (rc) return rc;
@@ -1087,6 +1124,7 @@
 
 int dw_step(dw_handle* h, const int32_t* action, int32_t action_b, int32_t action_n, double L) {
     NEED(h, DW_EINVAL, "null handle");
+    if (action || h->prm.n_agents) SETTLE(h);
     HIPCHK(hipSetDevice(h->prm.device));
     if (action) {
         int rc = stage_host_actions(h, action, action_b, action_n);
@@ -1099,6 +1137,7 @@
 
 int dw_step_device_actions(dw_handle* h, double L) {
     NEED(h, DW_EINVAL, "null handle");
+    SETTLE(h);
     HIPCHK(hipSetDevice(h->prm.device));
     int rc = launch_agents(h, h->action.get(), h->prm.batch, h->prm.n_agents);
     if (rc) return rc;
@@ -1107,6 +1146,7 @@
 
 int dw_upload_actions(dw_handle* h, const int32_t* action) {
     NEED(h && action, DW_EINVAL, "null argument");
+    SETTLE(h);
     HIPCHK(hipSetDevice(h->prm.device));
     const size_t bn = (size_t)h->prm.batch * h->prm.n_agents;
     if (bn) {
@@ -1118,6 +1158,7 @@
 
 int dw_download_actions(dw_handle* h, int32_t* action) {
     NEED(h && action, DW_EINVAL, "null argument");
+    SETTLE(h);
     HIPCHK(hipSetDevice(h->prm.device));
     const size_t bn = (size_t)h->prm.batch * h->prm.n_agents;
     if (bn) HIPCHK(hipMemcpyAsync(action, h->action.get(), sizeof(int) * bn, hipMemcpyDeviceToHost, h->stream));
@@ -1134,6 +1175,7 @@
     auto advance = [&]() { L += dL; L = L > max_L ? max_L : L; L = L < min_L ? min_L : L; };
     int s0 = 0;
     h->fused_launches = 0;
+    if (use_device_actions || (h->prm.height * h->prm.width <= 4096 && episode_form(h) != EPISODE_STEPWISE)) SETTLE(h);
     if (!use_device_actions && nsteps >= 1 && h->have_state && !cur_quantised(h)) {
         int rc = launch_forward(h, L);
         if (rc) return rc;
@@ -1155,22 +1197,28 @@
         *L_io = L;
         return DW_OK;
     }
-    if (!use_device_actions && h->plan.allow_fuse && h->have_state && nsteps - s0 >= 3) {
+    const bool defer = !use_device_actions && h->plan.fmt_planes && !h->sw.no_deferred_tail && nsteps - s0 >= 2 &&
+                       (nsteps - s0) % 2 == 0;
+    if (!use_device_actions && h->plan.allow_fuse && h->have_state && (nsteps - s0 >= 3 || defer)) {
         drop_unquantised_previous(h);
-        HIPCHK(hipEventRecord(h->evf0, h->stream));
-        int launched = 0;
-        while (nsteps - s0 >= 3) {
+        auto pair = [&](bool last) {
             const double L1 = L;
             advance();
             const double L2 = L;
             advance();
-            int rc = launch_forward_fused2(h, L1, L2);
-            if (rc) return rc;
             s0 += 2;
+            return launch_forward_fused2(h, L1, L2, nullptr, 0.f, nullptr, last);
+        };
+        HIPCHK(hipEventRecord(h->evf0, h->stream));
+        int launched = 0;
+        while (nsteps - s0 >= (defer ? 4 : 3)) {
+            if (int rc = pair(false)) return rc;
             launched += 1;
         }
         HIPCHK(hipEventRecord(h->evf1, h->stream));
         h->fused_launches = launched;
+        if (defer)
+            if (int rc = pair(true)) return rc;
     }
     for (int s = s0; s < nsteps; ++s) {
         int rc;
@@ -1305,6 +1353,7 @@
 static int run_series(dw_handle* h, int32_t nsteps, const double* L_schedule, dw_world_stats* trace, dw_temp_stats* temps,
                       bool always_even, bool may_pair, SeriesForm form = SHARED_L, const dw_world_params* worlds = nullptr) {
     const bool pw = form != SHARED_L;
+    SETTLE(h);
     NEED(nsteps >= 0, DW_EINVAL, "nsteps < 0");
     if (nsteps == 0) return DW_OK;
     NEED(h->have_state, DW_ESTATE, "no state uploaded (call dw_upload_state_* or dw_init_random)");
@@ -1374,6 +1423,7 @@
 int dw_forward_f64(dw_handle* h, const double* light, const double* dark, double L, double* grid7,
                    double* temps, double* betas, double* growth, double* temp_effective) {
     NEED(h && light && dark && grid7, DW_EINVAL, "null argument");
+    SETTLE(h);
     const dw_params& p = h->prm;
     HIPCHK(hipSetDevice(p.device));
     const size_t n = h->cells;
@@ -1427,6 +1477,7 @@
 
 int dw_conv3x3_f64(dw_handle* h, const double* plane, const double kernel[9], double* out) {
     NEED(h && plane && kernel && out, DW_EINVAL, "null argument");
+    SETTLE(h);
     const dw_params& p = h->prm;
     HIPCHK(hipSetDevice(p.device));
     const size_t n = h->cells;
@@ -1449,6 +1500,7 @@
 
 int dw_stage_f64(dw_handle* h, int stage, const double* in, double* out, double L, const double kernel[9]) {
     NEED(h && in && out, DW_EINVAL, "null argument");
+    SETTLE(h);
     NEED(stage >= kStageAlbedo && stage <= kStageGrowth, DW_EINVAL, "bad stage %d", stage);
     NEED(kernel || stage > kStageDensity, DW_EINVAL, "the stencil stages need their 3x3 kernel");
     const dw_params& p = h->prm;
@@ -1476,6 +1528,7 @@
 
 int dw_get_obs(dw_handle* h, double L_init, double* obs) {
     NEED(h, DW_EINVAL, "null handle");
+    SETTLE(h);
     const dw_params& p = h->prm;
     HIPCHK(hipSetDevice(p.device));
     const size_t bn = (size_t)p.batch * p.n_agents;
@@ -1492,6 +1545,7 @@
 int dw_env_step(dw_handle* h, const int32_t* action, int32_t action_b, int32_t action_n, double L, double* obs,
                 double* reward, uint8_t* done) {
     NEED(h, DW_EINVAL, "null handle");
+    SETTLE(h);
     const dw_params& p = h->prm;
     HIPCHK(hipSetDevice(p.device));
     const size_t bn = (size_t)p.batch * p.n_agents;
@@ -1536,6 +1590,7 @@
 
 int dw_get_reward_done(dw_handle* h, double* reward, uint8_t* done) {
     NEED(h, DW_EINVAL, "null handle");
+    SETTLE(h);
     const dw_params& p = h->prm;
     HIPCHK(hipSetDevice(p.device));
     const int bn = p.batch * p.n_agents;
@@ -1576,6 +1631,7 @@
 
 int dw_policy_greedy(dw_handle* h, int mode) {
     NEED(h, DW_EINVAL, "null handle");
+    SETTLE(h);
     const dw_params& p = h->prm;
     HIPCHK(hipSetDevice(p.device));
     const int bn = p.batch * p.n_agents;
@@ -1589,6 +1645,7 @@
 
 int dw_policy_per_agent(dw_handle* h, const int32_t* agent_mode) {
     NEED(h && agent_mode, DW_EINVAL, "null argument");
+    SETTLE(h);
     const dw_params& p = h->prm;
     HIPCHK(hipSetDevice(p.device));
     const int bn = p.batch * p.n_agents;
@@ -1660,6 +1717,7 @@
 int dw_policy_mlp(dw_handle* h, const double* params, int32_t n_params, int32_t agent_begin, int32_t agent_end,
                   double L_init) {
     NEED(h && params, DW_EINVAL, "null argument");
+    SETTLE(h);
     HIPCHK(hipSetDevice(h->prm.device));
     NEED(n_params == 63 * 16 + 16 * 32 + 32 * 9, DW_EINVAL, "the MLP policy has 1808 parameters (63-16-32-9), got %d", n_params);
     return policy_mlp_impl(h, params, 1, nullptr, agent_begin, agent_end, L_init);
@@ -1668,6 +1726,7 @@
 int dw_policy_mlp_population(dw_handle* h, const double* params, int32_t n_members, const int32_t* world_member,
                              int32_t agent_begin, int32_t agent_end, double L_init) {
     NEED(h && params && world_member, DW_EINVAL, "null argument");
+    SETTLE(h);
     HIPCHK(hipSetDevice(h->prm.device));
     NEED(n_members >= 1, DW_EINVAL, "n_members < 1");
     return policy_mlp_impl(h, params, n_members, world_member, agent_begin, agent_end, L_init);
@@ -1677,6 +1736,7 @@
                        const int32_t* member_a, const int32_t* member_b, int32_t split, double L_init, double* reward,
                        uint8_t* done) {
     NEED(h && L_schedule, DW_EINVAL, "null argument");
+    SETTLE(h);
     const dw_params& p = h->prm;
     HIPCHK(hipSetDevice(p.device));
     NEED(nsteps >= 1 && nsteps <= 4096, DW_EINVAL, "nsteps must be in 1..4096");
@@ -1783,6 +1843,7 @@
 
 int dw_lifespan_reset(dw_handle* h) {
     NEED(h, DW_EINVAL, "null handle");
+    SETTLE(h);
     const dw_params& p = h->prm;
     HIPCHK(hipSetDevice(p.device));
     const size_t bn = (size_t)p.batch * (p.n_agents > 0 ? p.n_agents : 1);
@@ -1794,6 +1855,7 @@
 
 int dw_lifespan_accumulate(dw_handle* h, uint32_t threshold_k) {
     NEED(h, DW_EINVAL, "null handle");
+    SETTLE(h);
     const dw_params& p = h->prm;
     HIPCHK(hipSetDevice(p.device));
     HIPCHK(hipMemsetAsync(h->n_alive.get(), 0, sizeof(int), h->stream));
@@ -1806,6 +1868,7 @@
 
 int dw_lifespan_download(dw_handle* h, int32_t* done_at, int32_t* agents_done_at, int32_t* n_worlds_alive) {
     NEED(h, DW_EINVAL, "null handle");
+    SETTLE(h);
     const dw_params& p = h->prm;
     HIPCHK(hipSetDevice(p.device));
     if (done_at) HIPCHK(hipMemcpyAsync(done_at, h->done_at.get(), sizeof(int) * p.batch, hipMemcpyDeviceToHost, h->stream));
@@ -1997,6 +2060,7 @@
                             uint8_t* world_alive, uint8_t* agent_ok, dw_world_stats* trace) {
     const dw_params& p = h->prm;
     HIPCHK(hipSetDevice(p.device));
+    SETTLE(h);
     if (int rc = check_episode_call(h, nsteps, policy_mode, use_table, table)) return rc;
     const int C = p.height * p.width, N = p.n_agents, B = p.batch;
     const EpisodeForm form = episode_form(h);
@@ -2061,6 +2125,7 @@
                             uint8_t* agent_ok) {
     NEED(h && worlds && L_schedule, DW_EINVAL, "null argument");
     NEED(policy_mode >= 0 && policy_mode <= 3, DW_EINVAL, "bad policy mode");
+    SETTLE(h);
     const dw_params& p = h->prm;
     HIPCHK(hipSetDevice(p.device));
     if (int rc = check_episode_call(h, nsteps, policy_mode, use_table, table)) return rc;
@@ -2143,6 +2208,7 @@
 
 int dw_snapshot_save_slot(dw_handle* h, int32_t slot) {
     NEED(h, DW_EINVAL, "null handle");
+    SETTLE(h);
     NEED(slot >= 0 && slot < DW_SNAPSHOT_SLOTS, DW_EINVAL, "snapshot slot out of range");
     const dw_params& p = h->prm;
     HIPCHK(hipSetDevice(p.device));
@@ -2210,6 +2276,7 @@
     if (int rc = launch_copy_regions(h, J)) return rc;
     HIPCHK(hipMemsetAsync(h->stats2[1 - h->sp].get(), 0, h->stats_bytes, h->stream));
     h->unq = sn.unq;
+    h->tail_deferred = false;
     h->stepped = sn.stepped;
     h->L_last = sn.L_last;
     h->L_per_world = sn.L_per_world;
@@ -2223,6 +2290,7 @@
 
 int dw_set_stream(dw_handle* h, void* hip_stream) {
     NEED(h, DW_EINVAL, "null handle");
+    SETTLE(h);
     HIPCHK(hipSetDevice(h->prm.device));
     HIPCHK(hipStreamSynchronize(h->stream));
     if (h->own_stream) HIPCHK(hipStreamDestroy(h->stream));
@@ -2257,6 +2325,7 @@
 int dw_device_planes(dw_handle* h, int which, void** light, void** dark) {
     NEED(h && light && dark, DW_EINVAL, "null argument");
     NEED(which == DW_STATE_CURRENT || which == DW_STATE_PREVIOUS, DW_EINVAL, "bad state selector");
+    if (which == DW_STATE_PREVIOUS) SETTLE(h);
     const int buf = which == DW_STATE_CURRENT ? h->cur : 1 - h->cur;
     NEED(which != DW_STATE_CURRENT || cur_quantised(h), DW_ESTATE,
          "the current state is an un-quantised upload: it has no binary16 planes before the first step");
@@ -2290,6 +2359,10 @@
                 snprintf(buf + m, buflen - m, ", seam strips: %d x %d columns + %d columns of %d row bands per wave", pl.seam_geom.ncs,
                          kSeamCols, pl.left_geom.cols_per_strip, pl.left_geom.wpr);
             }
+            if (pl.fmt_planes && !h->sw.no_deferred_tail) {
+                const size_t m = std::strlen(buf);
+                snprintf(buf + m, buflen - m, "; an even run ends on a pair that reduces its second step (_last_pw), tail deferred");
+            }
             const size_t m = std::strlen(buf);
             snprintf(buf + m, buflen - m, ")");
         }
@@ -2342,6 +2415,7 @@
 
 int dw_audit_tie_bound(dw_handle* h, double L, double out[4]) {
     NEED(h && out, DW_EINVAL, "null argument");
+    SETTLE(h);
     const dw_params& p = h->prm;
     HIPCHK(hipSetDevice(p.device));
     NEED(h->have_state && cur_quantised(h), DW_ESTATE, "the audit needs a quantised current state");
diff --git a/therldaisyworld_amd/csrc/dw_common.hpp b/therldaisyworld_amd/csrc/dw_common.hpp
--- a/therldaisyworld_amd/csrc/dw_common.hpp
+++ b/therldaisyworld_amd/csrc/dw_common.hpp
@@ -55,6 +55,11 @@
 }
 __device__ __forceinline__ float4 fmt_load4(const dw_i32x4& rsrc, int voff, int soff) {
     const dw_fmt_f32x4 v = dw_buf_load_fmt4(rsrc, voff, soff, 0);
+    return make_float4(v.x, v.y, v.z, v.w);
+}
+constexpr int kBufAuxAgentScope = 16;
+__device__ __forceinline__ float4 fmt_load4_agent(const dw_i32x4& rsrc, int voff) {
+    const dw_fmt_f32x4 v = dw_buf_load_fmt4(rsrc, voff, 0, kBufAuxAgentScope);
     return make_float4(v.x, v.y, v.z, v.w);
 }
 __device__ __forceinline__ float4 fmt_load2x2(const dw_i32x4& rsrc, int voff_a, int voff_b, int soff) {
diff --git a/therldaisyworld_amd/csrc/dw_plan.hpp b/therldaisyworld_amd/csrc/dw_plan.hpp
--- a/therldaisyworld_amd/csrc/dw_plan.hpp
+++ b/therldaisyworld_amd/csrc/dw_plan.hpp
@@ -13,7 +13,7 @@
 
 struct Switches {
     bool no_sym = false, no_pack = false, no_fuse = false, no_ring = false, no_fmt_planes = false, no_seam_strips = false,
-         no_episode_kernel = false,
+         no_deferred_tail = false, no_episode_kernel = false,
          no_episode_wave = false, no_agent_fuse = false, no_agent_preapply = false, first_f64 = false,
          first_generic = false, force_rescan = false, test_hooks = false;
     int pack_min_strips = -1, strip_rows = 0, tile_rpt = 0, queue_cap = -1, mismatch_cap = -1, trace_rows = 0;
@@ -37,6 +37,7 @@
     w.test_hooks = std::getenv("DW_TEST_HOOKS") != nullptr;
     flag("DW_NO_SYM", w.no_sym); flag("DW_NO_PACK", w.no_pack); flag("DW_NO_FUSE", w.no_fuse); flag("DW_NO_RING", w.no_ring);
     flag("DW_NO_FMT_PLANES", w.no_fmt_planes); flag("DW_NO_SEAM_STRIPS", w.no_seam_strips);
+    flag("DW_NO_DEFERRED_TAIL", w.no_deferred_tail);
     flag("DW_NO_EPISODE_KERNEL", w.no_episode_kernel); flag("DW_NO_EPISODE_WAVE", w.no_episode_wave);
     flag("DW_NO_AGENT_FUSE", w.no_agent_fuse); flag("DW_NO_AGENT_PREAPPLY", w.no_agent_preapply);
     flag("DW_FIRST_STEP_F64", w.first_f64); flag("DW_FIRST_GENERIC", w.first_generic);
diff --git a/therldaisyworld_amd/csrc/dw_step_fused.hpp b/therldaisyworld_amd/csrc/dw_step_fused.hpp
--- a/therldaisyworld_amd/csrc/dw_step_fused.hpp
+++ b/therldaisyworld_amd/csrc/dw_step_fused.hpp
@@ -56,7 +56,7 @@
 }
 
 template <int MODE, bool EXACT, bool PACK = false, bool STATS = false, bool SYM = false, typename TI = plane_t,
-          typename TO = plane_t, bool TRACE = false, bool FMT = false, int SEAM = kSeamNone>
+          typename TO = plane_t, bool TRACE = false, bool FMT = false, int SEAM = kSeamNone, bool LAST = false>
 __device__ __forceinline__ void fused2_body(const TI* __restrict__ inL, const TI* __restrict__ inD,
                                             TO* __restrict__ outL, TO* __restrict__ outD, const FusedGeom& G,
                                             const PhysF32& P1_, const PhysF32& P2_, const PhysF64& P64,
@@ -68,6 +68,7 @@
     static_assert(!RING || !PACK, "the ring exchange is written for un-packed worlds");
     static_assert(!TRACE || (!PACK && !STATS && !RING), "the trace form exists for un-packed overlapped / rotating strips");
     static_assert(SEAM == kSeamNone || FMT, "the seam strips exist for the format-access kernel");
+    static_assert(!LAST || FMT, "the reductions of step 2 alone exist for the format-access kernels");
     static_assert(!FMT || (MODE == kFusedOvl && !EXACT && !PACK && !STATS && !TRACE), "the format-access form exists for the plain float32 kernel on overlapped strips");
     __shared__ float s_edge[RING ? 2 * 4 * 8 : 1];
     __shared__ uint4 s_queue[EXACT ? 4 * kWaveQueueCap * 3 : 1];
@@ -446,6 +447,7 @@
                 }
             } else if constexpr (FMT) {
                 if (writes) {
+                    if constexpr (LAST) trace_step2(l2, d2);
                     fmt_store4(fmt_outL, fmt_col, (r0 + j - 4) * fmt_row, make_float4(l2[0], l2[1], l2[2], l2[3]));
                     fmt_store4(fmt_outD, fmt_col, (r0 + j - 4) * fmt_row, make_float4(d2[0], d2[1], d2[2], d2[3]));
                 }
@@ -684,6 +686,41 @@
             atomicAdd(&t2->sum_d, (unsigned long long)d2);
         }
     }
+    if constexpr (LAST) {
+        if constexpr (SEAM == kSeamLeft) {
+            wait_row_stores_before_patching();
+            for (int k0 = 0; k0 < nr; k0 += 8) {
+                float4 wl[8], wd[8];
+#pragma unroll
+                for (int jj = 0; jj < 8; ++jj) {
+                    const int voff = fmt_col + (r0 + band_dr + min(k0 + jj, band_nr - 1)) * fmt_row;
+                    wl[jj] = fmt_load4_agent(fmt_outL, voff);
+                    wd[jj] = fmt_load4_agent(fmt_outD, voff);
+                }
+#pragma unroll
+                for (int jj = 0; jj < 8; ++jj) {
+                    if (writes && k0 + jj < band_nr) {
+                        const float ol[4] = {wl[jj].x, wl[jj].y, wl[jj].z, wl[jj].w}, od[4] = {wd[jj].x, wd[jj].y, wd[jj].z, wd[jj].w};
+                        trace_step2(ol, od);
+                    }
+                }
+            }
+        }
+        unsigned int l2 = (unsigned int)tr_l2.x + (unsigned int)tr_l2.y;
+        unsigned int d2 = (unsigned int)tr_d2.x + (unsigned int)tr_d2.y;
+        const float m2 = wave_max(__int_as_float(tr_m2));
+#pragma unroll
+        for (int o = 32; o > 0; o >>= 1) {
+            l2 += (unsigned int)__shfl_xor((int)l2, o, 64);
+            d2 += (unsigned int)__shfl_xor((int)d2, o, 64);
+        }
+        if (lane == 0) {
+            StatsDev* const t2 = trace + b;
+            atomicMax(&t2->max_k, (unsigned int)m2);
+            atomicAdd(&t2->sum_l, (unsigned long long)l2);
+            atomicAdd(&t2->sum_d, (unsigned long long)d2);
+        }
+    }
     if (STATS) {
         if (PACK) {
             float m = st_m1;
@@ -766,6 +803,35 @@
                                                                                                 zero, zero, zero_me, zero_n);
 }
 
+template <int MODE>
+__global__ __launch_bounds__(256) __attribute__((amdgpu_waves_per_eu(DW_FUSED_FAST_WAVES, DW_FUSED_FAST_WAVES)))
+void step_stream_fused2_fmt_last_pw(const plane_t* __restrict__ inL, const plane_t* __restrict__ inD,
+                                    plane_t* __restrict__ outL, plane_t* __restrict__ outD, FusedGeom G, PhysF32 P1, PhysF32 P2,
+                                    unsigned long long* __restrict__ zero_me, int zero_n, StatsDev* __restrict__ stats) {
+    const PhysF64 dummy{};
+    const double zero = 0.0;
+    fused2_body<MODE, false, false, false, false, plane_t, plane_t, false, true, kSeamNone, true>(
+        inL, inD, outL, outD, G, P1, P2, dummy, zero, zero, zero_me, zero_n, nullptr, 0.f, stats);
+}
+__global__ __launch_bounds__(256) __attribute__((amdgpu_waves_per_eu(DW_FUSED_FAST_WAVES, DW_FUSED_FAST_WAVES)))
+void step_stream_fused2_seam_last_pw(const plane_t* __restrict__ inL, const plane_t* __restrict__ inD,
+                                     plane_t* __restrict__ outL, plane_t* __restrict__ outD, FusedGeom G, PhysF32 P1, PhysF32 P2,
+                                     unsigned long long* __restrict__ zero_me, int zero_n, StatsDev* __restrict__ stats) {
+    const PhysF64 dummy{};
+    const double zero = 0.0;
+    fused2_body<kFusedOvl, false, false, false, false, plane_t, plane_t, false, true, kSeamStrip, true>(
+        inL, inD, outL, outD, G, P1, P2, dummy, zero, zero, zero_me, zero_n, nullptr, 0.f, stats);
+}
+__global__ __launch_bounds__(256) __attribute__((amdgpu_waves_per_eu(DW_FUSED_FAST_WAVES, DW_FUSED_FAST_WAVES)))
+void step_stream_fused2_left_last_pw(const plane_t* __restrict__ inL, const plane_t* __restrict__ inD,
+                                     plane_t* __restrict__ outL, plane_t* __restrict__ outD, FusedGeom G, PhysF32 P1, PhysF32 P2,
+                                     unsigned long long* __restrict__ zero_me, int zero_n, StatsDev* __restrict__ stats) {
+    const PhysF64 dummy{};
+    const double zero = 0.0;
+    fused2_body<kFusedOvl, false, false, false, false, plane_t, plane_t, false, true, kSeamLeft, true>(
+        inL, inD, outL, outD, G, P1, P2, dummy, zero, zero, zero_me, zero_n, nullptr, 0.f, stats);
+}
+
 #ifndef DW_EXACT_PACK_WAVES
 #define DW_EXACT_PACK_WAVES 3
 #endif
```

Result: no change. 829.2 billion, median of 6 (+0.4%).
